# saforem2/l2hmc-qcd

Measured on AMD Instinct MI355X. Metric: chain*leapfrog-steps/sec, 4D SU(3) 8^4 fp64 (+ plaquette/force-kernel HBM GB/s in "rooflines"), higher is better.
Workload: dtype f64; 1 GPU; 4D SU(3) 8x8x8x8, beta=6.0, 256 chains/GPU, complex128/fp64, Dynamics.forward merged L2HMC, nleapfrog=4 (8 LF steps/trajectory), vnet units [256], verbose=False, default Dynamics switches (mc_states.out.v is formed on first access); global_chains=256, parallelism=chains sharded x1

## Files before the change

include/l2q.h:

```cpp
#ifndef L2Q_H_
#define L2Q_H_

#include <stddef.h>
#include <stdint.h>

#ifdef __cplusplus
extern "C" {
#endif

#define L2Q_OK 0
#define L2Q_EINVAL (-1)
#define L2Q_ESHAPE (-2)
#define L2Q_EHIP (-3)

#define L2Q_ACT_NONE 0
#define L2Q_ACT_TANH 1
#define L2Q_ACT_RELU 2
#define L2Q_ACT_LEAKY_RELU 3
#define L2Q_ACT_ELU 4
#define L2Q_ACT_SWISH 5

#define L2Q_HALF_F16 0
#define L2Q_HALF_BF16 1

const char* l2q_last_error(void);
int l2q_version(void);
int l2q_set_tuning(const char* key, int value);
int l2q_kernel_name(const char* entry, int T, int X, int Y, int Z, char* buf, size_t buf_bytes);
int l2q_init(int device);

#define L2Q_COMM_ID_BYTES 128
int l2q_comm_unique_id(void* id_out);
int l2q_comm_init(const void* id, int nranks, int rank, void** comm_out);
int l2q_allreduce_grads(void* comm, void* grad, long n, int elem_bytes, void* stream);
int l2q_comm_destroy(void* comm);
int l2q_comm_abort(void* comm);
int l2q_comm_version(void);

size_t l2q_reduce_ws_bytes(int nb, long n_per_chain);

int l2q_transpose(const void* in, void* out, long batch, int rows, int cols, int elem_bytes,
                  void* stream);
int l2q_su3_pack(const void* x_ref, void* x_nat, int nb, long V, void* stream);
int l2q_su3_unpack(const void* x_nat, void* x_ref, int nb, long V, void* stream);
int l2q_su3_unpack_select(const void* a_nat, const void* b_nat, const float* mask, void* x_ref, int nb,
                          long V, void* stream);

int l2q_su3_plaq_reduce(const void* xn, int nb, int T, int X, int Y, int Z, double* out,
                        void* ws, size_t ws_bytes, void* stream);
int l2q_su3_plaq_planes(const void* xn, int nb, int T, int X, int Y, int Z, double* out, void* ws,
                        size_t ws_bytes, void* stream);
int l2q_su3_wilson_loops(const void* xn, int nb, int T, int X, int Y, int Z, void* out, void* stream);
int l2q_diff_norm2_reduce(const double* a, const double* b, int nb, long n, double* out, void* ws,
                          size_t ws_bytes, void* stream);
int l2q_su3_force(const void* xn, double beta, void* fn, int nb, int T, int X, int Y, int Z,
                  void* stream);
int l2q_su3_force_kick(const void* xn, double beta, double coef, void* vn, int nb, int T,
                       int X, int Y, int Z, void* stream);
int l2q_su3_force_kick_to(const void* xn, double beta, double coef, const void* v_in, void* v_out,
                          int nb, int T, int X, int Y, int Z, void* stream);
int l2q_su3_expm_mul(const void* xn, const void* vn, double eps, const float* mask_n,
                     int complement, void* out, int nb, long V, void* stream);
int l2q_su3_expm_mul2(const void* xn, const void* vn, double eps, const float* mask_n,
                      int complement_first, void* out, int nb, long V, void* stream);
int l2q_su3_expm_mul2_vec8(const void* xn, const void* vn, double eps, const float* mask_n,
                           int complement_first, void* out, double* vec, int nb, long V,
                           void* stream);
int l2q_su3_expm_mul2_digits(const void* xn, const void* vn, double eps, const float* mask_n, int complement_first,
                             void* out, void* image, int a_exp, int nb, long V, void* stream);
int l2q_su3_projsu_digits(const void* in, void* image, int a_exp, long nfields, long V, void* stream);
int l2q_su3_project_su(const void* in, void* out, long nfields, long V, void* stream);
int l2q_su3_projsu_vec8(const void* in, double* vec, long nfields, long V, void* stream);
int l2q_su3_project_u(const void* in, void* out, long nfields, long V, void* stream);
int l2q_su3_mul(const void* a, const void* b, int adjoint_a, int adjoint_b, void* out,
                long nfields, long V, void* stream);
int l2q_su3_project_tah(const void* in, void* out, long nfields, long V, void* stream);
int l2q_su3_kinetic_reduce(const void* vn, int nb, long V, double* out, void* ws,
                           size_t ws_bytes, void* stream);
int l2q_su3_assemble_tah(const double* normals, void* vn, long nfields, long V, void* stream);
int l2q_su3_check_su(const void* xn, int nb, long V, double* out, void* ws, size_t ws_bytes,
                     void* stream);

int l2q_su3_clover_reduce(const void* xn, int nb, int T, int X, int Y, int Z, double* out,
                          void* ws, size_t ws_bytes, void* stream);
int l2q_su3_flow_stage(const void* x_in, const void* p_in, double c, double s, void* p_out, void* x_out,
                       int nb, int T, int X, int Y, int Z, void* stream);
int l2q_su3_flow_step(const void* x_in, void* x_out, void* ws_p, void* ws_x, double eps, int nb, int T, int X,
                      int Y, int Z, void* stream);

int l2q_su3_line_extend(const void* lines_in, const void* xn, int n, void* lines_out, int nb, int T, int X, int Y,
                        int Z, void* stream);
int l2q_su3_loop_reduce(const void* a, int r, const void* b, int t, double* out, int nb, int T, int X, int Y, int Z,
                        void* ws, size_t ws_bytes, void* stream);
int l2q_su3_polyakov(const void* xn, int mu, void* out, int nb, int T, int X, int Y, int Z, void* stream);

int l2q_su3_heatbath(void* xn, double beta, int mu, int parity, const double* u, int ntry, double* fails, int nb,
                     int T, int X, int Y, int Z, void* ws, size_t ws_bytes, void* stream);
int l2q_su3_overrelax(void* xn, int mu, int parity, int nb, int T, int X, int Y, int Z, void* stream);

int l2q_v_update(void* v, const void* force, const void* s, const void* t, const void* q,
                 double eps, int forward, int is_complex, int elem_bytes, int nb, long n,
                 void* logdet, void* ws, size_t ws_bytes, void* stream);
int l2q_v_update_to(const void* v_in, void* v_out, const void* force, const void* s, const void* t,
                    const void* q, double eps, int forward, int is_complex, int elem_bytes, int nb,
                    long n, void* logdet, void* ws, size_t ws_bytes, void* stream);

int l2q_accept(const void* h_init, const void* h_prop, const void* sumlogdet, const void* u,
               void* acc, float* mask, int nb, int elem_bytes, void* stream);
int l2q_select_rows(const void* a, const void* b, const float* mask, void* out, int nb,
                    long row_bytes, void* stream);
int l2q_scale_f64(const double* x, double alpha, double* y, long n, void* stream);

int l2q_gemm_f64(const double* A, const double* W, int M, int N, long K, const double* A2,
                 const double* W2, long K2, const double* bias, const double* bias2,
                 const double* coeff, double scale, int act, double* C, void* ws,
                 size_t ws_bytes, void* stream);
size_t l2q_gemm_ws_bytes(int M, int N, long K, long K2);
size_t l2q_gemm_sliced_bytes(int N, long K);
int l2q_gemm_sliced_build(const double* W, int N, long K, void* image, size_t image_bytes, int* usable,
                          void* stream);
size_t l2q_gemm_sliced_ws_bytes(int M, int N, long K, long K2);
int l2q_gemm_sliced_f64(const double* A, const void* image, long K, int a_exp, const double* A2,
                        const void* image2, long K2, int a2_exp, int M, int N, const double* bias,
                        const double* bias2, const double* coeff, double scale, int act, double* C, void* ws,
                        size_t ws_bytes, void* stream);
size_t l2q_gemm_digits_bytes(long M, long K);
int l2q_gemm_digits_slice(const double* A, long M, long K, int a_exp, void* image, size_t image_bytes, void* stream);
int l2q_gemm_digits_f64(const void* A, const void* image, long K, int a_exp, const void* A2, const void* image2,
                        long K2, int a2_exp, int M, int N, const double* bias, const double* bias2,
                        const double* coeff, double scale, int act, double* C, void* ws, size_t ws_bytes,
                        void* stream);
int l2q_vnet_heads_vupdate_f64(const double* Z, int M, int K, long N, const double* Ws,
                               const double* bs, const double* cs, double scale_s,
                               const double* Wt, const double* bt, double scale_t,
                               const double* Wq, const double* bq, const double* cq,
                               double scale_q, void* v, const void* force, int is_complex,
                               double eps, int forward, double* logdet, void* ws,
                               size_t ws_bytes, void* stream);
int l2q_vnet_heads_vupdate_to_f64(const double* Z, int M, int K, long N, const double* Ws,
                                  const double* bs, const double* cs, double scale_s,
                                  const double* Wt, const double* bt, double scale_t,
                                  const double* Wq, const double* bq, const double* cq,
                                  double scale_q, const void* v_in, void* v_out, const void* force,
                                  int is_complex, double eps, int forward, double* logdet, void* ws,
                                  size_t ws_bytes, void* stream);
int l2q_vnet_heads_vupdate_pair_f64(const double* Z, int M, int K, long N, const double* Ws,
                                    const double* bs, const double* cs, double scale_s,
                                    const double* Wt, const double* bt, double scale_t,
                                    const double* Wq, const double* bq, const double* cq,
                                    double scale_q, void* v, const void* force, int is_complex,
                                    double eps1, int forward1, int flip_between, double eps2,
                                    int forward2, double* logdet, void* ws, size_t ws_bytes,
                                    void* stream);
int l2q_vnet_heads_vupdate_pair_mid_f64(const double* Z, int M, int K, long N, const double* Ws,
                                        const double* bs, const double* cs, double scale_s,
                                        const double* Wt, const double* bt, double scale_t,
                                        const double* Wq, const double* bq, const double* cq,
                                        double scale_q, void* v, const void* force, int is_complex,
                                        double eps1, int forward1, int flip_between, double eps2,
                                        int forward2, double* logdet, double* logdet1,
                                        double* vnorm2_mid, void* ws, size_t ws_bytes, void* stream);
size_t l2q_vnet_heads_ws_bytes(int M, long N);
// ... 221 lines not shown
```

l2hmc-qcd_amd/csrc/heads_common.hpp:

```cpp
#pragma once
#include "l2q_common.hpp"

namespace l2q {

__device__ __forceinline__ double rcp_nr(double d) {
  double r = __builtin_amdgcn_rcp(d);
  r = fma(r, fma(-d, r, 1.0), r);
  r = fma(r, fma(-d, r, 1.0), r);
  return r;
}

__device__ __forceinline__ double fast_tanh(double x) {
  const double c = fmin(fmax(x, -20.0), 20.0);
  const double t = 1.0 - 2.0 * rcp_nr(exp(2.0 * c) + 1.0);
  return (x != x) ? x : t;
}

__device__ __forceinline__ double exp_small(double x) {
  if (fabs(x) < 0.125) {
    double r = 1.0 / 39916800.0;
    r = fma(r, x, 1.0 / 3628800.0);
    r = fma(r, x, 1.0 / 362880.0);
    r = fma(r, x, 1.0 / 40320.0);
    r = fma(r, x, 1.0 / 5040.0);
    r = fma(r, x, 1.0 / 720.0);
    r = fma(r, x, 1.0 / 120.0);
    r = fma(r, x, 1.0 / 24.0);
    r = fma(r, x, 1.0 / 6.0);
    r = fma(r, x, 0.5);
    r = fma(r, x, 1.0);
    return fma(r, x, 1.0);
  }
  return exp(x);
}
__device__ __forceinline__ double exp_bf_core(double xc) {
  const double k = __builtin_rint(xc * 1.4426950408889634);
  double r = fma(-k, 6.93147180369123816490e-01, xc);
  r = fma(-k, 1.90821492927058770002e-10, r);
  double p = 1.0 / 479001600.0;
  p = fma(p, r, 1.0 / 39916800.0);
  p = fma(p, r, 1.0 / 3628800.0);
  p = fma(p, r, 1.0 / 362880.0);
  p = fma(p, r, 1.0 / 40320.0);
  p = fma(p, r, 1.0 / 5040.0);
  p = fma(p, r, 1.0 / 720.0);
  p = fma(p, r, 1.0 / 120.0);
  p = fma(p, r, 1.0 / 24.0);
  p = fma(p, r, 1.0 / 6.0);
  p = fma(p, r, 0.5);
  p = fma(p, r, 1.0);
  p = fma(p, r, 1.0);
  return __builtin_amdgcn_ldexp(p, (int)k);
}
__device__ __forceinline__ double exp_bf(double x) {
  const double y = exp_bf_core(fmin(fmax(x, -708.0), 709.0));
  return (x != x) ? x : y;
}
__device__ __forceinline__ double tanh_bf(double x) {
  const double c = fmin(fmax(x, -20.0), 20.0);
  const double t = 1.0 - 2.0 * rcp_nr(exp_bf_core(2.0 * c) + 1.0);
  return (x != x) ? x : t;
}

struct HeadsArgs {
  const double* Z;
  const double* W[3];
  const double* b[3];
  const double* cs;
  const double* cq;
  double ss, st, sq;
  double eps;
  double eps2;
  int fwd2, flip;
  double* v;
  const double* vin;
  const double* F;
  double* logdet_part;
  double* ld1_part;
  double* ke_part;
  int M, N, K, ncols_part;
  double* tape_s = nullptr;
  double* tape_t = nullptr;
  double* tape_q = nullptr;
};

}
```

l2hmc-qcd_amd/csrc/heads_sliced.hip:

```cpp
#include "heads_common.hpp"
#include <type_traits>
#include <vector>

namespace l2q {

constexpr int OZ_NS = 7;
constexpr int OZ_BITS = 54;
constexpr int OZ_KB = 4;
constexpr int OZ_K = 64 * OZ_KB;
constexpr int OZ_FRAG = 1024;
constexpr int OZ_CHUNK = OZ_NS * OZ_KB * OZ_FRAG;

#ifndef L2Q_SL_PROF
#define L2Q_SL_PROF 0
#endif
#ifndef L2Q_SL_V2
#define L2Q_SL_V2 1
#endif
#ifndef L2Q_SL_SKIP
#define L2Q_SL_SKIP 0
#endif
typedef int v4i32 __attribute__((ext_vector_type(4)));
typedef __attribute__((address_space(3))) void* lds_ptr_t;

// ... 351 lines not shown
    p = fma(p, r, 1.0 / 39916800.0);
    p = fma(p, r, 1.0 / 3628800.0);
    p = fma(p, r, 1.0 / 362880.0);
    p = fma(p, r, 1.0 / 40320.0);
    p = fma(p, r, 1.0 / 5040.0);
    p = fma(p, r, 1.0 / 720.0);
    p = fma(p, r, 1.0 / 120.0);
    p = fma(p, r, 1.0 / 24.0);
    p = fma(p, r, 1.0 / 6.0);
    p = fma(p, r, 0.5);
    p = fma(p, r, 1.0);
    return fma(p, r, 1.0);
  };
#if L2Q_SL_V2
  auto exp_poly7 = [](double r) {
    double p = 1.0 / 5040.0;
    p = fma(p, r, 1.0 / 720.0);
    p = fma(p, r, 1.0 / 120.0);
    p = fma(p, r, 1.0 / 24.0);
    p = fma(p, r, 1.0 / 6.0);
    p = fma(p, r, 0.5);
    p = fma(p, r, 1.0);
    return fma(p, r, 1.0);
  };
#endif
  auto exp4x2 = [&](const double (&xa)[4], const double (&xb)[4], double (&ya)[4], double (&yb)[4]) {
    bool small = true;
#pragma unroll
    for (int r = 0; r < 4; ++r) small = small && fabs(xa[r]) < 0.34 && fabs(xb[r]) < 0.34;
#if L2Q_SL_V2
    bool tiny = true;
#pragma unroll
    for (int r = 0; r < 4; ++r) tiny = tiny && fabs(xa[r]) < 0x1p-6 && fabs(xb[r]) < 0x1p-6;
    if (__all(tiny)) {
#pragma unroll
      for (int r = 0; r < 4; ++r) { ya[r] = exp_poly7(xa[r]); yb[r] = exp_poly7(xb[r]); }
      return;
    }
#endif
    if (__all(small)) {
#pragma unroll
      for (int r = 0; r < 4; ++r) { ya[r] = exp_poly(xa[r]); yb[r] = exp_poly(xb[r]); }
    } else {
#pragma unroll
      for (int r = 0; r < 4; ++r) { ya[r] = exp_bf(xa[r]); yb[r] = exp_bf(xb[r]); }
    }
  };
  auto stage_b = [&] {
    if (L2Q_SL_SKIP & 1) return;
    double xa[4], xb[4];
#pragma unroll
    for (int r = 0; r < 4; ++r) {
      xa[r] = FWD ? heps * s_[r] : -heps * s_[r];
      xb[r] = eps * q_[r];
    }
    exp4x2(xa, xb, es_, eq_);
    if (PAIR && !same2) {
#pragma unroll
      for (int r = 0; r < 4; ++r) {
        xa[r] = a.fwd2 ? h2 * s_[r] : -h2 * s_[r];
        xb[r] = a.eps2 * q_[r];
      }
      exp4x2(xa, xb, es2_, eq2_);
    }
  };
  auto stage_c = [&](long t, const Operands& q, double2 (&outv)[4]) {
    const long n = t * 16 + (lane & 15);
#pragma unroll
    for (int r = 0; r < 4; ++r) {
      const bool ok = n < a.N && (mrow + r) < a.M;
      double vr = q.vv[r].x, vi = q.vv[r].y;
      const double fr0 = q.ff[r].x, fi0 = q.ff[r].y;
      if (L2Q_SL_SKIP & 1) { vr += s_[r] + t_[r] + fr0; vi += q_[r] + fi0; }
      else {
        const double s = s_[r], tt = t_[r];
        const double lj = FWD ? heps * s : -heps * s;
        {
          const double fr = fr0 * eq_[r] + tt, fi = fi0 * eq_[r];
          if (FWD) { vr = es_[r] * vr - heps * fr; vi = es_[r] * vi - heps * fi; }
          else { vr = es_[r] * (vr + heps * fr); vi = es_[r] * (vi + heps * fi); }
        }
        if (!PAIR) {
          if (ok) ld[r] += lj;
        } else {
          if (MID) { if (ok) { ld1[r] += lj; ke[r] += fma(vr, vr, vi * vi); } }
          if (a.flip) { vr = -vr; vi = -vi; }
          const double lj2 = a.fwd2 ? h2 * s : -h2 * s;
          if (ok) ld[r] += lj + lj2;
          const double e2 = same2 ? es_[r] : es2_[r], g2 = same2 ? eq_[r] : eq2_[r];
          const double fr = fr0 * g2 + tt, fi = fi0 * g2;
          if (a.fwd2) { vr = e2 * vr - h2 * fr; vi = e2 * vi - h2 * fi; }
          else { vr = e2 * (vr + h2 * fr); vi = e2 * (vi + h2 * fi); }
        }
      }
      outv[r] = make_double2(vr, vi);
    }
  };
  auto store = [&](long t, const double2 (&outv)[4]) {
    const long n = t * 16 + (lane & 15);
#pragma unroll
    for (int r = 0; r < 4; ++r) {
      if (n < a.N && (mrow + r) < a.M) {
        const long oo = rowoff[r] + n;
        if (CPLX) reinterpret_cast<double2*>(a.v)[oo] = outv[r];
        else a.v[oo] = outv[r].x;
        if (TAPE) { a.tape_s[oo] = s_[r]; a.tape_t[oo] = t_[r]; a.tape_q[oo] = q_[r]; }
      }
    }
  };
  Operands cur, nxt;
  const char* wsrc = o.Wsl + t0 * 3 * (long)OZ_CHUNK + lane * 16;
  auto issue = [&](long qi, int f0) {
    const long qc = qi < nq ? qi : nq - 1;
    const int stage = (int)(qi % 3);
    const char* src = wsrc + qc * (long)OZ_CHUNK;
    __builtin_amdgcn_sched_barrier(0);
#pragma unroll
    for (int f = f0; f < OZ_NS; ++f) {
      const int frag = p + 4 * f;
      __builtin_amdgcn_global_load_lds((const __attribute__((address_space(1))) void*)(src + frag * OZ_FRAG),
                                       (lds_ptr_t)(lds + stage * OZ_CHUNK + frag * OZ_FRAG), 16, 0, 0);
    }
    __builtin_amdgcn_sched_barrier(0);
  };
#if L2Q_SL_PROF
  long long prof_bar = 0, prof_mem = 0, prof_conv = 0;
  const long long prof_t0 = clock64();
#define L2Q_SL_T(acc, ...) do { const long long c0_ = clock64(); __VA_ARGS__; acc += clock64() - c0_; } while (0)
#define L2Q_SL_CBAR(vm) do { const long long c0_ = clock64();                                            \
    asm volatile("s_waitcnt vmcnt(" #vm ") lgkmcnt(0)\n\ts_barrier" ::: "memory"); prof_bar += clock64() - c0_; } while (0)
#else
#define L2Q_SL_T(acc, ...) do { __VA_ARGS__; } while (0)
#define L2Q_SL_CBAR(vm) asm volatile("s_waitcnt vmcnt(" #vm ") lgkmcnt(0)\n\ts_barrier" ::: "memory")
#endif
  double fs[4], ft[4], fq[4], gs[4], gt[4];
  double2 outv[4];
  if (ntl > 0) {
    issue(0, 0);
    issue(1, 0);
    fetch(t0, cur);
    L2Q_SL_CBAR(16);
    issue(2, L2Q_SL_NPD);
    L2Q_SL_CBAR(0);
    issue(3, L2Q_SL_NPD);
    conv(0, fs);
#if L2Q_SL_V2
    tanh_s(cur, fs, sn_);
#endif
    L2Q_SL_CBAR(0);
    issue(4, L2Q_SL_NPD);
    conv(1, ft);
    for (long u = 0; u < ntl; ++u) {
      const long t = t0 + u;
      const bool more = u + 1 < ntl;
      L2Q_SL_CBAR(0);
      L2Q_SL_T(prof_mem, if (u > 0) store(t - 1, outv); issue(3 * u + 5, L2Q_SL_NPD));
      L2Q_SL_T(prof_conv, conv(3 * u + 2, fq));
      L2Q_SL_T(prof_mem, fetch(more ? t + 1 : t, nxt));
      stage_a(cur, fs, ft, fq);
      if (more) {
        L2Q_SL_CBAR(16);
        L2Q_SL_T(prof_mem, issue(3 * u + 6, L2Q_SL_NPD));
        L2Q_SL_T(prof_conv, conv(3 * u + 3, gs));
      }
      stage_b();
      if (more) {
        L2Q_SL_CBAR(0);
        L2Q_SL_T(prof_mem, issue(3 * u + 7, L2Q_SL_NPD));
        L2Q_SL_T(prof_conv, conv(3 * u + 4, gt));
      }
      stage_c(t, cur, outv);
#if L2Q_SL_V2
      if (more) tanh_s(nxt, gs, sn_);
#endif
      if (more) {
        cur = nxt;
#pragma unroll
        for (int r = 0; r < 4; ++r) { fs[r] = gs[r]; ft[r] = gt[r]; }
      }
    }
    store(t1 - 1, outv);
  } else {
    L2Q_SL_CBAR(0);
  }
#undef L2Q_SL_CBAR
#undef L2Q_SL_T
#if L2Q_SL_PROF
  if (o.dbg && lane == 0) {
    long long* d = o.dbg + ((long)blockIdx.x * 8 + wave) * 4;
    d[0] = clock64() - prof_t0; d[1] = prof_bar; d[2] = prof_mem; d[3] = prof_conv;
  }
#endif
  asm volatile("s_waitcnt vmcnt(0)" ::: "memory");
#pragma unroll
  for (int r = 0; r < 4; ++r) {
    double x = ld[r], x1 = ld1[r], xk = ke[r];
#pragma unroll
    for (int off = 8; off > 0; off >>= 1) {
      x += __shfl_xor(x, off, 64);
      if (MID) { x1 += __shfl_xor(x1, off, 64); xk += __shfl_xor(xk, off, 64); }
    }
    const long m = mrow + r;
    if ((lane & 15) == 0 && m < a.M) {
      a.logdet_part[m * a.ncols_part + cw] = x;
      if (MID) {
        a.ld1_part[m * a.ncols_part + cw] = x1;
        a.ke_part[m * a.ncols_part + cw] = xk;
      }
    }
  }
}

static inline long sliced_chunks(long N) { return cdiv(N, 16) * 3; }
static inline size_t sliced_scale_off(long N) { return ((size_t)sliced_chunks(N) * OZ_CHUNK + 255) & ~(size_t)255; }
static inline int sliced_rg(int M) { return (int)cdiv(M, 64); }
static inline int sliced_ncw(int M) {
  const int per_xcd = 32 / sliced_rg(M);
  return 8 * (per_xcd > 0 ? per_xcd : 1);
}

}

using namespace l2q;

static int sliced_launch(const char* who, double* tape_s, double* tape_t, double* tape_q, const double* Z, int M,
                         int K, long N, const void* sliced,
                                      const double* bs, const double* cs, double scale_s, const double* bt,
                                      double scale_t, const double* bq, const double* cq, double scale_q,
                                      const void* v_in, void* v, const void* force, int is_complex, double eps1,
                                      int forward1, int pair, int flip_between, double eps2, int forward2,
                                      double* logdet, double* logdet1, double* vnorm2_mid, void* ws,
                                      size_t ws_bytes, void* stream) {
  L2Q_REQUIRE(Z && sliced && bs && bt && bq && cs && cq && v && force && logdet && ws, L2Q_EINVAL,
              "null pointer (the sliced kernel takes per-entry scales cs / cq)");
  L2Q_REQUIRE(K == OZ_K, L2Q_ESHAPE, "the sliced heads kernel serves K = 256");
  L2Q_REQUIRE(M > 0 && N > 0 && N < 2000000000L, L2Q_EINVAL, "bad size");
  const bool mid = logdet1 != nullptr;
  L2Q_REQUIRE(!mid || (pair && vnorm2_mid), L2Q_EINVAL, "mid-point outputs belong to the pair kernel");
  L2Q_REQUIRE(ws_bytes >= l2q_vnet_heads_sliced_ws_bytes(M, N), L2Q_ESHAPE, "workspace too small");
  auto al = [](const void* p) { return (reinterpret_cast<uintptr_t>(p) & 15) == 0; };
  const void* vin = v_in ? v_in : v;
  L2Q_REQUIRE(al(Z) && al(v) && al(vin) && al(force) && (reinterpret_cast<uintptr_t>(sliced) & 255) == 0 &&
                  (reinterpret_cast<uintptr_t>(ws) & 255) == 0,
              L2Q_ESHAPE, "operands must be 16-byte aligned (slice buffer and workspace 256-byte)");
  hipStream_t st = (hipStream_t)stream;
  const int rg = sliced_rg(M), ncw = sliced_ncw(M);
  const long mpad = (long)rg * 64;
  char* zs = (char*)ws;
  double* zscale = (double*)(zs + (mpad / 16) * OZ_CHUNK);
  double* part = zscale + mpad;
  hipLaunchKernelGGL(oz_split_kernel, dim3((unsigned)cdiv(mpad, 4)), dim3(256), 0, st, Z, (long)M, mpad, 1, 0,
                     zs, zscale, 1, oz_zflag_ptr(), 0x1p-6);
  HeadsArgs a;
  a.tape_s = tape_s; a.tape_t = tape_t; a.tape_q = tape_q;
  a.Z = Z; a.W[0] = a.W[1] = a.W[2] = nullptr;
  a.b[0] = bs; a.b[1] = bt; a.b[2] = bq; a.cs = cs; a.cq = cq;
  a.ss = scale_s; a.st = scale_t; a.sq = scale_q; a.eps = eps1; a.eps2 = eps2; a.fwd2 = forward2;
  a.flip = flip_between;
  a.v = (double*)v; a.vin = (const double*)vin; a.F = (const double*)force;
  a.logdet_part = part; a.ld1_part = part + (size_t)M * ncw; a.ke_part = part + 2 * (size_t)M * ncw;
  a.M = M; a.N = (int)N; a.K = K; a.ncols_part = ncw;
  SlicedArgs o;
  o.Zs = zs; o.zscale = zscale; o.Wsl = (const char*)sliced;
  o.wscale = (const double*)((const char*)sliced + sliced_scale_off(N));
  o.ncw = ncw; o.rg = rg; o.dbg = nullptr;
#if L2Q_SL_PROF
  static long long* dbg = nullptr;
  if (!dbg) (void)hipMalloc(&dbg, 4096 * 8 * 4 * sizeof(long long));
  (void)hipMemsetAsync(dbg, 0, 4096 * 8 * 4 * sizeof(long long), st);
  o.dbg = dbg;
#endif
  o.tiles_per_cw = (int)cdiv(cdiv(N, 16), ncw);
  const dim3 grid((unsigned)(rg * ncw)), block(512);
#define L2Q_SL(C, F, P, MD) hipLaunchKernelGGL((heads_sliced_kernel<C, F, P, MD>), grid, block, 0, st, a, o)
#define L2Q_SL_F(C, P, MD) do { if (forward1) L2Q_SL(C, true, P, MD); else L2Q_SL(C, false, P, MD); } while (0)
#define L2Q_SL_C(P, MD) do { if (is_complex) L2Q_SL_F(true, P, MD); else L2Q_SL_F(false, P, MD); } while (0)
  if (tape_s) {
    if (is_complex) {
      if (forward1) hipLaunchKernelGGL((heads_sliced_kernel<true, true, false, false, true>), grid, block, 0, st, a, o);
      else hipLaunchKernelGGL((heads_sliced_kernel<true, false, false, false, true>), grid, block, 0, st, a, o);
    } else {
      if (forward1) hipLaunchKernelGGL((heads_sliced_kernel<false, true, false, false, true>), grid, block, 0, st, a, o);
      else hipLaunchKernelGGL((heads_sliced_kernel<false, false, false, false, true>), grid, block, 0, st, a, o);
    }
  } else if (mid) L2Q_SL_C(true, true);
  else if (pair) L2Q_SL_C(true, false);
  else L2Q_SL_C(false, false);
#undef L2Q_SL_C
#undef L2Q_SL_F
#undef L2Q_SL
#if L2Q_SL_PROF
  {
    (void)hipStreamSynchronize(st);
    const int nblk = rg * ncw;
    std::vector<long long> h((size_t)nblk * 8 * 4);
    (void)hipMemcpy(h.data(), o.dbg, h.size() * sizeof(long long), hipMemcpyDeviceToHost);
    double tot[2] = {0, 0}, bar[2] = {0, 0}, vm = 0, ldsw = 0, mx[2] = {0, 0}, umem = 0, uconv = 0;
    for (int b = 0; b < nblk; ++b)
      for (int w = 0; w < 8; ++w) {
        const long long* d = &h[((size_t)b * 8 + w) * 4];
        const int c = w >= 4;
        tot[c] += d[0]; bar[c] += d[1]; if (!c) { vm += d[2]; ldsw += d[3]; }
        else { umem += d[2]; uconv += d[3]; }
        if (d[0] > mx[c]) mx[c] = (double)d[0];
      }
    const double n = nblk * 4.0;
    fprintf(stderr, "[sliced prof] matrix waves: total %.0f (max %.0f) barrier %.0f vmcnt %.0f lgkmcnt %.0f | update waves: total %.0f barrier %.0f dma+fetch+store issue %.0f conv %.0f  (clock64 ticks, mean per wave)\n",
            tot[0] / n, mx[0], bar[0] / n, vm / n, ldsw / n, tot[1] / n, bar[1] / n, umem / n, uconv / n);
  }
#endif
  launch_finalize(a.logdet_part, logdet, M, ncw, 1, 1.0, 0.0, st);
  if (mid) {
    launch_finalize(a.ld1_part, logdet1, M, ncw, 1, 1.0, 0.0, st);
    launch_finalize(a.ke_part, vnorm2_mid, M, ncw, 1, 1.0, 0.0, st);
  }
  return check_launch(who);
}

extern "C" {

size_t l2q_heads_sliced_bytes(int K, long N) {
  if (K != OZ_K || N <= 0) return 0;
  return sliced_scale_off(N) + (size_t)3 * N * sizeof(double) + 256;
}

int l2q_heads_sliced_build(const double* Ws, const double* Wt, const double* Wq, int K, long N, void* sliced,
                           size_t sliced_bytes, int* usable, void* stream) {
  L2Q_REQUIRE(Ws && Wt && Wq && sliced && usable, L2Q_EINVAL, "null pointer");
  L2Q_REQUIRE(K == OZ_K, L2Q_ESHAPE, "the sliced heads kernel serves K = 256");
  L2Q_REQUIRE(N > 0 && N < 2000000000L, L2Q_EINVAL, "bad size");
  L2Q_REQUIRE(sliced_bytes >= l2q_heads_sliced_bytes(K, N), L2Q_ESHAPE, "buffer too small");
  auto al = [](const void* p) { return (reinterpret_cast<uintptr_t>(p) & 15) == 0; };
  L2Q_REQUIRE(al(Ws) && al(Wt) && al(Wq) && (reinterpret_cast<uintptr_t>(sliced) & 255) == 0, L2Q_ESHAPE,
              "operands must be 16-byte aligned (the slice buffer 256-byte)");
  hipStream_t st = (hipStream_t)stream;
  char* buf = (char*)sliced;
  double* wscale = (double*)(buf + sliced_scale_off(N));
  int* flag = (int*)(wscale + 3 * N);
  (void)hipMemsetAsync(flag, 0, sizeof(int), st);
  const long Npad = cdiv(N, 16) * 16;
  const double* W[3] = {Ws, Wt, Wq};
  for (int h = 0; h < 3; ++h)
    hipLaunchKernelGGL(oz_split_kernel, dim3((unsigned)cdiv(Npad, 4)), dim3(256), 0, st, W[h], N, Npad, 3, h,
                       buf, wscale + (long)h * N, 0, flag, 0x1p-6);
  int hflag = 0;
  if (hipMemcpyAsync(&hflag, flag, sizeof(int), hipMemcpyDeviceToHost, st) != hipSuccess ||
      hipStreamSynchronize(st) != hipSuccess) {
    set_error("l2q_heads_sliced_build: %s", hipGetErrorString(hipGetLastError()));
    return L2Q_EHIP;
  }
  *usable = hflag ? 0 : 1;
  return check_launch("l2q_heads_sliced_build");
}

int l2q_heads_sliced_zflag(int reset, int* count, void* stream) {
  L2Q_REQUIRE(count, L2Q_EINVAL, "null pointer");
  hipStream_t st = (hipStream_t)stream;
  int* p = oz_zflag_ptr();
  L2Q_REQUIRE(p, L2Q_EHIP, "device symbol not found");
  if (hipMemcpyAsync(count, p, sizeof(int), hipMemcpyDeviceToHost, st) != hipSuccess ||
      (reset && hipMemsetAsync(p, 0, sizeof(int), st) != hipSuccess) ||
      hipStreamSynchronize(st) != hipSuccess) {
    set_error("l2q_heads_sliced_zflag: %s", hipGetErrorString(hipGetLastError()));
    return L2Q_EHIP;
  }
  return L2Q_OK;
}

size_t l2q_vnet_heads_sliced_ws_bytes(int M, long N) {
  if (M <= 0 || N <= 0) return 0;
  const size_t mpad = (size_t)sliced_rg(M) * 64;
  return (mpad / 16) * OZ_CHUNK + mpad * sizeof(double) + (size_t)M * sliced_ncw(M) * 3 * sizeof(double) + 512;
}

int l2q_vnet_heads_vupdate_sliced_f64(const double* Z, int M, int K, long N, const void* sliced,
                                      const double* bs, const double* cs, double scale_s, const double* bt,
                                      double scale_t, const double* bq, const double* cq, double scale_q,
                                      const void* v_in, void* v, const void* force, int is_complex, double eps1,
                                      int forward1, int pair, int flip_between, double eps2, int forward2,
                                      double* logdet, double* logdet1, double* vnorm2_mid, void* ws,
                                      size_t ws_bytes, void* stream) {
  return sliced_launch("l2q_vnet_heads_vupdate_sliced_f64", nullptr, nullptr, nullptr, Z, M, K, N, sliced, bs, cs,
                       scale_s, bt, scale_t, bq, cq, scale_q, v_in, v, force, is_complex, eps1, forward1, pair,
                       flip_between, eps2, forward2, logdet, logdet1, vnorm2_mid, ws, ws_bytes, stream);
}

int l2q_vnet_heads_vupdate_sliced_tape_f64(const double* Z, int M, int K, long N, const void* sliced,
                                           const double* bs, const double* cs, const double* bt, double scale_t,
                                           const double* bq, const double* cq, const void* v_in, void* v,
                                           const void* force, int is_complex, double eps, int forward,
                                           double* s_out, double* t_out, double* q_out, double* logdet, void* ws,
                                           size_t ws_bytes, void* stream) {
  L2Q_REQUIRE(s_out && t_out && q_out, L2Q_EINVAL, "null pointer");
  return sliced_launch("l2q_vnet_heads_vupdate_sliced_tape_f64", s_out, t_out, q_out, Z, M, K, N, sliced, bs, cs, 1.0,
                       bt, scale_t, bq, cq, 1.0, v_in, v, force, is_complex, eps, forward, 0, 0, 0.0, 0, logdet,
                       nullptr, nullptr, ws, ws_bytes, stream);
}

// ... 2 lines not shown
```

l2hmc-qcd_amd/csrc/su3_force_link.hip:

```cpp
#include "su3_force_tile.hpp"
#include "su3_launch.hpp"

namespace l2q {

#ifdef L2Q_LK_NOFENCE
#define L2Q_LK_FENCE() do { } while (0)
#else
#define L2Q_LK_FENCE() do { asm volatile("" ::: "memory"); __builtin_amdgcn_sched_barrier(0); } while (0)
#endif

#ifndef L2Q_LK_EXP
#define L2Q_LK_EXP 0
#endif
#ifndef L2Q_LK_FULL_DIAG
#define L2Q_LK_FULL_DIAG 0
#endif

constexpr int kLkThreads = kRS * 4;
constexpr int kLkOffS0 = 0, kLkOffS1 = 3 * kPlaneB, kLkOffT = 6 * kPlaneB;
constexpr int kLkLds = 7 * kPlaneB;

template <int INM>
__device__ __forceinline__ constexpr bool lk_in(int dir) { return dir == 0 ? true : ((INM >> (dir - 1)) & 1) != 0; }

struct LkCtx {
  __amdgpu_buffer_rsrc_t rs, ro, rv;
  Dims d;
  int V16, Vs16, tile0b, lt, t0, t1;
  int sp, px, py, pz;
  double coef;
  int lo;
};

__host__ __device__ constexpr int lk_other(int mu, int j) { return j + (j >= mu ? 1 : 0); }

template <int MODE, int MU, int INM>
__device__ __forceinline__ void force_link_sweep(const LkCtx& c) {
  constexpr bool IN_MU = lk_in<INM>(MU);
  const Dims& d = c.d;
  const int T = d.T, V16 = c.V16, Vs16 = c.Vs16;
  const __amdgpu_buffer_rsrc_t rs = c.rs, ro = c.ro, rv = c.rv;
  const int q_sp = c.sp * 16;
  int q_pmu = q_sp, mx = c.px, my = c.py, mz = c.pz;
  if (MU != 0) {
    int q = hop(c.sp, c.px, c.py, c.pz, MU, +1, d);
    q_pmu = q * 16;
    mz = q % d.Z; q /= d.Z;
    my = q % d.Y; q /= d.Y;
    mx = q;
  }
  int q_pp[4], q_pm[4], q_pmm[4];
#pragma unroll
  for (int nu = 1; nu < 4; ++nu) {
    q_pp[nu] = hop(c.sp, c.px, c.py, c.pz, nu, +1, d) * 16;
    q_pm[nu] = hop(c.sp, c.px, c.py, c.pz, nu, -1, d) * 16;
    q_pmm[nu] = hop(q_pmu / 16, mx, my, mz, nu, -1, d) * 16;
  }
  const int lb = -c.tile0b;
  const int own = (MU == 0 ? 0 : (MU - 1) * kPlaneB) + c.lt * 16;
  {
    const int ta = (c.t0 - 1 + T) % T;
#pragma unroll
    for (int e = 0; e < 9; ++e) {
      const double2 va = buf_ld(rs, q_sp, (MU * 9 + e) * V16 + ta * Vs16);
      if (MU == 0) {
        *reinterpret_cast<double2*>(fr_lds + kLkOffT + own + e * kEnt) = va;
      } else {
        const double2 vb = buf_ld(rs, q_sp, (MU * 9 + e) * V16 + (c.t0 % T) * Vs16);
        *reinterpret_cast<double2*>(fr_lds + kLkOffS0 + own + e * kEnt) = va;
        *reinterpret_cast<double2*>(fr_lds + kLkOffS1 + own + e * kEnt) = vb;
      }
    }
  }
  __syncthreads();
  int cur = 0;
  M3 carry;
  if (MU != 0) m3_zero(carry);
  const int niter = (c.t1 - c.t0) + 1;
#pragma unroll 1
  for (int it = 0; it < niter; ++it) {
    const int tcur = (c.t0 - 1 + it + T) % T;
    const int tnext = (tcur + 1 == T) ? 0 : tcur + 1;
    const int offSc = cur ? kLkOffS1 : kLkOffS0;
    const int offSn = cur ? kLkOffS0 : kLkOffS1;
    const int gcur = tcur * Vs16, gnxt = tnext * Vs16;
    const bool more = it + 1 < niter;
    auto oc = [&](int rho, int qb) {
      return Opnd<true>{(rho == 0 ? kLkOffT : offSc + (rho - 1) * kPlaneB) + lb + qb, qb, rho * 9 * V16 + gcur};
    };
    auto on = [&](int rho, int qb) {
      return Opnd<true>{offSn + (rho - 1) * kPlaneB + lb + qb, qb, rho * 9 * V16 + gnxt};
    };
#if L2Q_LK_EXP & 1
    auto gco = [&](int rho, int qb) { return oc(rho, q_sp); };
    auto gno = [&](int rho, int qb) { return on(rho == 0 ? 1 : rho, q_sp); };
#else
    auto gco = [&](int rho, int qb) { return Opnd<false>{0, qb, rho * 9 * V16 + gcur}; };
    auto gno = [&](int rho, int qb) { return Opnd<false>{0, qb, rho * 9 * V16 + gnxt}; };
#endif
    double2 pre[9];
    if (more && !(L2Q_LK_EXP & 4)) {
      const int tp = MU == 0 ? tnext : ((tnext + 1 == T) ? 0 : tnext + 1);
#pragma unroll
      for (int e = 0; e < 9; ++e) pre[e] = buf_ld(rs, q_sp, (MU * 9 + e) * V16 + tp * Vs16);
    }
    M3 acc;
    double2 outv[9];
    m3_zero(acc);
    if constexpr (MU == 0) {
      if (it >= c.lo) {
#pragma unroll
        for (int nu_ = 1; nu_ < 4; ++nu_) {
          const int nu = (L2Q_LK_EXP & 64) ? 4 - nu_ : nu_;
          M3 a, t;
          if (it >= c.lo) {
          ld_m(a, on(nu, q_sp), rs, V16);
          if (lk_in<INM>(nu)) mul_xh_stream<false>(t, a, oc(0, q_pp[nu]), rs, V16);
          else mul_xh_stream<false>(t, a, gco(0, q_pp[nu]), rs, V16);
          mac_stream<true>(acc, t, oc(nu, q_sp), rs, V16);
          }
// ... 17 lines not shown
        M3 a, t;
        if (IN_MU) ld_m(a, oc(0, q_pmu), rs, V16);
        else ld_m(a, gco(0, q_pmu), rs, V16);
        if (it >= c.lo) {
          acc = carry;
          mul_xh_stream<false>(t, a, on(MU, q_sp), rs, V16);
          mac_stream<true>(acc, t, oc(0, q_sp), rs, V16);
          L2Q_LK_FENCE();
        }
        if (more) {
          mul_xh_stream<true>(t, a, oc(MU, q_sp), rs, V16);
          m3_zero(carry);
          mac_stream<false>(carry, t, oc(0, q_sp), rs, V16);
          L2Q_LK_FENCE();
        }
      }
      if (it >= c.lo) {
#pragma unroll
        for (int nu_ = 1; nu_ < 4; ++nu_) {
          const int nu = (L2Q_LK_EXP & 64) ? 4 - nu_ : nu_;
          if (nu == MU) continue;
          M3 a, t;
          if (it >= c.lo) {
          if (IN_MU) ld_m(a, oc(nu, q_pmu), rs, V16);
          else ld_m(a, gco(nu, q_pmu), rs, V16);
          if (lk_in<INM>(nu)) mul_xh_stream<false>(t, a, oc(MU, q_pp[nu]), rs, V16);
          else mul_xh_stream<false>(t, a, gco(MU, q_pp[nu]), rs, V16);
          mac_stream<true>(acc, t, oc(nu, q_sp), rs, V16);
          }
          L2Q_LK_FENCE();
          if (it < c.lo) continue;
          if (IN_MU && lk_in<INM>(nu)) ld_m(a, oc(nu, q_pmm[nu]), rs, V16);
          else ld_m(a, gco(nu, q_pmm[nu]), rs, V16);
          if (lk_in<INM>(nu)) {
            mul_xh_stream<true>(t, a, oc(MU, q_pm[nu]), rs, V16);
            mac_stream<false>(acc, t, oc(nu, q_pm[nu]), rs, V16);
            L2Q_LK_FENCE();
          } else {
            mul_xh_stream<true>(t, a, gco(MU, q_pm[nu]), rs, V16);
            mac_stream<false>(acc, t, gco(nu, q_pm[nu]), rs, V16);
            L2Q_LK_FENCE();
          }
        }
      }
    }
    if (MODE == 2 && it >= c.lo) {
      const int so = MU * 9 * V16 + gcur;
      M3 gl, g;
#pragma unroll
      for (int e = 0; e < 9; ++e) {
        const double2 o = buf_ld_nt(rv, q_sp, so + e * V16);
        gl.re[e] = o.x; gl.im[e] = o.y;
      }
      m3_tah(g, gl);
#pragma unroll
      for (int i = 0; i < 3; ++i)
#pragma unroll
        for (int j = 0; j < 3; ++j) {
          double sr = 0.0, si = 0.0;
#pragma unroll
          for (int k = 0; k < 3; ++k) {
            const double ar = acc.re[3 * j + k], ai = -acc.im[3 * j + k];
            sr = fma(g.re[3 * i + k], ar, sr); sr = fma(-g.im[3 * i + k], ai, sr);
            si = fma(g.re[3 * i + k], ai, si); si = fma(g.im[3 * i + k], ar, si);
          }
          const double2 o = buf_ld_nt(ro, q_sp, so + (3 * i + j) * V16);
          outv[3 * i + j] = make_double2(fma(c.coef, sr, o.x), fma(c.coef, si, o.y));
        }
#pragma unroll
      for (int e = 0; e < 9; ++e) buf_st_nt(ro, q_sp, so + e * V16, outv[e]);
    }
    if (MODE != 2 && it >= c.lo) {
      M3 ua;
      const Opnd<true> uo = oc(MU, q_sp);
#pragma unroll
      for (int i = 0; i < 3; ++i) {
        R3 ur;
        ld_row<true>(ur, uo.lds, rs, uo.voff, uo.soff, V16, i);
#pragma unroll
        for (int j = 0; j < 3; ++j) {
          double sr = 0.0, si = 0.0;
#pragma unroll
          for (int k = 0; k < 3; ++k) {
            if (L2Q_LK_FULL_DIAG || i != j) { sr = fma(ur.re[k], acc.re[3 * k + j], sr); sr = fma(-ur.im[k], acc.im[3 * k + j], sr); }
            si = fma(ur.re[k], acc.im[3 * k + j], si); si = fma(ur.im[k], acc.re[3 * k + j], si);
          }
          ua.re[3 * i + j] = sr; ua.im[3 * i + j] = si;
        }
      }
      const int so = MU * 9 * V16 + gcur;
      const double tri = (ua.im[0] + ua.im[4] + ua.im[8]) / 3.0;
#pragma unroll
      for (int i = 0; i < 3; ++i)
#pragma unroll
        for (int j = 0; j < 3; ++j) {
          const int e = 3 * i + j, et = 3 * j + i;
          const double fr = (!L2Q_LK_FULL_DIAG && i == j) ? 0.0 : 0.5 * (ua.re[e] - ua.re[et]);
          double fi = 0.5 * (ua.im[e] + ua.im[et]);
          if (i == j) fi -= tri;
          double2 v2 = make_double2(c.coef * fr, c.coef * fi);
          if (MODE == 1) {
            const double2 o = buf_ld_nt(rv, q_sp, so + e * V16);
            v2.x += o.x; v2.y += o.y;
          }
          outv[e] = v2;
        }
      if (!(L2Q_LK_EXP & 32)) {
#pragma unroll
        for (int e = 0; e < 9; ++e)
          if (!(L2Q_LK_EXP & 2) || outv[e].x == 1.2345e300) {
            if (L2Q_LK_EXP & 16) buf_st(ro, q_sp, so + e * V16, outv[e]);
            else buf_st_nt(ro, q_sp, so + e * V16, outv[e]);
          }
      }
    }
    if (!(L2Q_LK_EXP & 8)) __syncthreads();
    if (more && !(L2Q_LK_EXP & 4)) {
      const int dst = (MU == 0 ? kLkOffT : offSc) + own;
#pragma unroll
      for (int e = 0; e < 9; ++e) *reinterpret_cast<double2*>(fr_lds + dst + e * kEnt) = pre[e];
    }
    if ((L2Q_LK_EXP & 32) && MODE != 2 && it >= c.lo) {
      const int so = MU * 9 * V16 + gcur;
#pragma unroll
      for (int e = 0; e < 9; ++e) {
        if (L2Q_LK_EXP & 16) buf_st(ro, q_sp, so + e * V16, outv[e]);
        else buf_st_nt(ro, q_sp, so + e * V16, outv[e]);
      }
    }
    cur ^= 1;
    if (!(L2Q_LK_EXP & 8)) __syncthreads();
  }
}

#ifndef L2Q_LK_OCC
#define L2Q_LK_OCC 2
#endif
template <int MODE, int INM>
__global__ __launch_bounds__(kLkThreads, L2Q_LK_OCC) void su3_force_link_kernel(
    const double2* __restrict__ xn, Dims d, int nsb, int tsplit, int swz, double coef,
    const double2* vin, double2* out, int lo, int stagger) {
  if (stagger > 0 && blockIdx.x >= 256 && blockIdx.x < 512) {
    for (int i = 0; i < stagger; ++i) __builtin_amdgcn_s_sleep(32);
  }
  const long w = xcd_swizzle(blockIdx.x, gridDim.x, swz);
  const int per_chain = nsb * tsplit;
  const long c = w / per_chain;
  const int rr = (int)(w % per_chain);
  const int tc = rr / nsb, sb = rr % nsb;
  const int V = d.V, T = d.T;
  LkCtx k;
  k.d = d;
  k.V16 = V * 16;
  k.Vs16 = d.X * d.Y * d.Z * 16;
  k.tile0b = sb * kRS * 16;
  k.lt = threadIdx.x & (kRS - 1);
  const int wv = __builtin_amdgcn_readfirstlane(threadIdx.x / kRS);
  const int tlen = (T + tsplit - 1) / tsplit;
  k.t0 = tc * tlen;
  k.t1 = min(T, k.t0 + tlen);
  const int chain_bytes = 36 * k.V16;
  k.rs = __builtin_amdgcn_make_buffer_rsrc((void*)(xn + c * 36L * V), 0, chain_bytes, 0x00020000);
  k.ro = __builtin_amdgcn_make_buffer_rsrc((void*)(out + c * 36L * V), 0, chain_bytes, 0x00020000);
  k.rv = __builtin_amdgcn_make_buffer_rsrc((void*)((MODE != 0 ? vin : out) + c * 36L * V), 0, chain_bytes, 0x00020000);
  k.sp = sb * kRS + k.lt;
  {
    int q = k.sp;
    k.pz = q % d.Z; q /= d.Z;
    k.py = q % d.Y; q /= d.Y;
    k.px = q;
  }
  k.coef = coef;
  k.lo = lo;
  switch (wv) {
    case 0: force_link_sweep<MODE, 0, INM>(k); break;
    case 1: force_link_sweep<MODE, 1, INM>(k); break;
    case 2: force_link_sweep<MODE, 2, INM>(k); break;
    default: force_link_sweep<MODE, 3, INM>(k); break;
  }
}

template <int MODE, int INM>
static void launch_link_variant(const double2* xn, Dims d, int nb, int nsb, int tsplit, double coef,
                                const double2* vin, double2* out, hipStream_t st) {
  static PerDeviceOnce attr_once;
  if (attr_once.first()) {
    (void)hipFuncSetAttribute((const void*)su3_force_link_kernel<MODE, INM>,
                              hipFuncAttributeMaxDynamicSharedMemorySize, kLkLds);
  }
  hipLaunchKernelGGL((su3_force_link_kernel<MODE, INM>), dim3((unsigned)((long)nb * nsb * tsplit)),
                     dim3(kLkThreads), kLkLds, st, xn, d, nsb, tsplit, tuning().xcd_swizzle, coef, vin, out, 1,
                     tuning().force_stagger);
}

int force_link_inmask(const Dims& d) {
  int m = 0;
  if (kRS % d.Z == 0) m |= 4;
  if (kRS % (d.Y * d.Z) == 0) m |= 2;
  if (kRS % (d.X * d.Y * d.Z) == 0) m |= 1;
  return m;
}

bool force_link_applicable(const Dims& d) {
  return (d.X * d.Y * d.Z) % kRS == 0 && 36.0 * d.V * 16.0 < 2.0e9;
}

void launch_force_link_bwd(const double2* xn, Dims d, int nb, double coef, const double2* gf, double2* gx,
                           hipStream_t st) {
  const int Vs = d.X * d.Y * d.Z;
  const int nsb = Vs / kRS;
  const int tsplit = t_chunks((long)nb * nsb, d.T, 1024);
  switch (force_link_inmask(d)) {
    case 7: launch_link_variant<2, 7>(xn, d, nb, nsb, tsplit, coef, gf, gx, st); break;
    case 6: launch_link_variant<2, 6>(xn, d, nb, nsb, tsplit, coef, gf, gx, st); break;
    case 4: launch_link_variant<2, 4>(xn, d, nb, nsb, tsplit, coef, gf, gx, st); break;
    default: launch_link_variant<2, 0>(xn, d, nb, nsb, tsplit, coef, gf, gx, st);
  }
}

void launch_force_link(bool kick, const double2* xn, Dims d, int nb, double coef, double2* out, hipStream_t st,
                       const double2* vin) {
  if (vin == nullptr) vin = out;
  const int Vs = d.X * d.Y * d.Z;
  const int nsb = Vs / kRS;
  const int tsplit = t_chunks((long)nb * nsb, d.T, 1024, tuning().force_tsplit);
#define L2Q_LK_CASE(M)                                                                    \
  case M:                                                                                 \
    if (kick) launch_link_variant<1, M>(xn, d, nb, nsb, tsplit, coef, vin, out, st);           \
    else launch_link_variant<0, M>(xn, d, nb, nsb, tsplit, coef, vin, out, st);                \
    break;
  switch (force_link_inmask(d)) {
    L2Q_LK_CASE(7)
    L2Q_LK_CASE(6)
    L2Q_LK_CASE(4)
    default:
      if (kick) launch_link_variant<1, 0>(xn, d, nb, nsb, tsplit, coef, vin, out, st);
      else launch_link_variant<0, 0>(xn, d, nb, nsb, tsplit, coef, vin, out, st);
  }
#undef L2Q_LK_CASE
}

}
```

l2hmc-qcd_amd/csrc/su3_kernels.hip:

```cpp
#include "su3_launch.hpp"
#include "digits.hpp"
#include "half_common.hpp"

namespace l2q {

template <int OCC>
__global__ __launch_bounds__(kBlock, OCC) void su3_plaq_kernel(const double2* __restrict__ xn,
                                                               Dims d, long nblk, int swz,
                                                               double* __restrict__ partial) {
  __shared__ double lds[8];
  const long total = (long)gridDim.x;
  const long w = xcd_swizzle(blockIdx.x, total, swz);
  const long c = w / nblk, blk = w % nblk;
  const int s = (int)blk * kBlock + threadIdx.x;
  double sr = 0.0, si = 0.0;
  if (s < d.V) {
    const double2* xc = xn + c * 36L * d.V;
    const Site p = site_coords(s, d);
    const int V = d.V;
#pragma unroll 1
    for (int u = 1; u < 4; ++u) {
      const int s_pu = fwd(s, coord_of(p, u), d, u);
#pragma unroll 1
      for (int v = 0; v < u; ++v) {
// ... 610 lines not shown
    }
  }
}
template <bool TWO, bool VEC8>
__global__ __launch_bounds__(kBlock, XU_OCC) void su3_expm_mul_kernel(const double2* xn,
                                                              const double2* __restrict__ vn,
                                                              double eps,
                                                              const float* __restrict__ mask,
                                                              int complement, double2* out,
                                                              double* __restrict__ out_vec,
                                                              int V, long nblk, int lo) {
  const long f = blockIdx.x / nblk, blk = blockIdx.x % nblk;
  const int s = (int)blk * kBlock + threadIdx.x;
  if (s >= V) return;
  su3_expm_mul_body<TWO, VEC8 ? 1 : 0>(xn, vn, eps, mask, complement, out, out_vec, V, f, s, lo, 0.0, 0.0, nullptr);
}
__global__ __launch_bounds__(kBlock, XU_OCC) void su3_expm_mul_digits_kernel(const double2* xn,
                                                                     const double2* __restrict__ vn, double eps,
                                                                     const float* __restrict__ mask, int complement,
                                                                     double2* out, char* __restrict__ image, int V,
                                                                     long nblk, int lo, double dsc, double dlim,
                                                                     int* flag) {
  const long f = blockIdx.x / nblk, blk = blockIdx.x % nblk;
  const int s = (int)blk * kBlock + threadIdx.x;
  if (s >= V) return;
  su3_expm_mul_body<true, 2>(xn, vn, eps, mask, complement, out, image, V, f, s, lo, dsc, dlim, flag);
}

template <int MODE>
__global__ __launch_bounds__(kBlock) void su3_project_kernel(const double2* in,
                                                             double2* out_links,
                                                             double* __restrict__ out_vec, int V,
                                                             long nblk) {
  const long f = blockIdx.x / nblk, blk = blockIdx.x % nblk;
  const int s = (int)blk * kBlock + threadIdx.x;
  if (s >= V) return;
  M3 x, r;
  load_link(x, in + f * 9L * V, V, s);
  if (MODE == 2) {
    m3_tah(r, x);
  } else if (MODE == 3) {
    m3_project_u(r, x);
  } else {
    m3_project_su(r, x);
  }
  if (MODE == 1) {
    double v[8];
    m3_to_vec8(v, r);
#pragma unroll
    for (int a = 0; a < 8; ++a) out_vec[(f * 8 + a) * (long)V + s] = v[a];
  } else {
    store_link(out_links + f * 9L * V, V, s, r);
  }
}
__global__ __launch_bounds__(kBlock) void su3_project_digits_kernel(const double2* in, char* __restrict__ image, int V,
                                                                    long nblk, double dsc, double dlim, int* flag) {
  const long f = blockIdx.x / nblk, blk = blockIdx.x % nblk;
  const int s = (int)blk * kBlock + threadIdx.x;
  if (s >= V) return;
  M3 x, r;
  load_link(x, in + f * 9L * V, V, s);
  m3_project_su(r, x);
  double v[8];
  m3_to_vec8(v, r);
  if (su3_vec8_to_digits(v, image, f, s, V, dsc, dlim)) atomicOr(flag, 1);
}

__global__ __launch_bounds__(kBlock) void su3_mul_kernel(const double2* a, const double2* b,
                                                         int adj_a, int adj_b, double2* out, int V,
                                                         long nblk) {
  const long f = blockIdx.x / nblk, blk = blockIdx.x % nblk;
  const int s = (int)blk * kBlock + threadIdx.x;
  if (s >= V) return;
  M3 x, y, r;
  load_link(x, a + f * 9L * V, V, s);
  load_link(y, b + f * 9L * V, V, s);
  if (adj_a && adj_b) m3_mul_aa(r, x, y);
  else if (adj_a) m3_mul_an(r, x, y);
  else if (adj_b) m3_mul_na(r, x, y);
  else m3_mul_nn(r, x, y);
  store_link(out + f * 9L * V, V, s, r);
}

__global__ __launch_bounds__(kBlock) void su3_assemble_tah_kernel(const double* __restrict__ nrm,
                                                                  double2* __restrict__ vn, long V,
                                                                  long nblk, long nlinks) {
  const long f = blockIdx.x / nblk, blk = blockIdx.x % nblk;
  const long s = blk * kBlock + threadIdx.x;
  if (s >= V) return;
  const long l = f * V + s;
  const double h = 0.70710678118654757;
  const double r3 = h * nrm[0 * nlinks + l];
  const double r8 = h * 0.57735026918962573 * nrm[1 * nlinks + l];
  const double r01 = h * nrm[2 * nlinks + l], r02 = h * nrm[3 * nlinks + l];
  const double r12 = h * nrm[4 * nlinks + l], i01 = h * nrm[5 * nlinks + l];
  const double i02 = h * nrm[6 * nlinks + l], i12 = h * nrm[7 * nlinks + l];
  double2* o = vn + f * 9 * V;
  o[0 * V + s] = make_double2(0.0, r8 + r3);
  o[1 * V + s] = make_double2(r01, i01);
  o[2 * V + s] = make_double2(r02, i02);
  o[3 * V + s] = make_double2(-r01, i01);
  o[4 * V + s] = make_double2(0.0, r8 - r3);
  o[5 * V + s] = make_double2(r12, i12);
  o[6 * V + s] = make_double2(-r02, i02);
  o[7 * V + s] = make_double2(-r12, i12);
  o[8 * V + s] = make_double2(0.0, -2.0 * r8);
}

__global__ __launch_bounds__(kBlock) void su3_norm2_kernel(const double2* __restrict__ vn,
                                                           long n_per_chain, long nblk,
                                                           double* __restrict__ partial) {
  __shared__ double lds[4];
  const long c = blockIdx.x / nblk, blk = blockIdx.x % nblk;
  const double2* v = vn + c * n_per_chain;
  double acc = 0.0;
  const long base = blk * (4L * kBlock);
#pragma unroll
  for (int k = 0; k < 4; ++k) {
    const long j = base + (long)k * kBlock + threadIdx.x;
    if (j < n_per_chain) {
      const double2 d = v[j];
      acc = fma(d.x, d.x, acc);
      acc = fma(d.y, d.y, acc);
    }
  }
  const double r = block_sum(acc, lds);
  if (threadIdx.x == 0) partial[c * nblk + blk] = r;
}

__global__ __launch_bounds__(kBlock) void su3_check_kernel(const double2* __restrict__ xn, long V,
                                                           long nblk, double* __restrict__ psum,
                                                           double* __restrict__ pmax) {
  __shared__ double lds[8];
  const long c = blockIdx.x / nblk, blk = blockIdx.x % nblk;
  const long l = blk * kBlock + threadIdx.x;
  double dv = 0.0;
  const bool on = l < 4 * V;
  if (on) {
    const long mu = l / V, s = l % V;
    M3 x, t;
    load_link(x, xn + (c * 4 + mu) * 9L * V, (int)V, (int)s);
    m3_mul_an(t, x, x);
    t.re[0] -= 1.0; t.re[4] -= 1.0; t.re[8] -= 1.0;
#pragma unroll
    for (int i = 0; i < 9; ++i) dv += t.re[i] * t.re[i] + t.im[i] * t.im[i];
    double dr, di;
    m3_det(dr, di, x);
    dv += (dr - 1.0) * (dr - 1.0) + di * di;
  }
  const double bs = block_sum(dv, lds);
  const double bm = block_max(dv, lds + 4);
  if (threadIdx.x == 0) { psum[c * nblk + blk] = bs; pmax[c * nblk + blk] = bm; }
}

__global__ void check_finalize_kernel(const double* __restrict__ psum,
                                      const double* __restrict__ pmax, long nblk, double nlinks,
                                      double* __restrict__ out) {
  __shared__ double lds[8];
  const long c = blockIdx.x;
  double s = 0.0, m = 0.0;
  for (long b = threadIdx.x; b < nblk; b += blockDim.x) {
    s += psum[c * nblk + b];
    m = fmax(m, pmax[c * nblk + b]);
  }
  const double ts = block_sum(s, lds);
  const double tm = block_max(m, lds + 4);
  if (threadIdx.x == 0) {
    out[c * 2 + 0] = sqrt(ts / nlinks / 20.0);
    out[c * 2 + 1] = sqrt(tm / 20.0);
  }
}

}

using namespace l2q;

template <bool KICK>
struct ForceInst {
  static constexpr int kFS = KICK ? kFSKick : kFSPlain, kVar = KICK ? 2 : 0, kLpt = KICK ? 1 : kLptPlain, kTileOcc = 2;
};

namespace l2q {
ForceKernel pick_force(const Dims& d, bool kick) {
  const int ft = tuning().force_tile;
  if (!kick && ft == 7 && force_plaq_applicable(d)) return ForceKernel::PlaqShare;
  if (ft >= 5 && force_link_applicable(d)) return ForceKernel::Link;
  return (d.X * d.Y * d.Z) % (kick ? kFSKick : kFSPlain) == 0 ? ForceKernel::Slice : ForceKernel::Tile;
}
}

template <bool KICK>
static void launch_force(const double2* xn, Dims d, int nb, double coef, double2* out, hipStream_t st) {
  using I = ForceInst<KICK>;
  switch (pick_force(d, KICK)) {
    case ForceKernel::PlaqShare: launch_force_plaq(xn, d, nb, coef, out, st); return;
    case ForceKernel::Link: launch_force_link(KICK, xn, d, nb, coef, out, st); return;
    case ForceKernel::Slice: {
      const int nsb = d.X * d.Y * d.Z / I::kFS;
      const int tsplit = t_chunks((long)nb * nsb, d.T, 512);
      const size_t lds = 2ul * 4 * 9 * I::kFS * sizeof(double2);
      static PerDeviceOnce attr_once;
      if (attr_once.first()) {
        (void)hipFuncSetAttribute((const void*)su3_force_slice_kernel<KICK, I::kFS, I::kVar, I::kLpt>,
                                  hipFuncAttributeMaxDynamicSharedMemorySize, (int)lds);
      }
      hipLaunchKernelGGL((su3_force_slice_kernel<KICK, I::kFS, I::kVar, I::kLpt>),
                         dim3((unsigned)((long)nb * nsb * tsplit)), dim3(4 * I::kFS / I::kLpt), lds, st, xn, d, nsb,
                         tsplit, tuning().xcd_swizzle, coef, out);
      return;
    }
    case ForceKernel::Tile: {
      const long ntile = cdiv(d.V, 64);
      hipLaunchKernelGGL((su3_force_tile_kernel<KICK, I::kTileOcc>), dim3((unsigned)(nb * ntile)), dim3(kBlock), 0,
                         st, xn, d, ntile, tuning().xcd_swizzle, coef, out);
    }
  }
}

template <bool KICK>
static void force_kernel_name(const Dims& d, char* buf, size_t n) {
  using I = ForceInst<KICK>;
  const char* k = KICK ? "true" : "false";
  switch (pick_force(d, KICK)) {
    case ForceKernel::PlaqShare: snprintf(buf, n, "su3_force_plaq_kernel"); break;
    case ForceKernel::Link: snprintf(buf, n, "su3_force_link_kernel<%d, %d>", KICK, force_link_inmask(d)); break;
    case ForceKernel::Slice:
      snprintf(buf, n, "su3_force_slice_kernel<%s, %d, %d, %d>", k, I::kFS, I::kVar, I::kLpt);
      break;
    case ForceKernel::Tile: snprintf(buf, n, "su3_force_tile_kernel<%s, %d>", k, I::kTileOcc);
  }
}

enum class PlaqKernel { SliceYZ, Slice, Flat };
constexpr int kPlaqOcc = 2;
static PlaqKernel pick_plaq(const Dims& d) {
  if ((d.X * d.Y * d.Z) % kSlice != 0) return PlaqKernel::Flat;
  return kSlice % (d.Y * d.Z) == 0 ? PlaqKernel::SliceYZ : PlaqKernel::Slice;
}

extern "C" {

int l2q_kernel_name(const char* entry, int T, int X, int Y, int Z, char* buf, size_t buf_bytes) {
  L2Q_REQUIRE(entry && buf && buf_bytes > 0, L2Q_EINVAL, "null pointer");
  const Dims dd = strncmp(entry, "l2q_su3_", 8) ? Dims{} : make_dims(T, X, Y, Z);
  buf[0] = 0;
  if (!strcmp(entry, "l2q_su3_plaq_reduce")) {
    const PlaqKernel pk = pick_plaq(dd);
    if (pk == PlaqKernel::Flat) snprintf(buf, buf_bytes, "su3_plaq_kernel<%d>", kPlaqOcc);
    else snprintf(buf, buf_bytes, "su3_plaq_slice_kernel<%s>", pk == PlaqKernel::SliceYZ ? "true" : "false");
  } else if (!strcmp(entry, "l2q_su3_force")) {
    force_kernel_name<false>(dd, buf, buf_bytes);
  } else if (!strcmp(entry, "l2q_su3_force_kick")) {
    force_kernel_name<true>(dd, buf, buf_bytes);
  } else if (!strcmp(entry, "l2q_su3_clover_reduce")) {
    snprintf(buf, buf_bytes, "%s", clover_slice_applicable(dd) ? "su3_clover_slice_kernel" : "su3_clover_kernel");
  } else if (!strcmp(entry, "l2q_su3_flow_stage")) {
    char kick[128];
    force_kernel_name<true>(dd, kick, sizeof(kick));
    snprintf(buf, buf_bytes, "%s + su3_expm_mul_kernel<false, false>", kick);
  } else if (!strcmp(entry, "l2q_vnet_heads_vupdate_sliced_f64")) {
    snprintf(buf, buf_bytes, "heads_sliced_kernel");
  } else if (!strncmp(entry, "l2q_vnet_heads_vupdate", 22)) {
    snprintf(buf, buf_bytes, "%s", heads_f64_kernel_name());
  } else if (!strcmp(entry, "l2q_gemm_h")) {
    snprintf(buf, buf_bytes, "%s", gemm_h_kernel_name(T, X, (long)Y));
  } else if (!strcmp(entry, "l2q_gemm_sliced_f64")) {
    snprintf(buf, buf_bytes, "gemm_sliced_kernel");
  } else if (!strcmp(entry, "l2q_gemm_digits_f64")) {
    snprintf(buf, buf_bytes, "gemm_digits_kernel");
  } else if (!strcmp(entry, "l2q_gemm_digits_slice")) {
    snprintf(buf, buf_bytes, "gd_slice_kernel");
  } else if (!strcmp(entry, "l2q_su3_expm_mul2_digits")) {
    snprintf(buf, buf_bytes, "su3_expm_mul_digits_kernel");
  } else if (!strcmp(entry, "l2q_su3_projsu_digits")) {
    snprintf(buf, buf_bytes, "su3_project_digits_kernel");
  } else if (!strcmp(entry, "l2q_gemm_f64")) {
    snprintf(buf, buf_bytes, "%s", gemm_f64_kernel_name());
  }
  return L2Q_OK;
}

size_t l2q_reduce_ws_bytes(int nb, long n_per_chain) {
  if (nb <= 0 || n_per_chain <= 0) return 0;
  return (size_t)nb * (size_t)cdiv(n_per_chain, kBlock) * 4 * sizeof(double) + 256;
}

int l2q_su3_plaq_reduce(const void* xn, int nb, int T, int X, int Y, int Z, double* out, void* ws,
                        size_t ws_bytes, void* stream) {
  L2Q_REQUIRE(xn && out && ws, L2Q_EINVAL, "null pointer");
  L2Q_REQUIRE(su3_dims_ok(nb, T, X, Y, Z), L2Q_EINVAL, "non-positive size");
  const Dims d = make_dims(T, X, Y, Z);
  hipStream_t st = (hipStream_t)stream;
  double* partial = (double*)ws;
  const int swz = tuning().xcd_swizzle;
  const PlaqKernel pk = pick_plaq(d);
  if (pk != PlaqKernel::Flat) {
    const int nsb = X * Y * Z / kSlice;
    const int tsplit = t_chunks((long)nb * nsb, T, 1024);
    const long per_chain = (long)nsb * tsplit;
    L2Q_REQUIRE(ws_bytes >= (size_t)nb * per_chain * 2 * sizeof(double), L2Q_ESHAPE, "workspace too small");
    if (pk == PlaqKernel::SliceYZ)
      hipLaunchKernelGGL(su3_plaq_slice_kernel<true>, dim3((unsigned)(nb * per_chain)), dim3(kSlice), 0, st,
                         (const double2*)xn, d, nsb, tsplit, swz, partial);
    else hipLaunchKernelGGL(su3_plaq_slice_kernel<false>, dim3((unsigned)(nb * per_chain)), dim3(kSlice), 0, st,
                            (const double2*)xn, d, nsb, tsplit, swz, partial);
    launch_finalize(partial, out, nb, per_chain, 2, 1.0, 0.0, st);
    return check_launch("l2q_su3_plaq_reduce");
  }
  const long nblk = cdiv(d.V, kBlock);
  L2Q_REQUIRE(ws_bytes >= (size_t)nb * nblk * 2 * sizeof(double), L2Q_ESHAPE, "workspace too small");
  hipLaunchKernelGGL(su3_plaq_kernel<kPlaqOcc>, dim3((unsigned)(nb * nblk)), dim3(kBlock), 0, st,
                     (const double2*)xn, d, nblk, swz, partial);
  launch_finalize(partial, out, nb, nblk, 2, 1.0, 0.0, st);
  return check_launch("l2q_su3_plaq_reduce");
}

int l2q_su3_wilson_loops(const void* xn, int nb, int T, int X, int Y, int Z, void* out, void* stream) {
  L2Q_REQUIRE(xn && out, L2Q_EINVAL, "null pointer");
  L2Q_REQUIRE(su3_dims_ok(nb, T, X, Y, Z), L2Q_EINVAL, "non-positive size");
  const Dims d = make_dims(T, X, Y, Z);
  const long nblk = cdiv(d.V, kBlock);
  hipLaunchKernelGGL(su3_wloops_kernel, dim3((unsigned)(nb * nblk)), dim3(kBlock), 0, (hipStream_t)stream,
                     (const double2*)xn, d, nblk, (long)nb, (double2*)out);
  return check_launch("l2q_su3_wilson_loops");
}

int l2q_su3_plaq_planes(const void* xn, int nb, int T, int X, int Y, int Z, double* out, void* ws,
                        size_t ws_bytes, void* stream) {
  L2Q_REQUIRE(xn && out && ws, L2Q_EINVAL, "null pointer");
  L2Q_REQUIRE(su3_dims_ok(nb, T, X, Y, Z), L2Q_EINVAL, "non-positive size");
  const Dims d = make_dims(T, X, Y, Z);
  const long nblk = cdiv(d.V, kBlock);
  L2Q_REQUIRE(ws_bytes >= (size_t)nb * nblk * 12 * sizeof(double), L2Q_ESHAPE, "workspace too small");
  hipStream_t st = (hipStream_t)stream;
  hipLaunchKernelGGL(su3_plaq_planes_kernel, dim3((unsigned)(nb * nblk)), dim3(kBlock), 0, st,
                     (const double2*)xn, d, nblk, (double*)ws);
  launch_finalize((const double*)ws, out, nb, nblk, 12, 1.0, 0.0, st);
  return check_launch("l2q_su3_plaq_planes");
}

int l2q_diff_norm2_reduce(const double* a, const double* b, int nb, long n, double* out, void* ws,
                          size_t ws_bytes, void* stream) {
  L2Q_REQUIRE(a && b && out && ws, L2Q_EINVAL, "null pointer");
  L2Q_REQUIRE(nb > 0 && n > 0, L2Q_EINVAL, "non-positive size");
  const long nblk = cdiv(n, 4L * kBlock);
  L2Q_REQUIRE(ws_bytes >= (size_t)nb * nblk * sizeof(double), L2Q_ESHAPE, "workspace too small");
  hipStream_t st = (hipStream_t)stream;
  hipLaunchKernelGGL(diff_norm2_kernel, dim3((unsigned)(nb * nblk)), dim3(kBlock), 0, st, a, b, n,
                     nblk, (double*)ws);
  launch_finalize((const double*)ws, out, nb, nblk, 1, 1.0, 0.0, st);
  return check_launch("l2q_diff_norm2_reduce");
}

int l2q_su3_force(const void* xn, double beta, void* fn, int nb, int T, int X, int Y, int Z,
                  void* stream) {
  L2Q_REQUIRE(xn && fn, L2Q_EINVAL, "null pointer");
  L2Q_REQUIRE(su3_dims_ok(nb, T, X, Y, Z), L2Q_EINVAL, "non-positive size");
  L2Q_REQUIRE(xn != fn, L2Q_EINVAL, "force output must not alias the gauge field");
  const Dims d = make_dims(T, X, Y, Z);
  launch_force<false>((const double2*)xn, d, nb, beta / 3.0, (double2*)fn, (hipStream_t)stream);
  return check_launch("l2q_su3_force");
}

int l2q_su3_force_kick(const void* xn, double beta, double coef, void* vn, int nb, int T, int X,
                       int Y, int Z, void* stream) {
  L2Q_REQUIRE(xn && vn, L2Q_EINVAL, "null pointer");
  L2Q_REQUIRE(su3_dims_ok(nb, T, X, Y, Z), L2Q_EINVAL, "non-positive size");
  const Dims d = make_dims(T, X, Y, Z);
  launch_force<true>((const double2*)xn, d, nb, coef * beta / 3.0, (double2*)vn, (hipStream_t)stream);
  return check_launch("l2q_su3_force_kick");
}

int l2q_su3_force_kick_to(const void* xn, double beta, double coef, const void* v_in, void* v_out,
                          int nb, int T, int X, int Y, int Z, void* stream) {
  L2Q_REQUIRE(xn && v_in && v_out, L2Q_EINVAL, "null pointer");
  L2Q_REQUIRE(su3_dims_ok(nb, T, X, Y, Z), L2Q_EINVAL, "non-positive size");
  const Dims d = make_dims(T, X, Y, Z);
  hipStream_t st = (hipStream_t)stream;
  if (v_in != v_out && force_link_runs(d)) {
    launch_force_link(true, (const double2*)xn, d, nb, coef * beta / 3.0, (double2*)v_out, st,
                      (const double2*)v_in);
    return check_launch("l2q_su3_force_kick_to");
  }
  if (v_in != v_out)
    (void)hipMemcpyAsync(v_out, v_in, (size_t)nb * 36 * d.V * sizeof(double2), hipMemcpyDeviceToDevice, st);
  return l2q_su3_force_kick(xn, beta, coef, v_out, nb, T, X, Y, Z, stream);
}

int l2q_su3_expm_mul(const void* xn, const void* vn, double eps, const float* mask_n,
                     int complement, void* out, int nb, long V, void* stream) {
  L2Q_REQUIRE(xn && vn && out, L2Q_EINVAL, "null pointer");
  L2Q_REQUIRE(su3_field_ok(nb, V), L2Q_EINVAL, "bad size");
  const long nblk = cdiv(V, kBlock);
  hipLaunchKernelGGL((su3_expm_mul_kernel<false, false>), dim3((unsigned)(nb * 4L * nblk)), dim3(kBlock),
                     0, (hipStream_t)stream, (const double2*)xn, (const double2*)vn, eps, mask_n,
                     complement, (double2*)out, (double*)nullptr, (int)V, nblk, 0);
  return check_launch("l2q_su3_expm_mul");
}

int l2q_su3_expm_mul2(const void* xn, const void* vn, double eps, const float* mask_n,
                      int complement_first, void* out, int nb, long V, void* stream) {
  L2Q_REQUIRE(xn && vn && out && mask_n, L2Q_EINVAL, "null pointer");
  L2Q_REQUIRE(su3_field_ok(nb, V), L2Q_EINVAL, "bad size");
  const long nblk = cdiv(V, kBlock);
  hipLaunchKernelGGL((su3_expm_mul_kernel<true, false>), dim3((unsigned)(nb * 4L * nblk)), dim3(kBlock),
                     0, (hipStream_t)stream, (const double2*)xn, (const double2*)vn, eps, mask_n,
                     complement_first, (double2*)out, (double*)nullptr, (int)V, nblk, 0);
  return check_launch("l2q_su3_expm_mul2");
}

int l2q_su3_expm_mul2_vec8(const void* xn, const void* vn, double eps, const float* mask_n,
                           int complement_first, void* out, double* vec, int nb, long V,
                           void* stream) {
  L2Q_REQUIRE(xn && vn && out && mask_n && vec, L2Q_EINVAL, "null pointer");
  L2Q_REQUIRE(su3_field_ok(nb, V), L2Q_EINVAL, "bad size");
  const long nblk = cdiv(V, kBlock);
  hipLaunchKernelGGL((su3_expm_mul_kernel<true, true>), dim3((unsigned)(nb * 4L * nblk)), dim3(kBlock),
                     0, (hipStream_t)stream, (const double2*)xn, (const double2*)vn, eps, mask_n,
                     complement_first, (double2*)out, vec, (int)V, nblk, 0);
  return check_launch("l2q_su3_expm_mul2_vec8");
}

int l2q_su3_expm_mul2_digits(const void* xn, const void* vn, double eps, const float* mask_n, int complement_first,
                             void* out, void* image, int a_exp, int nb, long V, void* stream) {
  L2Q_REQUIRE(xn && vn && out && mask_n && image, L2Q_EINVAL, "null pointer");
  L2Q_REQUIRE(su3_field_ok(nb, V) && V % 64 == 0, L2Q_EINVAL, "the digit image serves V % 64 == 0");
  L2Q_REQUIRE(a_exp > -900 && a_exp < 900, L2Q_EINVAL, "bad operand exponent");
  L2Q_REQUIRE((reinterpret_cast<uintptr_t>(image) & 15) == 0, L2Q_ESHAPE, "the image must be 16-byte aligned");
  int* flag = gs_flag();
  L2Q_REQUIRE(flag, L2Q_EHIP, "device symbol gs_flag_dev not found");
  const long nblk = cdiv(V, kBlock);
  hipLaunchKernelGGL(su3_expm_mul_digits_kernel, dim3((unsigned)(nb * 4L * nblk)), dim3(kBlock), 0,
                     (hipStream_t)stream, (const double2*)xn, (const double2*)vn, eps, mask_n, complement_first,
                     (double2*)out, (char*)image, (int)V, nblk, 0, ldexp(1.0, GD_BITS - a_exp), ldexp(1.0, a_exp), flag);
  return check_launch("l2q_su3_expm_mul2_digits");
}

int l2q_su3_projsu_digits(const void* in, void* image, int a_exp, long nfields, long V, void* stream) {
  L2Q_REQUIRE(in && image, L2Q_EINVAL, "null pointer");
  L2Q_REQUIRE(su3_field_ok(nfields, V) && V % 64 == 0 && nfields % 4 == 0, L2Q_EINVAL,
              "the digit image serves whole chains (4 fields each) with V % 64 == 0");
  L2Q_REQUIRE(a_exp > -900 && a_exp < 900, L2Q_EINVAL, "bad operand exponent");
  L2Q_REQUIRE((reinterpret_cast<uintptr_t>(image) & 15) == 0, L2Q_ESHAPE, "the image must be 16-byte aligned");
  int* flag = gs_flag();
  L2Q_REQUIRE(flag, L2Q_EHIP, "device symbol gs_flag_dev not found");
  const long nblk = cdiv(V, kBlock);
  hipLaunchKernelGGL(su3_project_digits_kernel, dim3((unsigned)(nfields * nblk)), dim3(kBlock), 0, (hipStream_t)stream,
                     (const double2*)in, (char*)image, (int)V, nblk, ldexp(1.0, GD_BITS - a_exp), ldexp(1.0, a_exp),
                     flag);
  return check_launch("l2q_su3_projsu_digits");
}

int l2q_su3_project_su(const void* in, void* out, long nfields, long V, void* stream) {
  L2Q_REQUIRE(in && out, L2Q_EINVAL, "null pointer");
  L2Q_REQUIRE(su3_field_ok(nfields, V), L2Q_EINVAL, "bad size");
  const long nblk = cdiv(V, kBlock);
  hipLaunchKernelGGL(su3_project_kernel<0>, dim3((unsigned)(nfields * nblk)), dim3(kBlock), 0,
                     (hipStream_t)stream, (const double2*)in, (double2*)out, (double*)nullptr, (int)V,
                     nblk);
  return check_launch("l2q_su3_project_su");
}

int l2q_su3_projsu_vec8(const void* in, double* vec, long nfields, long V, void* stream) {
  L2Q_REQUIRE(in && vec, L2Q_EINVAL, "null pointer");
  L2Q_REQUIRE(su3_field_ok(nfields, V), L2Q_EINVAL, "bad size");
  const long nblk = cdiv(V, kBlock);
  hipLaunchKernelGGL(su3_project_kernel<1>, dim3((unsigned)(nfields * nblk)), dim3(kBlock), 0,
                     (hipStream_t)stream, (const double2*)in, (double2*)nullptr, vec, (int)V, nblk);
  return check_launch("l2q_su3_projsu_vec8");
}

int l2q_su3_project_tah(const void* in, void* out, long nfields, long V, void* stream) {
  L2Q_REQUIRE(in && out, L2Q_EINVAL, "null pointer");
  L2Q_REQUIRE(su3_field_ok(nfields, V), L2Q_EINVAL, "bad size");
  const long nblk = cdiv(V, kBlock);
  hipLaunchKernelGGL(su3_project_kernel<2>, dim3((unsigned)(nfields * nblk)), dim3(kBlock), 0,
                     (hipStream_t)stream, (const double2*)in, (double2*)out, (double*)nullptr, (int)V,
                     nblk);
  return check_launch("l2q_su3_project_tah");
}

int l2q_su3_project_u(const void* in, void* out, long nfields, long V, void* stream) {
  L2Q_REQUIRE(in && out, L2Q_EINVAL, "null pointer");
  L2Q_REQUIRE(su3_field_ok(nfields, V), L2Q_EINVAL, "bad size");
  const long nblk = cdiv(V, kBlock);
  hipLaunchKernelGGL(su3_project_kernel<3>, dim3((unsigned)(nfields * nblk)), dim3(kBlock), 0,
                     (hipStream_t)stream, (const double2*)in, (double2*)out, (double*)nullptr, (int)V,
                     nblk);
  return check_launch("l2q_su3_project_u");
}

int l2q_su3_mul(const void* a, const void* b, int adjoint_a, int adjoint_b, void* out,
                long nfields, long V, void* stream) {
  L2Q_REQUIRE(a && b && out, L2Q_EINVAL, "null pointer");
  L2Q_REQUIRE(su3_field_ok(nfields, V), L2Q_EINVAL, "bad size");
  const long nblk = cdiv(V, kBlock);
  hipLaunchKernelGGL(su3_mul_kernel, dim3((unsigned)(nfields * nblk)), dim3(kBlock), 0,
                     (hipStream_t)stream, (const double2*)a, (const double2*)b, adjoint_a, adjoint_b,
                     (double2*)out, (int)V, nblk);
  return check_launch("l2q_su3_mul");
}

int l2q_su3_kinetic_reduce(const void* vn, int nb, long V, double* out, void* ws, size_t ws_bytes,
                           void* stream) {
  L2Q_REQUIRE(vn && out && ws, L2Q_EINVAL, "null pointer");
  L2Q_REQUIRE(su3_field_ok(nb, V), L2Q_EINVAL, "bad size");
  const long n = 36 * V;
  const long nblk = cdiv(n, 4L * kBlock);
  L2Q_REQUIRE(ws_bytes >= (size_t)nb * nblk * sizeof(double), L2Q_ESHAPE, "workspace too small");
  hipStream_t st = (hipStream_t)stream;
  hipLaunchKernelGGL(su3_norm2_kernel, dim3((unsigned)(nb * nblk)), dim3(kBlock), 0, st,
                     (const double2*)vn, n, nblk, (double*)ws);
  launch_finalize((const double*)ws, out, nb, nblk, 1, 0.5, -0.5 * 8.0 * 4.0 * (double)V, st);
  return check_launch("l2q_su3_kinetic_reduce");
}

int l2q_su3_assemble_tah(const double* normals, void* vn, long nfields, long V, void* stream) {
  L2Q_REQUIRE(normals && vn, L2Q_EINVAL, "null pointer");
  L2Q_REQUIRE(su3_field_ok(nfields, V), L2Q_EINVAL, "bad size");
  const long nblk = cdiv(V, kBlock);
  hipLaunchKernelGGL(su3_assemble_tah_kernel, dim3((unsigned)(nfields * nblk)), dim3(kBlock), 0,
                     (hipStream_t)stream, normals, (double2*)vn, V, nblk, nfields * V);
  return check_launch("l2q_su3_assemble_tah");
}

int l2q_su3_check_su(const void* xn, int nb, long V, double* out, void* ws, size_t ws_bytes,
                     void* stream) {
  L2Q_REQUIRE(xn && out && ws, L2Q_EINVAL, "null pointer");
  L2Q_REQUIRE(su3_field_ok(nb, V), L2Q_EINVAL, "bad size");
  const long nblk = cdiv(4 * V, kBlock);
  L2Q_REQUIRE(ws_bytes >= (size_t)nb * nblk * 2 * sizeof(double), L2Q_ESHAPE, "workspace too small");
  hipStream_t st = (hipStream_t)stream;
  double* psum = (double*)ws;
  double* pmax = psum + (size_t)nb * nblk;
  hipLaunchKernelGGL(su3_check_kernel, dim3((unsigned)(nb * nblk)), dim3(kBlock), 0, st,
                     (const double2*)xn, V, nblk, psum, pmax);
  hipLaunchKernelGGL(check_finalize_kernel, dim3(nb), dim3(kBlock), 0, st, psum, pmax, nblk,
                     4.0 * (double)V, out);
  return check_launch("l2q_su3_check_su");
}

}
```

l2hmc-qcd_amd/csrc/su3_launch.hpp:

```cpp
#pragma once
#include "su3_links.hpp"

namespace l2q {

inline Dims make_dims(int T, int X, int Y, int Z) { return Dims{T, X, Y, Z, T * X * Y * Z}; }

inline bool su3_dims_ok(int nb, int T, int X, int Y, int Z) {
  return nb > 0 && T > 0 && X > 0 && Y > 0 && Z > 0 && (double)T * X * Y * Z * 36.0 < 2.0e9;
}
inline bool su3_field_ok(long n, long V) { return n > 0 && V > 0 && V <= 200000000L; }

inline int t_chunks(long groups, int T, int target, int forced = 0) {
  long tsplit = forced > 0 ? forced : cdiv(target, groups);
  if (tsplit > T) tsplit = T;
  if (tsplit < 1) tsplit = 1;
  return (int)cdiv(T, cdiv(T, tsplit));
}

bool force_link_applicable(const Dims& d);
int force_link_inmask(const Dims& d);
void launch_force_link(bool kick, const double2* xn, Dims d, int nb, double coef, double2* out, hipStream_t st,
                       const double2* vin = nullptr);
void launch_force_link_bwd(const double2* xn, Dims d, int nb, double coef, const double2* gf, double2* gx,
                           hipStream_t st);
bool force_plaq_applicable(const Dims& d);
void launch_force_plaq(const double2* xn, Dims d, int nb, double coef, double2* out, hipStream_t st);
bool clover_slice_applicable(const Dims& d);

enum class ForceKernel { PlaqShare, Link, Slice, Tile };
ForceKernel pick_force(const Dims& d, bool kick);
inline bool force_link_runs(const Dims& d) { return pick_force(d, true) == ForceKernel::Link; }

}
```

l2hmc-qcd_amd/l2hmc/_ops.py:

```python
from __future__ import annotations

import math
from typing import Optional, Sequence

import torch

from . import native as N

C128 = torch.complex128

PARAM_GENERATION = [0]


def _vol(lat: Sequence[int]) -> int:
    v = 1
    for n in lat:
        v *= int(n)
    return v


def _ws(nb: int, n_per_chain: int, device) -> torch.Tensor:
    return N.workspace(N.reduce_ws_bytes(nb, n_per_chain), device)


# ... 11 lines not shown

def su3_pack(x: torch.Tensor) -> torch.Tensor:
    nb = x.shape[0]
    x = x.to(C128).contiguous()
    V = x.numel() // (nb * 36)
    out = torch.empty((nb, 4, 9, V), dtype=C128, device=x.device)
    N.call('l2q_su3_pack', x, out, nb, V)
    return out


def su3_unpack(xn: torch.Tensor, lat: Sequence[int]) -> torch.Tensor:
    nb, _, _, V = xn.shape
    out = torch.empty((nb, 4, *[int(i) for i in lat], 3, 3), dtype=C128, device=xn.device)
    N.call('l2q_su3_unpack', xn.contiguous(), out, nb, V)
    return out


def su3_unpack_select(an: torch.Tensor, bn: torch.Tensor, mask: torch.Tensor,
                      lat: Sequence[int]) -> torch.Tensor:
    nb, _, _, V = an.shape
    out = torch.empty((nb, 4, *[int(i) for i in lat], 3, 3), dtype=C128, device=an.device)
    N.call('l2q_su3_unpack_select', an.contiguous(), bn.contiguous(), mask.to(torch.float32).contiguous(),
           out, nb, V)
    return out


def pack_entries(a: torch.Tensor, V: int, ncomp: int = 9) -> torch.Tensor:
    nb = a.shape[0]
    return transpose(a.reshape(nb * 4, V, ncomp), nb * 4, V, ncomp).reshape(nb, -1)


def unpack_entries(a: torch.Tensor, V: int, ncomp: int = 9) -> torch.Tensor:
    nb = a.shape[0]
    return transpose(a.reshape(nb * 4, ncomp, V), nb * 4, ncomp, V).reshape(nb, -1)


def native_index(V: int, ncomp: int, device) -> torch.Tensor:
    return (torch.arange(4 * V * ncomp, device=device).reshape(4, V, ncomp)
            .permute(0, 2, 1).reshape(-1).contiguous())


def su3_plaq_sums_n(xn: torch.Tensor, lat: Sequence[int]) -> torch.Tensor:
    nb = xn.shape[0]
    T, X, Y, Z = (int(i) for i in lat)
    out = torch.empty((nb, 2), dtype=torch.float64, device=xn.device)
    ws = _ws(nb, T * X * Y * Z * 36, xn.device)
    N.call('l2q_su3_plaq_reduce', xn, nb, T, X, Y, Z, out, ws, ws.numel())
    return out


def su3_plaq_planes_n(xn: torch.Tensor, lat: Sequence[int]) -> torch.Tensor:
    nb = xn.shape[0]
    T, X, Y, Z = (int(i) for i in lat)
    out = torch.empty((nb, 6, 2), dtype=torch.float64, device=xn.device)
    ws = N.workspace(N.reduce_ws_bytes(nb, T * X * Y * Z) * 4, xn.device)
    N.call('l2q_su3_plaq_planes', xn, nb, T, X, Y, Z, out, ws, ws.numel())
    return out


def su3_wilson_loops_n(xn: torch.Tensor, lat: Sequence[int]) -> torch.Tensor:
    nb = xn.shape[0]
    T, X, Y, Z = (int(i) for i in lat)
    out = torch.empty((6, nb, T, X, Y, Z), dtype=C128, device=xn.device)
    N.call('l2q_su3_wilson_loops', xn, nb, T, X, Y, Z, out)
    return out


def diff_norm2(a: torch.Tensor, b: torch.Tensor) -> torch.Tensor:
    nb = a.shape[0]
    a, b = a.contiguous(), b.contiguous()
    n = a.numel() // nb * (2 if a.is_complex() else 1)
    out = torch.empty(nb, dtype=torch.float64, device=a.device)
    ws = _ws(nb, n, a.device)
    N.call('l2q_diff_norm2_reduce', a, b, nb, n, out, ws, ws.numel())
    return out


def su3_force_n(xn: torch.Tensor, beta: float, lat: Sequence[int]) -> torch.Tensor:
    nb = xn.shape[0]
    T, X, Y, Z = (int(i) for i in lat)
    f = torch.empty_like(xn)
    N.call('l2q_su3_force', xn, float(beta), f, nb, T, X, Y, Z)
    return f


def su3_force_kick_n(xn: torch.Tensor, beta: float, coef: float, vn: torch.Tensor,
                     lat: Sequence[int], v_src: Optional[torch.Tensor] = None) -> torch.Tensor:
    T, X, Y, Z = (int(i) for i in lat)
    if v_src is not None:
        assert v_src.shape == vn.shape and v_src.dtype == vn.dtype and v_src.is_contiguous()
        N.call('l2q_su3_force_kick_to', xn, float(beta), float(coef), v_src, vn, xn.shape[0], T, X, Y, Z)
        return vn
    N.call('l2q_su3_force_kick', xn, float(beta), float(coef), vn, xn.shape[0], T, X, Y, Z)
    return vn


def su3_expm_mul_n(xn: torch.Tensor, vn: torch.Tensor, eps: float,
                   mask_n: Optional[torch.Tensor] = None, complement: bool = False,
                   out: Optional[torch.Tensor] = None) -> torch.Tensor:
    nb, _, _, V = xn.shape
    out = torch.empty_like(xn) if out is None else out
    N.call('l2q_su3_expm_mul', xn, vn, float(eps), mask_n, int(complement), out, nb, V)
    return out


def su3_expm_mul2_n(xn: torch.Tensor, vn: torch.Tensor, eps: float, mask_n: torch.Tensor,
                    complement_first: bool, out: Optional[torch.Tensor] = None) -> torch.Tensor:
    nb, _, _, V = xn.shape
    out = torch.empty_like(xn) if out is None else out
    N.call('l2q_su3_expm_mul2', xn, vn, float(eps), mask_n, int(complement_first), out, nb, V)
    return out


def su3_expm_mul2_vec8_n(xn: torch.Tensor, vn: torch.Tensor, eps: float, mask_n: torch.Tensor,
                         complement_first: bool, out: Optional[torch.Tensor] = None):
    nb, _, _, V = xn.shape
    out = torch.empty_like(xn) if out is None else out
    vec = torch.empty((nb, 4, 8, V), dtype=torch.float64, device=xn.device)
    N.call('l2q_su3_expm_mul2_vec8', xn, vn, float(eps), mask_n, int(complement_first), out, vec,
           nb, V)
    return out, vec


def su3_project_su_n(xn: torch.Tensor) -> torch.Tensor:
    out = torch.empty_like(xn)
    nf, V = xn.numel() // (9 * xn.shape[-1]), xn.shape[-1]
    N.call('l2q_su3_project_su', xn, out, nf, V)
    return out


def su3_project_tah_n(xn: torch.Tensor) -> torch.Tensor:
    out = torch.empty_like(xn)
    nf, V = xn.numel() // (9 * xn.shape[-1]), xn.shape[-1]
    N.call('l2q_su3_project_tah', xn, out, nf, V)
    return out


def su3_project_u_n(xn: torch.Tensor) -> torch.Tensor:
    out = torch.empty_like(xn)
    nf, V = xn.numel() // (9 * xn.shape[-1]), xn.shape[-1]
    N.call('l2q_su3_project_u', xn, out, nf, V)
    return out


def su3_mul_n(an: torch.Tensor, bn: torch.Tensor, adjoint_a: bool = False,
              adjoint_b: bool = False) -> torch.Tensor:
    out = torch.empty_like(an)
    nf, V = an.numel() // (9 * an.shape[-1]), an.shape[-1]
    N.call('l2q_su3_mul', an, bn, int(adjoint_a), int(adjoint_b), out, nf, V)
    return out


def su3_projsu_vec8_n(xn: torch.Tensor, out: Optional[torch.Tensor] = None) -> torch.Tensor:
    V = xn.shape[-1]
    nf = xn.numel() // (9 * V)
    shape = (*xn.shape[:-2], 8, V)
    if out is None:
        out = torch.empty(shape, dtype=torch.float64, device=xn.device)
    elif out.numel() != nf * 8 * V or out.dtype != torch.float64 or not out.is_contiguous():
        raise N.L2QError('su3_projsu_vec8_n: bad output buffer')
    N.call('l2q_su3_projsu_vec8', xn, out, nf, V)
    return out.view(shape)


def su3_kinetic_n(vn: torch.Tensor) -> torch.Tensor:
    nb, _, _, V = vn.shape
    out = torch.empty(nb, dtype=torch.float64, device=vn.device)
    ws = _ws(nb, 36 * V, vn.device)
    N.call('l2q_su3_kinetic_reduce', vn, nb, V, out, ws, ws.numel())
    return out


def su3_assemble_tah_n(normals: torch.Tensor) -> torch.Tensor:
    V = normals.shape[-1]
    lead = tuple(normals.shape[1:-1])
    nf = 1
    for i in lead:
        nf *= int(i)
    out = torch.empty((*lead, 9, V), dtype=C128, device=normals.device)
    N.call('l2q_su3_assemble_tah', normals.contiguous(), out, nf, V)
    return out


def su3_check_su_n(xn: torch.Tensor) -> torch.Tensor:
    nb, _, _, V = xn.shape
    out = torch.empty((nb, 2), dtype=torch.float64, device=xn.device)
    ws = _ws(nb, 36 * V, xn.device)
    N.call('l2q_su3_check_su', xn, nb, V, out, ws, ws.numel())
    return out


def su3_clover_sums_n(xn: torch.Tensor, lat: Sequence[int]) -> torch.Tensor:
    nb = xn.shape[0]
    T, X, Y, Z = (int(i) for i in lat)
    out = torch.empty((nb, 3), dtype=torch.float64, device=xn.device)
    ws = _ws(nb, T * X * Y * Z * 36, xn.device)
    N.call('l2q_su3_clover_reduce', xn, nb, T, X, Y, Z, out, ws, ws.numel())
    return out


def su3_flow_stage_n(xn: torch.Tensor, pn: Optional[torch.Tensor], c: float, s: float, lat: Sequence[int],
                     p_out: Optional[torch.Tensor] = None, x_out: Optional[torch.Tensor] = None):
    T, X, Y, Z = (int(i) for i in lat)
    p_out = torch.empty_like(xn) if p_out is None else p_out
    x_out = torch.empty_like(xn) if x_out is None else x_out
    N.call('l2q_su3_flow_stage', xn, pn, float(c), float(s), p_out, x_out, xn.shape[0], T, X, Y, Z)
    return p_out, x_out


def su3_flow_step_n(xn: torch.Tensor, x_out: torch.Tensor, ws_p: torch.Tensor, ws_x: torch.Tensor, eps: float,
                    lat: Sequence[int]) -> torch.Tensor:
    T, X, Y, Z = (int(i) for i in lat)
    N.call('l2q_su3_flow_step', xn, x_out, ws_p, ws_x, float(eps), xn.shape[0], T, X, Y, Z)
    return x_out


def su3_flow_checkpoints_n(xn: torch.Tensor, nsteps: int, eps: float, lat: Sequence[int]):
    cps, cur = [], xn
    if int(nsteps) > 0:
        ws_p, ws_x = torch.empty_like(xn), torch.empty_like(xn)
        for _ in range(int(nsteps)):
            cps.append(cur)
            cur = su3_flow_step_n(cur, torch.empty_like(xn), ws_p, ws_x, eps, lat)
    return cur, cps


def su3_line_extend_n(lines: torch.Tensor, xn: torch.Tensor, n: int, lat: Sequence[int],
                      out: Optional[torch.Tensor] = None) -> torch.Tensor:
    T, X, Y, Z = (int(i) for i in lat)
    out = torch.empty_like(xn) if out is None else out
    N.call('l2q_su3_line_extend', lines, xn, int(n), out, xn.shape[0], T, X, Y, Z)
    return out


def su3_loop_sums_n(a: torch.Tensor, r: int, b: torch.Tensor, t: int, lat: Sequence[int]) -> torch.Tensor:
    nb = a.shape[0]
    T, X, Y, Z = (int(i) for i in lat)
    out = torch.empty((nb, 12, 2), dtype=torch.float64, device=a.device)
    ws = N.workspace(N.reduce_ws_bytes(nb, T * X * Y * Z) * 6, a.device)
    N.call('l2q_su3_loop_reduce', a, int(r), b, int(t), out, nb, T, X, Y, Z, ws, ws.numel())
    return torch.view_as_complex(out)


def su3_polyakov_n(xn: torch.Tensor, mu: int, lat: Sequence[int]) -> torch.Tensor:
    nb = xn.shape[0]
    lat = [int(i) for i in lat]
    mu = int(mu)
    if not 0 <= mu < 4:
        raise ValueError(f'su3_polyakov_n: mu must be 0..3, got {mu}')
    out = torch.empty((nb, *lat[:mu], *lat[mu + 1:]), dtype=C128, device=xn.device)
    N.call('l2q_su3_polyakov', xn, mu, out, nb, *lat)
    return out


def su3_heatbath_(xn: torch.Tensor, beta: float, mu: int, parity: int, u: torch.Tensor, ntry: int,
                  lat: Sequence[int]) -> torch.Tensor:
    nb = xn.shape[0]
    T, X, Y, Z = (int(i) for i in lat)
    ntry = int(ntry)
    vh = T * X * Y * Z // 2
    if u.dtype != torch.float64 or tuple(u.shape) != (nb, 3, 4 * ntry + 2, vh):
        raise ValueError(f'su3_heatbath_: u must be float64 [{nb}, 3, {4 * ntry + 2}, {vh}], got {u.dtype} '
                         f'{list(u.shape)}')
    fails = torch.empty(nb, dtype=torch.float64, device=xn.device)
# ... 337 lines not shown
def mem_gate(what: str, need_bytes: int, fraction: float, device) -> bool:
    pol = MEM_GATE_POLICY[0]
    if pol == 'always':
        ok = True
    elif pol == 'never':
        ok = False
    else:
        key = (what, int(need_bytes))
        if key in _MEM_GATE_AGREED:
            ok = _MEM_GATE_AGREED[key]
        else:
            ok = need_bytes <= fraction * device_headroom(device)
            if _multi_rank():
                ok = _MEM_GATE_AGREED[key] = _ranks_agree(ok, device)
    prev = MEM_GATE_LOG.get(what)
    MEM_GATE_LOG[what] = ok
    if not ok and prev is not False:
        import logging
        logging.getLogger('l2hmc').warning(
            'memory gate: %s not taken (%.2f GiB wanted, policy %s) -- the slower equivalent path runs; '
            'results agree with the faster one to rounding only', what, need_bytes / 2 ** 30, pol)
    return ok


def mem_gate_signature() -> tuple:
    return tuple(sorted(MEM_GATE_LOG.items()))


def heads_sliced_build(heads: dict):
    import ctypes
    ws_, wt, wq = heads['s'][0], heads['t'][0], heads['q'][0]
    n, k = ws_.shape
    if ws_.dtype != torch.float64 or k != SLICED_K or not ws_.is_cuda:
        return None
    nbytes = int(N.load().l2q_heads_sliced_bytes(k, n))
    if not mem_gate('sliced heads image', nbytes, SLICED_IMAGE_MAX_FREE_FRACTION[0], ws_.device):
        return None
    buf = torch.empty(nbytes, dtype=torch.uint8, device=ws_.device)
    usable = ctypes.c_int(0)
    N.call('l2q_heads_sliced_build', ws_, wt, wq, k, n, buf, nbytes, ctypes.byref(usable))
    return buf if usable.value else None


def heads_sliced_build_into(ws_: torch.Tensor, wt: torch.Tensor, wq: torch.Tensor,
                            buf: Optional[torch.Tensor] = None):
    import ctypes
    n, k = ws_.shape
    nbytes = int(N.load().l2q_heads_sliced_bytes(k, n))
    if buf is None or buf.numel() != nbytes or buf.device != ws_.device:
        if not mem_gate('sliced heads image (training tape)', nbytes, SLICED_IMAGE_MAX_FREE_FRACTION[0],
                        ws_.device):
            return None, False
        buf = torch.empty(nbytes, dtype=torch.uint8, device=ws_.device)
    usable = ctypes.c_int(0)
    N.call('l2q_heads_sliced_build', ws_, wt, wq, k, n, buf, nbytes, ctypes.byref(usable))
    return buf, bool(usable.value)


def vnet_heads_vupdate_sliced_tape(z: torch.Tensor, image: torch.Tensor, bs: torch.Tensor, cs: torch.Tensor,
                                   bt: torch.Tensor, scale_t: float, bq: torch.Tensor, cq: torch.Tensor,
                                   v: torch.Tensor, force: torch.Tensor, eps: float, forward: bool):
    m, k = z.shape
    n = bs.numel()
    out = torch.empty_like(v)
    s = torch.empty((m, n), dtype=torch.float64, device=z.device)
    t = torch.empty_like(s)
    q = torch.empty_like(s)
    logdet = torch.empty(m, dtype=torch.float64, device=z.device)
    nbytes = int(N.load().l2q_vnet_heads_sliced_ws_bytes(m, n))
    ws = N.workspace(nbytes, z.device)
    N.call('l2q_vnet_heads_vupdate_sliced_tape_f64', z, m, k, n, image, bs, cs, bt, float(scale_t), bq, cq, v,
           out, force, int(v.is_complex()), float(eps), int(forward), s, t, q, logdet, ws, ws.numel())
    return out, logdet, s, t, q


def heads_sliced_zflag(reset: bool = True) -> int:
    import ctypes
    count = ctypes.c_int(0)
    N.call('l2q_heads_sliced_zflag', int(reset), ctypes.byref(count))
    return int(count.value)


def _sliced_call(z, heads, scales, v, force, eps1, forward1, pair, flip, eps2, forward2, v_src=None,
                 mid=False):
    m, k = z.shape
    _, bs, cs = heads['s']
    _, bt, _ = heads['t']
    wq, bq, cq = heads['q']
    n = wq.shape[0]
    out = torch.empty((3 if mid else 1, m), dtype=torch.float64, device=z.device)
    nbytes = int(N.load().l2q_vnet_heads_sliced_ws_bytes(m, n))
    ws = N.workspace(nbytes, z.device)
    N.call('l2q_vnet_heads_vupdate_sliced_f64', z, m, k, n, heads['sliced'], bs, cs, float(scales[0]), bt,
           float(scales[1]), bq, cq, float(scales[2]), v_src, v, force, int(v.is_complex()), float(eps1),
           int(forward1), int(pair), int(flip), float(eps2), int(forward2), out[0],
           out[1] if mid else None, out[2] if mid else None, ws, ws.numel())
    return out


def _use_sliced(z, heads) -> bool:
    return (USE_SLICED_HEADS[0] and heads.get('use_sliced', True) and heads.get('sliced') is not None
            and z.dtype == torch.float64
            and z.shape[1] == SLICED_K and heads['s'][2] is not None and heads['q'][2] is not None)


def vnet_heads_vupdate_(z: torch.Tensor, heads: dict, scales, v: torch.Tensor,
                        force: torch.Tensor, eps: float, forward: bool,
                        v_src: Optional[torch.Tensor] = None) -> torch.Tensor:
    m, k = z.shape
    ws_, bs, cs = heads['s']
    wt, bt, _ = heads['t']
    wq, bq, cq = heads['q']
    n = ws_.shape[0]
    if _use_sliced(z, heads):
        if v_src is not None:
            assert v_src.shape == v.shape and v_src.dtype == v.dtype and v_src.is_contiguous()
        return _sliced_call(z, heads, scales, v, force, eps, forward, False, False, 0.0, False, v_src)[0]
    logdet = torch.empty(m, dtype=torch.float64, device=z.device)
    nbytes = int(N.load().l2q_vnet_heads_ws_bytes(m, n))
    ws = N.workspace(nbytes, z.device)
    if v_src is not None:
        assert v_src.shape == v.shape and v_src.dtype == v.dtype and v_src.is_contiguous()
        N.call('l2q_vnet_heads_vupdate_to_f64', z, m, k, n, ws_, bs, cs, float(scales[0]), wt, bt,
               float(scales[1]), wq, bq, cq, float(scales[2]), v_src, v, force,
               int(v.is_complex()), float(eps), int(forward), logdet, ws, ws.numel())
        return logdet
    N.call('l2q_vnet_heads_vupdate_f64', z, m, k, n, ws_, bs, cs, float(scales[0]), wt, bt,
           float(scales[1]), wq, bq, cq, float(scales[2]), v, force, int(v.is_complex()),
           float(eps), int(forward), logdet, ws, ws.numel())
    return logdet


def vnet_heads_vupdate_pair_(z: torch.Tensor, heads: dict, scales, v: torch.Tensor,
                             force: torch.Tensor, eps1: float, forward1: bool, flip: bool,
                             eps2: float, forward2: bool) -> torch.Tensor:
    m, k = z.shape
    ws_, bs, cs = heads['s']
    wt, bt, _ = heads['t']
    wq, bq, cq = heads['q']
    n = ws_.shape[0]
    if _use_sliced(z, heads):
        return _sliced_call(z, heads, scales, v, force, eps1, forward1, True, flip, eps2, forward2)[0]
    logdet = torch.empty(m, dtype=torch.float64, device=z.device)
    ws = N.workspace(int(N.load().l2q_vnet_heads_ws_bytes(m, n)), z.device)
    N.call('l2q_vnet_heads_vupdate_pair_f64', z, m, k, n, ws_, bs, cs, float(scales[0]), wt, bt,
           float(scales[1]), wq, bq, cq, float(scales[2]), v, force, int(v.is_complex()),
           float(eps1), int(forward1), int(flip), float(eps2), int(forward2), logdet, ws,
           ws.numel())
    return logdet


def vnet_heads_vupdate_pair_mid_(z: torch.Tensor, heads: dict, scales, v: torch.Tensor,
                                 force: torch.Tensor, eps1: float, forward1: bool, flip: bool,
                                 eps2: float, forward2: bool):
    m, k = z.shape
    ws_, bs, cs = heads['s']
    wt, bt, _ = heads['t']
    wq, bq, cq = heads['q']
    n = ws_.shape[0]
    if _use_sliced(z, heads):
        out = _sliced_call(z, heads, scales, v, force, eps1, forward1, True, flip, eps2, forward2, mid=True)
        return out[0], out[1], out[2]
    out = torch.empty((3, m), dtype=torch.float64, device=z.device)
    ws = N.workspace(int(N.load().l2q_vnet_heads_ws_bytes(m, n)), z.device)
    N.call('l2q_vnet_heads_vupdate_pair_mid_f64', z, m, k, n, ws_, bs, cs, float(scales[0]), wt, bt,
           float(scales[1]), wq, bq, cq, float(scales[2]), v, force, int(v.is_complex()),
           float(eps1), int(forward1), int(flip), float(eps2), int(forward2), out[0], out[1], out[2],
           ws, ws.numel())
    return out[0], out[1], out[2]


def u1_plaq_sums(x: torch.Tensor, lat: Sequence[int]) -> torch.Tensor:
    nb = x.shape[0]
    T, X = (int(i) for i in lat)
    out = torch.empty((nb, 3), dtype=x.dtype, device=x.device)
    N.call('l2q_u1_plaq_reduce', x, nb, T, X, x.element_size(), out)
    return out


def u1_wilson_loops(x: torch.Tensor, lat: Sequence[int]) -> torch.Tensor:
    T, X = (int(i) for i in lat)
    out = torch.empty((x.shape[0], T, X), dtype=x.dtype, device=x.device)
    N.call('l2q_u1_wilson_loops', x, x.shape[0], T, X, x.element_size(), out)
    return out


def u1_wilson_loops_bwd_(dx: torch.Tensor, g: torch.Tensor, lat: Sequence[int]) -> torch.Tensor:
    T, X = (int(i) for i in lat)
    N.call('l2q_u1_wilson_loops_bwd', g.to(dx.dtype).contiguous(), dx.shape[0], T, X, dx.element_size(), dx)
    return dx


def u1_force(x: torch.Tensor, beta: float, lat: Sequence[int]) -> torch.Tensor:
    T, X = (int(i) for i in lat)
    f = torch.empty_like(x)
    N.call('l2q_u1_force', x, float(beta), f, None, 0.0, x.shape[0], T, X, x.element_size())
    return f


def u1_force_kick_(x: torch.Tensor, beta: float, coef: float, v: torch.Tensor,
# ... 601 lines not shown
```

l2hmc-qcd_amd/l2hmc/dynamics/pytorch/dynamics.py:

```python
from __future__ import annotations

import logging
import os
from dataclasses import dataclass
from math import pi as PI
from pathlib import Path
from typing import Callable, Optional, Sequence, Tuple, Union

import numpy as np
import torch
from torch import nn

import l2hmc.configs as cfgs
from l2hmc import DEVICE
from l2hmc import _ops as ops
from l2hmc.dynamics.pytorch.trajectory import SamplerStepper, run_trajectory
from l2hmc.group.su3.pytorch.group import SU3
from l2hmc.group.u1.pytorch.group import U1Phase
from l2hmc.lattice.su3.pytorch.lattice import LatticeSU3
from l2hmc.lattice.u1.pytorch.lattice import LatticeU1
from l2hmc.network.pytorch.network import ConvStack, NetworkFactory, dummy_network

log = logging.getLogger(__name__)

TWO_PI = 2. * PI
Shape = Union[tuple, list]
Tensor = torch.Tensor
Array = np.ndarray

DynamicsInput = Tuple[Tensor, Tensor]
DynamicsOutput = Tuple[Tensor, dict]


class State:

    def __init__(self, x, v, beta, xshape=None):
        self._x, self._v, self.beta = x, v, beta
        if xshape is None:
            xshape = self.x.shape
        self.xshape = xshape
        self.nb = xshape[0]

    @property
    def x(self) -> Tensor:
        if callable(self._x):
            self._x = self._x()
        return self._x

    @x.setter
    def x(self, value) -> None:
        self._x = value

    @property
    def v(self) -> Tensor:
        if callable(self._v):
            self._v = self._v()
        return self._v

    @v.setter
    def v(self, value) -> None:
        self._v = value

    def __iter__(self):
        return iter((self.x, self.v, self.beta))

    def __repr__(self) -> str:
        return f'State(nb={self.nb}, xshape={tuple(self.xshape)}, beta={self.beta})'

    def flatten(self) -> 'State':
        return State(x=self.x.flatten(1), v=self.v.flatten(1), beta=self.beta)

    def to_numpy(self):
        return {'x': self.x.detach().cpu().numpy(), 'v': self.v.detach().cpu().numpy(),
                'beta': torch.as_tensor(self.beta).detach().cpu().numpy()}


@dataclass
class MonteCarloStates:
    init: State
    proposed: State
    out: State


def sigmoid(x: torch.Tensor) -> torch.Tensor:
    return 1. / (1. + torch.exp(-x))

# ... 18 lines not shown

    def combine(self, x: Tensor, y: Tensor) -> Tensor:
        return self.m * x + self.mb * y


def _beta(beta) -> float:
    return float(beta.item()) if isinstance(beta, torch.Tensor) else float(beta)


class Dynamics(nn.Module):
    def __init__(self, potential_fn: Callable, config: cfgs.DynamicsConfig,
                 network_factory: Optional[NetworkFactory] = None):
        super().__init__()
        self.config = config
        self.xdim = self.config.xdim
        self.xshape = self.config.xshape
        self.potential_fn = potential_fn
        self.nlf = self.config.nleapfrog
        self._device = DEVICE
        self.device = DEVICE
        self.group = self.config.group.upper()
        if self.group == 'U1':
            self.g = U1Phase()
            self.lattice = LatticeU1(self.config.nchains, self.config.latvolume)
        else:
            self.g = SU3()
            self.lattice = LatticeSU3(self.config.nchains, self.config.latvolume)
        self.latvolume = tuple(int(i) for i in self.config.latvolume)
        self.volume = int(np.prod(self.latvolume))
        self.network_factory = network_factory
        if network_factory is not None:
            self._networks_built = True
            self.networks = self._build_networks(network_factory)
            self.xnet = self.networks['xnet']
            self.vnet = self.networks['vnet']
            self.register_module('xnet', self.networks['xnet'])
            self.register_module('vnet', self.networks['vnet'])
            if self.group == 'SU3':
                nbytes = sum(p.numel() * p.element_size() for p in self.xnet.parameters())
                dev = DEVICE if isinstance(DEVICE, torch.device) else torch.device(DEVICE)
                if not ops.mem_gate('SU(3) xnet (never called) kept on the device', nbytes, 0.05, dev):
                    self.xnet.to('cpu')
        else:
            self._networks_built = False
            self.xnet = dummy_network
            self.vnet = dummy_network
            self.networks = {'xnet': self.xnet, 'vnet': self.vnet}
        self.masks = self._build_masks()
        self._dtype: torch.dtype = torch.get_default_dtype()
        if self._networks_built:
            self._dtype = self._get_vnet(0).input_layer.xlayer.weight.dtype
        rg = (not self.config.eps_fixed)
        self.xeps = nn.ParameterList([
            nn.parameter.Parameter(torch.tensor(self.config.eps, device=DEVICE),
                                   requires_grad=rg)
            for _ in range(self.config.nleapfrog)])
        self.veps = nn.ParameterList([
            nn.parameter.Parameter(torch.tensor(self.config.eps, device=DEVICE),
                                   requires_grad=rg)
            for _ in range(self.config.nleapfrog)])
        self.rng_device = DEVICE
        self.fuse_heads = True
        self.fuse_x_updates = True
        self.reuse_v_inputs = True
        self.pair_v_updates = True
        self.fuse_x_vec8 = True
        self.fuse_u1_steps = True
        owner = getattr(potential_fn, '__self__', None)
        want = LatticeSU3 if self.group == 'SU3' else LatticeU1
        if not (isinstance(owner, want)
                and getattr(potential_fn, '__name__', '') in ('action', 'potential_energy')):
            raise ValueError(
                'Dynamics(potential_fn=...): expected the bound `action` of a '
                f'{want.__name__} (got {potential_fn!r}); the HIP trajectory computes the Wilson / '
                'improved gauge action itself and cannot call an arbitrary potential')
        if [int(i) for i in owner._lattice_shape] != [int(i) for i in self.config.latvolume]:
            raise ValueError(f'potential_fn belongs to a lattice of shape {owner._lattice_shape}, '
                             f'config.latvolume is {list(self.config.latvolume)}')
        self.potential_c1 = float(getattr(owner, 'c1', 0.0) or 0.0) if self.group == 'SU3' else 0.0
        self.net_precision = None
        self.fuse_half_heads = True
        self.merge_hmc_kicks = True
        self._inject: Optional[dict] = None
        self._eps_cache: dict = {}
        self._masks_native: Optional[list] = None
        self._perm: dict = {}
        self._xcache = None
        self.cache_native_output = False
        self.pair_v_updates_verbose = True
        self.sliced_heads = True
        self.sliced_train_heads = True
        self.sliced_train_input = False
        self.defer_weight_grads = True
        self.fuse_x_halves_train = True
        self.fuse_v_pairs_bwd = True
        self.sliced_input = True
        self.autograd_forward = True
        self.native_training = True
        self.auto_graph = True
        self.auto_graph_su3 = False
        self.auto_graph_after = 3
        self._graphs: dict = {}
        self._graph_seen: dict = {}

    def train(self, mode: bool = True):
        was = self.training
        super().train(mode)
        if was and not mode and self._networks_built:
            from l2hmc.network.pytorch.network import LeapfrogLayer
            for m in self.networks.modules():
                if isinstance(m, LeapfrogLayer):
                    m.native_train_release()
        return self

    def set_net_precision(self, precision) -> None:
        table = {None: None, 'float32': None, 'fp32': None, 'fp16': torch.float16,
                 'bf16': torch.bfloat16, torch.float16: torch.float16,
                 torch.bfloat16: torch.bfloat16, torch.float32: None}
        if precision not in table:
            raise ValueError(f'set_net_precision: {precision!r}')
        half = table[precision]
        if half is not None and self.group != 'U1':
            raise ValueError('half-precision networks: U(1) only (SU(3) is complex128 by '
                             'definition, group/su3/pytorch/group.py:41)')
        from l2hmc.network.pytorch.network import LeapfrogLayer
        for m in self.networks.modules():
            if isinstance(m, LeapfrogLayer):
                m.set_precision(half)
        self.net_precision = half

    def get_models(self) -> dict:
        if self.config.use_separate_networks:
            xnet, vnet = {}, {}
            for lf in range(self.config.nleapfrog):
                vnet[str(lf)] = self._get_vnet(lf)
                if self.config.use_split_xnets:
                    xnet[str(lf)] = {'0': self._get_xnet(lf, first=True),
                                     '1': self._get_xnet(lf, first=False)}
                else:
                    xnet[str(lf)] = self._get_xnet(lf, first=True)
        else:
            vnet = self._get_vnet(0)
            if self.config.use_split_xnets:
                xnet = {'0': self._get_xnet(0, first=True), '1': self._get_xnet(0, first=False)}
            else:
                xnet = self._get_xnet(0, first=True)
        return {'xnet': xnet, 'vnet': vnet}

    def _build_networks(self, network_factory: NetworkFactory) -> nn.ModuleDict:
        split = self.config.use_split_xnets
        n = self.nlf if self.config.use_separate_networks else 1
        return network_factory.build_networks(n, split, group=self.g)

    def _build_masks(self):
        masks = []
        for _ in range(self.config.nleapfrog):
            _idx = np.arange(self.xdim)
            idx = np.random.permutation(_idx)[:self.xdim // 2]
            mask = np.zeros((self.xdim,), dtype=np.float32)
            mask[idx] = 1.
            masks.append(torch.from_numpy(mask[None, :]))
        return masks

    def set_masks(self, masks: Sequence) -> None:
        self.masks = [torch.as_tensor(np.asarray(m), dtype=torch.float32).reshape(1, -1)
                      for m in masks]
# ... 84 lines not shown
                                  float(sigmoid(vals[i].log())), q)
        return self._eps_cache[key][1]

    def _get_vnet(self, step: int):
        if not self._networks_built:
            return self.vnet
        if self.config.use_separate_networks:
            return self.vnet.get_submodule(str(step))
        return self.vnet

    def _get_xnet(self, step: int, first: bool = False):
        if not self._networks_built:
            return self.xnet
        if self.config.use_separate_networks:
            xnet = self.xnet.get_submodule(str(step))
            if self.config.use_split_xnets:
                return xnet.get_submodule('first') if first else xnet.get_submodule('second')
            return xnet
        return self.xnet

    def _get_mask(self, step: int) -> tuple[Tensor, Tensor]:
        m = self.masks[step]
        return m, torch.ones_like(m) - m

    def _native_masks(self) -> list:
        if self._masks_native is None:
            out = []
            for m in self.masks:
                m = m.to(DEVICE).reshape(1, -1).contiguous()
                if self.group == 'SU3':
                    m = ops.pack_entries(m, self.volume)
                out.append(m.reshape(-1).contiguous())
            self._masks_native = out
        return self._masks_native

    def _perms(self):
        if not self._perm:
            self._perm = {'in': ops.native_index(self.volume, 8, DEVICE),
                          'out': ops.native_index(self.volume, 9, DEVICE)}
        return self._perm

    def _pack(self, a: Tensor) -> Tensor:
        a = a.to(DEVICE)
        if self.group == 'SU3':
            return ops.su3_pack(a.reshape(a.shape[0], -1))
        return a.reshape(a.shape[0], 2, *self.latvolume).contiguous().clone()

    def _pack_input(self, x: Tensor) -> Tensor:
        c, self._xcache = self._xcache, None
        if (c is not None and self.group == 'SU3' and x is c[0] and x._version == c[1]
                and self.cache_native_output):
            return c[2]
        return self._pack(x)

    def _unpack(self, an: Tensor) -> Tensor:
        if self.group == 'SU3':
            return ops.su3_unpack(an, self.latvolume)
        return an.reshape(an.shape[0], 2, *self.latvolume)

    def _force_n(self, xn: Tensor, beta) -> Tensor:
        if self.group == 'SU3':
            return ops.su3_force_n(xn, _beta(beta), self.latvolume)
        return ops.u1_force(xn, _beta(beta), self.latvolume)

    def _kick_n(self, xn: Tensor, vn: Tensor, beta, coef: float,
                v_src: Optional[Tensor] = None) -> None:
        if self.group == 'SU3':
            ops.su3_force_kick_n(xn, _beta(beta), coef, vn, self.latvolume, v_src)
        else:
            if v_src is not None:
                vn.copy_(v_src)
            ops.u1_force_kick_(xn, _beta(beta), coef, vn, self.latvolume)

    def _potential_n(self, xn: Tensor, beta) -> Tensor:
        if self.group == 'SU3':
            b, c1 = _beta(beta), self.potential_c1
            pe = (-b * (1.0 - 8.0 * c1) / 3.0) * ops.su3_plaq_sums_n(xn, self.latvolume)[:, 0]
            if c1 != 0.0:
                pe = pe + (-b * c1 / 3.0) * ops.su3_rect_sums_n(xn, self.latvolume)
            return pe
        s = ops.u1_plaq_sums(xn, self.latvolume)
        return _beta(beta) * (self.volume - s[:, 0])

    def _kinetic_n(self, vn: Tensor) -> Tensor:
        return ops.su3_kinetic_n(vn) if self.group == 'SU3' else ops.u1_kinetic(vn)

    def _hamiltonian_n(self, xn: Tensor, vn: Tensor, beta) -> Tensor:
        return self._kinetic_n(vn) + self._potential_n(xn, beta)

    def _momentum_n(self, nb: int) -> Tensor:
        inj = self._inject.get('normals') if self._inject else None
        if self.group == 'SU3':
            shape = (nb, 4, *self.latvolume)
            if inj is not None:
                nrm = torch.as_tensor(inj, dtype=torch.float64).to(DEVICE)
            elif self.rng_device == 'cpu':
                nrm = torch.stack([torch.randn(shape, dtype=torch.float64)
                                   for _ in range(8)]).to(DEVICE)
            else:
                nrm = torch.randn((8, *shape), dtype=torch.float64, device=DEVICE)
            return ops.su3_assemble_tah_n(nrm.reshape(8, nb, 4, self.volume))
        shape = (nb, 2, *self.latvolume)
        if inj is not None:
            v = torch.as_tensor(inj).to(DEVICE)
        else:
            v = torch.randn(shape, device=self.rng_device).to(DEVICE)
        return v.reshape(nb, -1).to(self._real_dtype()).contiguous()

    def _real_dtype(self) -> torch.dtype:
        return torch.float64 if self.group == 'SU3' else self._dtype

    def _uniform(self, acc: Tensor) -> Tensor:
        inj = self._inject.get('u') if self._inject else None
        if inj is not None:
            return torch.as_tensor(inj).to(device=DEVICE, dtype=acc.dtype)
        if self.rng_device == 'cpu':
            return torch.rand(acc.shape, dtype=acc.dtype).to(DEVICE)
        return torch.rand_like(acc)

    def _vnet_n(self, step: int, xn: Tensor, fn: Tensor):
        vnet = self._get_vnet(step)
        nb = xn.shape[0]
        if not self._networks_built:
            z = torch.zeros((nb, self.xdim), dtype=self._real_dtype(), device=DEVICE)
            return z, z, z
        if self.group == 'SU3':
            p = self._perms()
            w = vnet.kernel_weights(p['in'], p['out'])
            xv = ops.su3_projsu_vec8_n(xn).reshape(nb, -1)
            fv = ops.su3_projsu_vec8_n(fn).reshape(nb, -1)
            return vnet.forward_flat(xv, fv, w)
        x = xn
        if isinstance(vnet.input_layer.conv_stack, ConvStack):
            x = vnet.input_layer.conv_stack(xn)
        return vnet.forward_flat(x.reshape(nb, -1), fn.reshape(nb, -1))

    def _xnet_n(self, step: int, first: bool, xn: Tensor, vn: Tensor, mask: Tensor,
                complement: bool):
        xnet = self._get_xnet(step, first)
        nb = xn.shape[0]
        if not self._networks_built:
            z = torch.zeros((nb, self.xdim), dtype=self._real_dtype(), device=DEVICE)
            return z, z, z
        xm = ops.u1_masked_cos_sin(xn, mask, complement, self.latvolume)
        if isinstance(xnet.input_layer.conv_stack, ConvStack):
            xm = xnet.input_layer.conv_stack(xm)
        return xnet.forward_flat(xm.reshape(nb, -1), vn.reshape(nb, -1))

    def _can_fuse_heads(self, vnet) -> bool:
        return (self.fuse_heads and self._networks_built and self.group == 'SU3'
                and vnet.units[-1] % 2 == 0)

    def _digit_inputs(self, vnet, nb: int, V: int) -> bool:
        if (self.training or not self.sliced_input or not ops.USE_SLICED_INPUT[0] or not ops.USE_DIGIT_INPUTS[0]
                or not ops.digits_ok(nb, V) or not self._can_fuse_heads(vnet)):
            return False
        if getattr(vnet, 'half_dtype', None) is not None:
            return False
        p = self._perms()
        w = vnet.kernel_weights(p['in'], p['out'])
        return (w.get('input_img') is not None and w['wx'].dtype == torch.float64
                and ops.gemm_sliced_pays(nb, w['wx'].shape[0], 32 * V, 32 * V))

    def _v_inputs_n(self, vnet, xn: Tensor, beta, ts: Optional[SamplerStepper] = None):
        nb = xn.shape[0]
        reuse = ts is not None and ts.reuse
        if reuse and ts.valid:
            fn = ts.F
        else:
            fn = self._force_n(xn, beta)
            if reuse:
                ts.valid, ts.F = True, fn
                ts.xv = ts.fv = None
                ts.z = {}
        if not self._can_fuse_heads(vnet):
            return fn, None, None
        p = self._perms()
        w = vnet.kernel_weights(p['in'], p['out'])
        hs = w['heads_scaled']
        hs['use_sliced'] = bool(self._sliced_wanted(vnet) and ops.USE_SLICED_HEADS[0])
        if hs['use_sliced'] and 'sliced' not in hs:
            hs['sliced'] = ops.heads_sliced_build(hs)
        if reuse and id(vnet) in ts.z:
            return fn, ts.z[id(vnet)], w
        if reuse and ts.xv is not None:
            xv, fv = ts.xv, ts.fv
            if isinstance(xv, ops.DigitImage) and not self._digit_inputs(vnet, nb, xn.shape[-1]):
                xv = ops.su3_projsu_vec8_n(xn).reshape(nb, -1)
                fv = ops.su3_projsu_vec8_n(fn).reshape(nb, -1)
        else:
            pre = None
            if reuse:
                pre, ts.xv_pre = ts.xv_pre, None
            if self._digit_inputs(vnet, nb, xn.shape[-1]):
                xv = pre if isinstance(pre, ops.DigitImage) else ops.su3_projsu_digits_n(xn)
                fv = ops.su3_projsu_digits_n(fn)
            else:
                if isinstance(pre, ops.DigitImage):
                    pre = None
                xv = pre if pre is not None else ops.su3_projsu_vec8_n(xn).reshape(nb, -1)
                fv = ops.su3_projsu_vec8_n(fn).reshape(nb, -1)
            if reuse:
                ts.xv, ts.fv = xv, fv
        z = vnet.hidden_flat(xv, fv, w, sliced_exp=ops.SLICED_INPUT_EXP if self.sliced_input else None)
        if reuse:
            ts.z[id(vnet)] = z
        return fn, z, w

    def _sliced_wanted(self, vnet) -> bool:
        if self.sliced_heads == 'force':
            return True
        return bool(self.sliced_heads) and getattr(vnet, 'act', None) == 'tanh'

    def _fused_u1(self, net) -> Optional[dict]:
        if not (self.fuse_u1_steps and self.group == 'U1' and self._networks_built
                and self._dtype == torch.float32 and self.xdim <= ops.u1_fused_max_n()
                and getattr(net, 'half_dtype', None) is None):
            return None
        net._check_mode()
        return net.kernel_weights().get('fused_u1')

    def _half_fused(self, net) -> bool:
        return (self.group == 'U1' and self._networks_built and self.fuse_half_heads
                and getattr(net, 'half_dtype', None) is not None)

    def _update_v_n(self, step: int, xn: Tensor, vn: Tensor, beta, forward: bool,
                    ts: Optional[SamplerStepper] = None, acc: Optional[Tensor] = None,
                    v_src: Optional[Tensor] = None) -> Tensor:
        eps = self._eps('v', step)
        nb = xn.shape[0]
        vnet = self._get_vnet(step)
        if v_src is not None and not (self.group == 'SU3' and self._can_fuse_heads(vnet)):
            vn.copy_(v_src)
            v_src = None
        fw = self._fused_u1(vnet)
        if fw is not None:
            return ops.u1_vstep_(xn, vn, _beta(beta), eps, forward, self.latvolume, fw, acc)
        if self._half_fused(vnet):
            fn = self._force_n(xn, beta)
            x = xn
            if isinstance(vnet.input_layer.conv_stack, ConvStack):
                x = vnet.input_layer.conv_stack(xn)
            w = vnet.kernel_weights()
            z = vnet.hidden_flat_h(x.reshape(nb, -1), fn.reshape(nb, -1), w)
            return ops.u1_heads_update_h_(z, w['h']['heads_scaled'], vnet.nw.t, vn.reshape(nb, -1),
                                          fn.reshape(nb, -1), eps, forward)
        fn, z, w = self._v_inputs_n(vnet, xn, beta, ts)
        if z is not None:
            return ops.vnet_heads_vupdate_(z, w['heads_scaled'], (vnet.nw.s, vnet.nw.t, vnet.nw.q),
                                           vn.reshape(nb, -1), fn.reshape(nb, -1), eps, forward,
                                           None if v_src is None else v_src.reshape(nb, -1))
        if v_src is not None:
            vn.copy_(v_src)
        s, t, q = self._vnet_n(step, xn, fn)
        return ops.v_update_(vn.reshape(nb, -1), fn.reshape(nb, -1), s, t, q, eps, forward)

    def _update_v_pair_n(self, step0: int, forward0: bool, flip: bool, step1: int,
                         forward1: bool, xn: Tensor, vn: Tensor, beta,
                         ts: Optional[SamplerStepper] = None) -> Tensor:
        nb = xn.shape[0]
        vnet = self._get_vnet(step1)
        fn, z, w = self._v_inputs_n(vnet, xn, beta, ts)
        args = (z, w['heads_scaled'], (vnet.nw.s, vnet.nw.t, vnet.nw.q), vn.reshape(nb, -1),
                fn.reshape(nb, -1), self._eps('v', step0), forward0, flip, self._eps('v', step1),
                forward1)
        if ts is None or not ts.late:
            return ops.vnet_heads_vupdate_pair_(*args)
        ld, ts.ld1, vn2 = ops.vnet_heads_vupdate_pair_mid_(*args)
        ts.ke = 0.5 * (vn2 - 8.0 * 4.0 * self.volume)
        return ld - ts.ld1

    def _can_pair_mid(self) -> bool:
        if self.group != 'SU3' or not self._networks_built:
            return False
        return all(int(self._get_vnet(st).units[-1]) % 16 == 0
                   for st in range(self.config.nleapfrog))

    def _update_x_n(self, step: int, xn: Tensor, vn: Tensor, mask: Tensor, complement: bool,
                    forward: bool, first: bool, acc: Optional[Tensor] = None) -> Optional[Tensor]:
        eps = self._eps('x', step)
        if self.group == 'SU3':
            ops.su3_expm_mul_n(xn, vn, eps if forward else -eps, mask, complement, out=xn)
            return None
        nb = xn.shape[0]
        fw = self._fused_u1(self._get_xnet(step, first))
        if fw is not None:
            return ops.u1_xstep_(xn.reshape(nb, -1), vn, mask, complement, eps, forward,
                                 self.config.use_ncp, fw, acc)
        xnet = self._get_xnet(step, first)
        if self._half_fused(xnet):
            w = xnet.kernel_weights()
            if isinstance(xnet.input_layer.conv_stack, ConvStack):
                xm = ops.u1_masked_cos_sin(xn, mask, complement, self.latvolume)
                xm = xnet.input_layer.conv_stack(xm)
                z = xnet.hidden_flat_h(xm.reshape(nb, -1), vn.reshape(nb, -1), w)
            else:
                z = xnet.hidden_flat_h_u1x(xn.reshape(nb, -1), mask, complement,
                                           vn.reshape(nb, -1), w)
            return ops.u1_heads_update_h_(z, w['h']['heads_scaled'], xnet.nw.t,
                                          xn.reshape(nb, -1), vn.reshape(nb, -1), eps, forward,
                                          mask=mask, complement=complement,
                                          use_ncp=self.config.use_ncp)
        s, t, q = self._xnet_n(step, first, xn, vn, mask, complement)
        return ops.u1_x_update_(xn.reshape(nb, -1), vn, s, t, q, mask, complement, eps,
                                forward, self.config.use_ncp)

    def _flip_v_n(self, vn: Tensor) -> Tensor:
        if self.group == 'SU3':
            return ops.scale(vn, -1.0, out=vn)
        return vn.neg_()

    def _lf_n(self, step: int, xn: Tensor, vn: Tensor, beta, forward: bool,
              ts: Optional[SamplerStepper] = None) -> Tensor:
        if forward:
            st, order = step, ((False, True), (True, False))
        else:
            st = self.config.nleapfrog - step - 1
            order = ((True, False), (False, True))
        m = self._native_masks()[st]
        if self.group == 'U1' and self.fuse_u1_steps:
            fv = self._fused_u1(self._get_vnet(st))
            fx = {True: self._fused_u1(self._get_xnet(st, True)),
                  False: self._fused_u1(self._get_xnet(st, False))} if fv is not None else None
            if fv is not None and fx[True] is not None and fx[False] is not None:
                nb, b = xn.shape[0], _beta(beta)
                ev, ex = self._eps('v', st), self._eps('x', st)
                ld = ops.u1_vstep_(xn, vn, b, ev, forward, self.latvolume, fv)
                for comp, first in order:
                    ops.u1_xstep_(xn.reshape(nb, -1), vn, m, comp, ex, forward,
                                  self.config.use_ncp, fx[first], ld)
                ops.u1_vstep_(xn, vn, b, ev, forward, self.latvolume, fv, ld)
                return ld
        prev = x_src = v_src = None
        if ts is not None:
            prev, x_src, v_src = ts.pending, ts.x_src, ts.v_src
            ts.pending = ts.x_src = ts.v_src = None
        late = bool(prev is not None and ts.late)
        xr = xn if x_src is None else x_src
        if v_src is not None and prev is not None:
            vn.copy_(v_src)
            v_src = None
        if prev is not None:
            st0, f0, flip = prev
            v0, v1 = self._get_vnet(st0), self._get_vnet(st)
            if v0 is v1 and self._can_fuse_heads(v1):
                ld = self._update_v_pair_n(st0, f0, flip, st, forward, xr, vn, beta, ts)
            else:
                ld = self._update_v_n(st0, xr, vn, beta, f0, ts)
                if late:
                    ts.ld1, ts.ke = ld, self._kinetic_n(vn)
                if flip:
                    self._flip_v_n(vn)
                l1 = self._update_v_n(st, xr, vn, beta, forward, ts)
                ld = l1 if late else ld + l1
        else:
            ld = self._update_v_n(st, xr, vn, beta, forward, ts, v_src=v_src)
        if self.group == 'SU3' and self.fuse_x_updates:
            eps = self._eps('x', st)
            if (ts is not None and ts.reuse and self.fuse_x_vec8
                    and self._can_fuse_heads(self._get_vnet(st))):
                if self._digit_inputs(self._get_vnet(st), xn.shape[0], xn.shape[-1]):
                    _, ts.xv_pre = ops.su3_expm_mul2_digits_n(xr, vn, eps if forward else -eps, m, not forward,
                                                              out=xn)
                else:
                    _, xv = ops.su3_expm_mul2_vec8_n(xr, vn, eps if forward else -eps, m, not forward,
                                                     out=xn)
                    ts.xv_pre = xv.reshape(xn.shape[0], -1)
            else:
                ops.su3_expm_mul2_n(xr, vn, eps if forward else -eps, m, not forward, out=xn)
        else:
            if x_src is not None:
                xn.copy_(x_src)
            for comp, first in order:
                l = self._update_x_n(st, xn, vn, m, comp, forward, first)
                if l is not None:
                    ld = ld + l
        if ts is not None:
            ts.valid = False
            if ts.defer:
                ts.pending = (st, forward, False)
                return ld
        return ld + self._update_v_n(st, xn, vn, beta, forward, ts)

    def _flush_pending_n(self, ts: Optional[SamplerStepper], xn, vn, beta) -> Optional[Tensor]:
        prev = ts.pending if ts is not None else None
        if prev is None:
            return None
        ts.pending = None
        st0, f0, flip = prev
        ld = self._update_v_n(st0, xn, vn, beta, f0, ts)
        if flip:
            self._flip_v_n(vn)
        return ld

    def group_to_vec(self, x: Tensor) -> Tensor:
        return self.g.group_to_vec(self.unflatten(x))

    def vec_to_group(self, x: Tensor) -> Tensor:
        x = self.unflatten(x)
        if self.group == 'SU3':
            return self.g.vec_to_group(x)
        return torch.complex(x[..., 0], x[..., 1])

    def grad_potential(self, x: Tensor, beta: Tensor) -> Tensor:
        return self.lattice.grad_action(x, beta)

    def hamiltonian(self, state: State) -> Tensor:
        return self.kinetic_energy(state.v) + self.potential_energy(state.x, state.beta)

    def kinetic_energy(self, v: Tensor) -> Tensor:
        return self._kinetic_n(self._pack(v) if self.group == 'SU3'
                               else v.to(DEVICE).reshape(v.shape[0], -1).contiguous())

    def potential_energy(self, x: Tensor, beta: Tensor):
        return self.potential_fn(x, beta)

    def _call_vnet(self, step: int, inputs: tuple[Tensor, Tensor]):
        x, force = inputs
        s, t, q = self._vnet_n(step, self._pack(x), self._pack(force))
        return self._heads_to_reference(s, t, q)

    def _call_xnet(self, step: int, inputs: tuple[Tensor, Tensor], first: bool = False):
        x, v = inputs
        if self.group == 'SU3':
            xnet = self._get_xnet(step, first)
            x = torch.stack([x.real, x.imag], 1)
            v = torch.stack([v.real, v.imag], 1)
            return xnet((x, v))
        ones = torch.ones(self.xdim, dtype=torch.float32, device=DEVICE)
        return self._xnet_n(step, first, self._pack(x), v.to(DEVICE).reshape(x.shape[0], -1),
                            ones, False)

    def _heads_to_reference(self, s, t, q):
        if self.group == 'SU3':
            return tuple(ops.unpack_entries(a, self.volume) for a in (s, t, q))
        return s, t, q

    def _update_v(self, step: int, state: State, forward: bool) -> tuple[State, Tensor]:
        xn = self._pack(state.x)
        vn = self._pack(state.v) if self.group == 'SU3' else \
            state.v.to(DEVICE).reshape(state.v.shape[0], -1).contiguous().clone()
        ld = self._update_v_n(step, xn, vn, state.beta, forward)
        v = self._unpack(vn) if self.group == 'SU3' else vn.reshape(state.v.shape)
        return State(state.x, v, state.beta), ld

    def _update_v_fwd(self, step: int, state: State) -> tuple[State, Tensor]:
        return self._update_v(step, state, True)

    def _update_v_bwd(self, step: int, state: State) -> tuple[State, Tensor]:
        return self._update_v(step, state, False)

    def _update_x(self, step: int, state: State, m: Tensor, first: bool, forward: bool):
        xn = self._pack(state.x)
        nb = xn.shape[0]
        m = m.to(DEVICE).reshape(1, -1).float().contiguous()
        if self.group == 'SU3':
            vn = self._pack(state.v)
            mask = ops.pack_entries(m, self.volume).reshape(-1)
        else:
            vn = state.v.to(DEVICE).reshape(nb, -1).contiguous()
            mask = m.reshape(-1)
        ld = self._update_x_n(step, xn, vn, mask, False, forward, first)
        if ld is None:
            ld = torch.zeros(nb, dtype=torch.get_default_dtype(), device=DEVICE)
        return State(x=self._unpack(xn), v=state.v, beta=state.beta), ld

    def _update_x_fwd(self, step: int, state: State, m: Tensor, first: bool):
        return self._update_x(step, state, m, first, True)

    def _update_x_bwd(self, step: int, state: State, m: Tensor, first: bool):
        return self._update_x(step, state, m, first, False)

    def _lf(self, step: int, state: State, forward: bool) -> tuple[State, Tensor]:
# ... 424 lines not shown
        nb, n = x.shape[0], x[0].numel()
        ones = torch.ones(n, dtype=torch.float32, device=DEVICE)
        cs = ops.u1_masked_cos_sin(x.reshape(nb, n), ones, False, (n // 2,)).reshape(nb, 2, n)
        return torch.stack([cs[:, 0].reshape(x.shape), cs[:, 1].reshape(x.shape)], dim=-1)

    @staticmethod
    def complexify(x: Tensor, dim: int = 1) -> Tensor:
        assert len(x.shape) >= 2
        assert x.shape[dim] == 2
        if dim != 1:
            xr, xi = x.transpose(0, dim)
            return torch.complex(xr.transpose(0, dim - 1), xi.transpose(0, dim - 1))
        if len(x.shape) == 2:
            return torch.complex(x[:, 0], x[:, 1])
        return torch.complex(x[:, 0, ...], x[:, 1, ...])

    def generate_proposal_hmc(self, inputs, eps=None, nleapfrog=None) -> dict:
        x, beta = inputs
        xn = self._pack(x)
        vn = self._momentum_n(xn.shape[0])
        x_, v_, hist = self._kernel_hmc_n(xn, vn, beta, eps, nleapfrog)
        return {'init': self._state_from_n(xn, vn, beta),
                'proposed': self._state_from_n(x_, v_, beta), 'metrics': hist}

    def generate_proposal_fb(self, inputs) -> dict:
        x, beta = inputs
        xn = self._pack(x)
        vn = self._momentum_n(xn.shape[0])
        x_, v_, hist = self._kernel_fb_n(xn, vn, beta)
        return {'init': self._state_from_n(xn, vn, beta),
                'proposed': self._state_from_n(x_, v_, beta), 'metrics': hist}

    def generate_proposal(self, inputs, forward: bool) -> dict:
        x, beta = inputs
        xn = self._pack(x)
        vn = self._momentum_n(xn.shape[0])
        x_, v_, hist = self._kernel_n(xn, vn, beta, forward)
        return {'init': self._state_from_n(xn, vn, beta),
                'proposed': self._state_from_n(x_, v_, beta), 'metrics': hist}

    def make_graphed(self, x: Tensor, beta: float, mode: str = 'fb', eps: Optional[float] = None,
                     nleapfrog: Optional[int] = None, warmup: int = 2) -> 'GraphedTransition':
        return GraphedTransition(self, x, float(beta), mode, eps, nleapfrog, warmup)

    def random_state(self, beta: float) -> State:
        x = self.g.random(list(self.xshape)).to(self.device)
        v = self.g.random_momentum(list(self.xshape)).to(x.device)
        return State(x=x, v=v, beta=torch.tensor(beta).to(self.device))

    def test_reversibility(self) -> dict[str, Array]:
        state = self.random_state(beta=1.)
        state_fwd, _ = self.transition_kernel(state, forward=True)
        state_, _ = self.transition_kernel(state_fwd, forward=False)
        dx = torch.abs(state.x - state_.x.reshape(state.x.shape))
        dv = torch.abs(state.v - state_.v.reshape(state.v.shape))
        return {'dx': dx.detach().cpu().numpy(), 'dv': dv.detach().cpu().numpy()}


class GraphedTransition:

    def __init__(self, dyn: Dynamics, x: Tensor, beta: float, mode: str, eps, nleapfrog,
                 warmup: int):
        assert mode in ('fb', 'hmc')
        if not torch.cuda.is_available():
            raise RuntimeError('GraphedTransition needs a GPU')
        self.dyn, self.beta, self.mode = dyn, beta, mode
        self._eps, self._nleapfrog, self._warmup = eps, nleapfrog, max(1, warmup)
        self.static_x = x.to(DEVICE).clone()
        self.captures = 0
        self.replays = 0
        self._capture()

    def _signature(self) -> tuple:
        d = self.dyn
        plist = getattr(self, '_plist', None)
        if plist is None:
            plist = self._plist = list(d.parameters())
        eps_ids = tuple(id(p) for p in d.xeps) + tuple(id(p) for p in d.veps)
        params = (eps_ids, tuple(p._version for p in plist))
        masks = tuple(id(m) for m in d.masks)
        flags = (d.fuse_heads, d.fuse_x_updates, d.reuse_v_inputs, d.pair_v_updates,
                 d.fuse_u1_steps, d.fuse_half_heads, d.merge_hmc_kicks, d.sliced_heads,
                 ops.USE_SLICED_HEADS[0], d.sliced_input, ops.USE_SLICED_INPUT[0], ops.USE_DIGIT_INPUTS[0],
                 d.pair_v_updates_verbose,
                 getattr(d, 'fuse_x_vec8', None), d.net_precision, d.config.verbose, d.training)
        return (ops.PARAM_GENERATION[0], params, masks, flags)

    def _run(self):
        if self.mode == 'fb':
            return self.dyn.apply_transition_fb((self.static_x, self.beta))
        return self.dyn.apply_transition_hmc((self.static_x, self.beta), eps=self._eps,
                                             nleapfrog=self._nleapfrog)

    def _capture(self) -> None:
        from l2hmc import native
        side = torch.cuda.Stream()
        side.wait_stream(torch.cuda.current_stream())
        with torch.cuda.stream(side):
            for _ in range(self._warmup):
                self._run()
        torch.cuda.current_stream().wait_stream(side)
        torch.cuda.synchronize()
        self._pinned = [native.pin_workspace(), list(self.dyn._native_masks())]
        from l2hmc.network.pytorch.network import LeapfrogLayer
        for m in self.dyn.modules():
            if isinstance(m, LeapfrogLayer):
                self._pinned.append(dict(m._head_cache))
        self.graph = torch.cuda.CUDAGraph()
        with torch.cuda.graph(self.graph):
            self.out_x, self.out_metrics = self._run()
        self._plist = None
        self._sig = self._signature()
        self.captures += 1

    def __call__(self, x: Tensor):
        if self._signature() != self._sig:
            self._capture()
        self.static_x.copy_(x.reshape(self.static_x.shape))
        self.graph.replay()
        self.replays += 1
        return self.out_x, self.out_metrics
```

l2hmc-qcd_amd/l2hmc/dynamics/pytorch/trajectory.py:

```python
from __future__ import annotations

import torch

Tensor = torch.Tensor


class SamplerStepper:
    __slots__ = ('dyn', 'beta', 'reuse', 'defer', 'late', 'lazy', 'x_src', 'v_src',
                 'valid', 'F', 'xv_pre', 'xv', 'fv', 'z',
                 'pending', 'ld1', 'ke')

    def __init__(self, dyn, beta, merged: bool):
        verbose = dyn.config.verbose
        su3 = dyn.group == 'SU3' and dyn._networks_built
        self.dyn, self.beta = dyn, beta
        self.reuse = bool(dyn.reuse_v_inputs)
        can_pair = merged and su3 and self.reuse and dyn.pair_v_updates
        self.late = bool(verbose and can_pair and dyn.pair_v_updates_verbose and dyn._can_pair_mid())
        self.defer = bool(can_pair and (not verbose or self.late))
        self.x_src = self.v_src = None
        self.valid = False
        self.F = self.xv_pre = self.xv = self.fv = None
        self.z = {}
        self.pending = self.ld1 = self.ke = None
        self.lazy = bool(merged and su3 and dyn.config.nleapfrog > 0)

    def start(self, xn: Tensor, vn: Tensor):
        if not self.lazy:
            return xn.clone(), vn.clone()
        self.x_src, self.v_src = xn, vn
        return torch.empty_like(xn), torch.empty_like(vn)

    def step(self, step: int, x: Tensor, v: Tensor, forward: bool):
        return x, v, self.dyn._lf_n(step, x, v, self.beta, forward, self)

    def flip(self, v: Tensor) -> Tensor:
        if self.pending is None:
            return self.dyn._flip_v_n(v)
        self.pending = (*self.pending[:2], True)
        return v

    def finish(self, x: Tensor, v: Tensor):
        return self.dyn._flush_pending_n(self, x, v, self.beta)


def run_trajectory(dyn, stepper, xn: Tensor, vn: Tensor, beta, directions: tuple):
    merged = len(directions) == 2
    verbose, nlf = dyn.config.verbose, dyn.config.nleapfrog
    x, v = stepper.start(xn, vn)
    sumlogdet = dyn._zeros_nb(xn.shape[0])
    sldf = sldb = torch.zeros_like(sumlogdet) if merged else None
    history: dict = {}
    h = h_init = dyn._hamiltonian_n(xn, vn, beta)

    def add_sld(forward, logdet):
        nonlocal sldf, sldb
        if forward:
            sldf = sldf + logdet
        else:
            sldb = sldb + logdet

    def record(energy, idx=None, forward=True):
        m = {'energy': energy, 'logprob': energy - sumlogdet, 'logdet': sumlogdet}
        if merged:
            m.update({'sldf': sldf if forward else torch.zeros_like(sldb), 'sldb': sldb,
                      'sld': sumlogdet})
        if idx is not None:
            m.update({'xeps': dyn.xeps[idx], 'veps': dyn.veps[idx]})
        dyn.update_history(m, history)
        return energy

    if verbose:
        record(h_init, 0 if merged else None)
    late_pe = late_idx = late_fwd = None
    for i, forward in enumerate(directions):
        if i > 0:
            v = stepper.flip(v)
        for step in range(nlf):
            x, v, logdet = stepper.step(step, x, v, forward)
            if late_pe is not None:
                sumlogdet = sumlogdet + stepper.ld1
                add_sld(late_fwd, stepper.ld1)
                h = record(stepper.ke + late_pe, late_idx, late_fwd)
            sumlogdet = sumlogdet + logdet
            if not verbose:
                continue
            if merged:
                add_sld(forward, logdet)
            idx = step if (forward or not merged) else nlf - step - 1
            if stepper.late:
                late_pe, late_idx, late_fwd = dyn._potential_n(x, beta), idx, forward
            else:
                h = record(dyn._hamiltonian_n(x, v, beta), idx, forward)
    last = stepper.finish(x, v)
    if last is not None:
        sumlogdet = sumlogdet + last
    if late_pe is not None:
        if last is not None:
            add_sld(late_fwd, last)
        h = record(dyn._kinetic_n(v) + late_pe, late_idx, late_fwd)
    if not verbose or nlf == 0:
        h = dyn._hamiltonian_n(x, v, beta)
    h_pair = (h_init, h) if merged else (h, h_init)
    acc = dyn._accept_prob_n(*h_pair, sumlogdet)
    history.update({'acc': acc, 'sumlogdet': sumlogdet})
    if verbose:
        history = dyn._stack_history(history)
    return x, v, history, h_init, h
```

l2hmc-qcd_amd/l2hmc/native.py:

```python
from __future__ import annotations

import ctypes as C
import os
from typing import Optional

import torch

_HERE = os.path.dirname(os.path.abspath(__file__))
LIB_PATH = os.path.join(_HERE, '_lib', os.environ.get('L2Q_LIB_NAME', 'libl2q.so'))

ACT = {None: 0, 'none': 0, 'tanh': 1, 'relu': 2, 'leaky_relu': 3, 'elu': 4, 'swish': 5}

P, I, L, D, F, Z = C.c_void_p, C.c_int, C.c_long, C.c_double, C.c_float, C.c_size_t

SIGNATURES = {
    'l2q_last_error': (C.c_char_p, []),
    'l2q_version': (I, []),
    'l2q_set_tuning': (I, [C.c_char_p, I]),
    'l2q_kernel_name': (I, [C.c_char_p, I, I, I, I, C.c_char_p, Z]),
    'l2q_init': (I, [I]),
    'l2q_comm_unique_id': (I, [P]),
    'l2q_comm_init': (I, [P, I, I, C.POINTER(P)]),
    'l2q_allreduce_grads': (I, [P, P, L, I, P]),
    'l2q_comm_destroy': (I, [P]),
    'l2q_comm_abort': (I, [P]),
    'l2q_comm_version': (I, []),
    'l2q_reduce_ws_bytes': (Z, [I, L]),
    'l2q_transpose': (I, [P, P, L, I, I, I, P]),
    'l2q_su3_pack': (I, [P, P, I, L, P]),
    'l2q_su3_unpack': (I, [P, P, I, L, P]),
    'l2q_su3_unpack_select': (I, [P, P, P, P, I, L, P]),
    'l2q_su3_plaq_reduce': (I, [P, I, I, I, I, I, P, P, Z, P]),
    'l2q_su3_plaq_planes': (I, [P, I, I, I, I, I, P, P, Z, P]),
    'l2q_su3_wilson_loops': (I, [P, I, I, I, I, I, P, P]),
    'l2q_diff_norm2_reduce': (I, [P, P, I, L, P, P, Z, P]),
    'l2q_su3_force': (I, [P, D, P, I, I, I, I, I, P]),
    'l2q_su3_force_kick': (I, [P, D, D, P, I, I, I, I, I, P]),
    'l2q_su3_force_kick_to': (I, [P, D, D, P, P, I, I, I, I, I, P]),
    'l2q_su3_expm_mul': (I, [P, P, D, P, I, P, I, L, P]),
    'l2q_su3_expm_mul2': (I, [P, P, D, P, I, P, I, L, P]),
    'l2q_su3_expm_mul2_vec8': (I, [P, P, D, P, I, P, P, I, L, P]),
    'l2q_su3_expm_mul2_digits': (I, [P, P, D, P, I, P, P, I, I, L, P]),
    'l2q_su3_projsu_digits': (I, [P, P, I, L, L, P]),
    'l2q_su3_project_su': (I, [P, P, L, L, P]),
    'l2q_su3_projsu_vec8': (I, [P, P, L, L, P]),
    'l2q_su3_project_tah': (I, [P, P, L, L, P]),
    'l2q_su3_project_u': (I, [P, P, L, L, P]),
    'l2q_su3_mul': (I, [P, P, I, I, P, L, L, P]),
    'l2q_su3_kinetic_reduce': (I, [P, I, L, P, P, Z, P]),
    'l2q_su3_assemble_tah': (I, [P, P, L, L, P]),
    'l2q_su3_check_su': (I, [P, I, L, P, P, Z, P]),
    'l2q_su3_clover_reduce': (I, [P, I, I, I, I, I, P, P, Z, P]),
    'l2q_su3_flow_stage': (I, [P, P, D, D, P, P, I, I, I, I, I, P]),
    'l2q_su3_flow_step': (I, [P, P, P, P, D, I, I, I, I, I, P]),
    'l2q_su3_line_extend': (I, [P, P, I, P, I, I, I, I, I, P]),
    'l2q_su3_loop_reduce': (I, [P, I, P, I, P, I, I, I, I, I, P, Z, P]),
    'l2q_su3_polyakov': (I, [P, I, P, I, I, I, I, I, P]),
    'l2q_su3_heatbath': (I, [P, D, I, I, P, I, P, I, I, I, I, I, P, Z, P]),
    'l2q_su3_overrelax': (I, [P, I, I, I, I, I, I, I, P]),
    'l2q_v_update': (I, [P, P, P, P, P, D, I, I, I, I, L, P, P, Z, P]),
    'l2q_v_update_to': (I, [P, P, P, P, P, P, D, I, I, I, I, L, P, P, Z, P]),
    'l2q_accept': (I, [P, P, P, P, P, P, I, I, P]),
    'l2q_select_rows': (I, [P, P, P, P, I, L, P]),
    'l2q_scale_f64': (I, [P, D, P, L, P]),
    'l2q_gemm_f64': (I, [P, P, I, I, L, P, P, L, P, P, P, D, I, P, P, Z, P]),
    'l2q_gemm_ws_bytes': (Z, [I, I, L, L]),
    'l2q_gemm_sliced_bytes': (Z, [I, L]),
    'l2q_gemm_sliced_build': (I, [P, I, L, P, Z, P, P]),
    'l2q_gemm_sliced_ws_bytes': (Z, [I, I, L, L]),
    'l2q_gemm_sliced_f64': (I, [P, P, L, I, P, P, L, I, I, I, P, P, P, D, I, P, P, Z, P]),
    'l2q_gemm_digits_bytes': (Z, [L, L]),
    'l2q_gemm_digits_slice': (I, [P, L, L, I, P, Z, P]),
    'l2q_gemm_digits_f64': (I, [P, P, L, I, P, P, L, I, I, I, P, P, P, D, I, P, P, Z, P]),
    'l2q_vnet_heads_vupdate_f64': (I, [P, I, I, L, P, P, P, D, P, P, D, P, P, P, D, P, P, I, D, I, P, P, Z, P]),
    'l2q_vnet_heads_vupdate_to_f64': (I, [P, I, I, L, P, P, P, D, P, P, D, P, P, P, D, P, P, P, I, D, I, P, P, Z, P]),
    'l2q_vnet_heads_vupdate_pair_f64': (I, [P, I, I, L, P, P, P, D, P, P, D, P, P, P, D, P, P, I, D, I, I, D, I, P, P, Z, P]),
    'l2q_vnet_heads_vupdate_pair_mid_f64': (I, [P, I, I, L, P, P, P, D, P, P, D, P, P, P, D, P, P, I, D, I, I, D, I, P, P, P, P, Z, P]),
    'l2q_vnet_heads_ws_bytes': (Z, [I, L]),
    'l2q_heads_sliced_bytes': (Z, [I, L]),
    'l2q_heads_sliced_build': (I, [P, P, P, I, L, P, Z, P, P]),
    'l2q_heads_sliced_zflag': (I, [I, P, P]),
    'l2q_vnet_heads_sliced_ws_bytes': (Z, [I, L]),
    'l2q_vnet_heads_vupdate_sliced_f64': (I, [P, I, I, L, P, P, P, D, P, D, P, P, D, P, P, P, I, D, I, I, I, D,
                                              I, P, P, P, P, Z, P]),
    'l2q_vnet_heads_vupdate_sliced_tape_f64': (I, [P, I, I, L, P, P, P, P, D, P, P, P, P, P, I, D, I, P, P, P, P,
                                                   P, Z, P]),
    'l2q_gemm_f32': (I, [P, P, I, I, L, P, P, L, P, P, P, F, I, P, P, Z, P]),
    'l2q_gemm_ex': (I, [P, I, P, I, I, I, L, I, I, P, P, Z, P]),
    'l2q_gemm_h': (I, [I, P, I, P, I, I, L, P, P, L, P, P, P, F, I, P, I, P, Z, P]),
    'l2q_gemm_h_ws_bytes': (Z, [I, I, L, L]),
    'l2q_gemm_h_skinny_splits': (I, [I, I, L, L, I]),
    'l2q_gemm_h_u1x': (I, [I, P, P, I, P, I, I, L, P, P, L, P, P, I, P, P, Z, P]),
    'l2q_u1_heads_update_h': (I, [I, P, I, I, L, P, P, P, P, P, F, P, P, P, I, P, P, P, I, F, I, I, P,
                                  I, P, Z, P]),
    'l2q_u1_heads_update_h_ws_bytes': (Z, [I, L]),
    'l2q_conv_gemm_periodic_h': (I, [I, P, I, L, L, L, L, I, I, I, I, I, P, I, P, I, I, P, P]),
    'l2q_conv_pool_gemm_periodic_h': (I, [I, P, I, L, L, L, L, I, I, I, I, I, P, I, P, I, I, P, P]),
    'l2q_maxpool_act_nhwc_h': (I, [I, P, I, I, I, I, I, I, P, P]),
    'l2q_nchw_to_nhwc_pad_h': (I, [I, P, I, I, I, I, I, P, P]),
    'l2q_u1_plaq_reduce': (I, [P, I, I, I, I, P, P]),
    'l2q_u1_wilson_loops': (I, [P, I, I, I, I, P, P]),
    'l2q_u1_wilson_loops_bwd': (I, [P, I, I, I, I, P, P]),
    'l2q_u1_force': (I, [P, D, P, P, D, I, I, I, I, P]),
    'l2q_u1_x_update': (I, [P, P, P, P, P, P, I, D, I, I, I, I, L, P, P]),
    'l2q_u1_wrap': (I, [P, P, L, I, P]),
    'l2q_u1_kinetic_reduce': (I, [P, I, L, I, P, P]),
    'l2q_axpy': (I, [P, D, P, L, I, P]),
    'l2q_u1_masked_cos_sin': (I, [P, P, I, P, I, L, I, P]),
    'l2q_conv2d_periodic_f32': (I, [P, P, P, P, I, I, I, I, I, I, I, I, P]),
    'l2q_im2col_periodic_f32': (I, [P, L, L, L, L, I, I, I, I, I, I, P, P]),
    'l2q_maxpool_act_nhwc_f32': (I, [P, I, I, I, I, I, I, P, P]),
    'l2q_conv_gemm_periodic_f32': (I, [P, L, L, L, L, I, I, I, I, I, P, I, P, I, I, P, P]),
    'l2q_nchw_to_nhwc_pad_f32': (I, [P, I, I, I, I, I, P, P]),
    'l2q_im2col_periodic_f64': (I, [P, L, L, L, L, I, I, I, I, I, I, P, P]),
    'l2q_maxpool_act_nhwc_f64': (I, [P, I, I, I, I, I, I, P, P]),
    'l2q_conv_gemm_periodic_f64': (I, [P, L, L, L, L, I, I, I, I, I, P, I, P, I, I, P, P]),
    'l2q_nchw_to_nhwc_pad_f64': (I, [P, I, I, I, I, I, P, P]),
    'l2q_u1_fused_max_n': (I, []),
    'l2q_u1_vstep_f32': (I, [P, P, D, D, I, I, I, I, P, P, P, P, P, I, P, P, P, P, P, D, P, P, P, I, I, P, P]),
    'l2q_u1_xstep_f32': (I, [P, P, P, I, D, I, I, I, I, P, P, P, P, P, I, P, P, P, P, P, D, P, P, P, I, I, P, P]),
    'l2q_act_fwd': (I, [P, I, L, I, P, P]),
    'l2q_act_bwd': (I, [P, P, I, L, I, P, P]),
    'l2q_act_bwd_sums': (I, [P, P, I, L, I, I, P, P, P, Z, P]),
    'l2q_act_fwd_r16': (I, [I, P, I, L, P, P]),
    'l2q_mul': (I, [P, P, D, L, I, P, P]),
    'l2q_axpy_rows': (I, [P, P, I, L, I, P, P]),
    'l2q_colsum': (I, [P, P, L, I, D, I, I, P, P, Z, P]),
    'l2q_colsum_ws_bytes': (Z, [L, I]),
    'l2q_scaled_tanh_bwd': (I, [P, P, P, D, I, I, I, P, P]),
    'l2q_scaled_tanh_bwd_sums': (I, [P, P, P, D, I, I, I, P, P, P, P, Z, P]),
    'l2q_bn_train_fwd': (I, [P, P, P, D, D, P, P, I, I, I, P, P, P, P]),
    'l2q_bn_bwd': (I, [P, P, P, P, P, I, I, I, P, P, P, P]),
    'l2q_col2im_periodic_f32': (I, [P, L, L, L, L, I, I, I, I, I, I, P, P]),
# ... 129 lines not shown
```

Baseline: 96210 chain*leapfrog-steps/s.

## Fuse plaquette action into force kernel and kinetic norms into momentum/heads kernels

Adds a force+action kernel that accumulates the plaquette real trace during the link-force sweep, so the potential energy for the Hamiltonian comes from the force pass instead of a separate plaquette reduction over the gauge field. Also fuses the momentum norm into the TAH momentum assembly and into the non-paired v-update heads kernel, so the separate kinetic-energy reductions are skipped. The trajectory code threads these cached energies through a sentinel and new stepper fields, which adds bookkeeping complexity and an extra finalize launch.

```diff
diff --git a/include/l2q.h b/include/l2q.h
--- a/include/l2q.h
+++ b/include/l2q.h
@@ -55,6 +55,9 @@
                           size_t ws_bytes, void* stream);
 int l2q_su3_force(const void* xn, double beta, void* fn, int nb, int T, int X, int Y, int Z,
                   void* stream);
+size_t l2q_su3_force_action_ws_bytes(int nb, int T, int X, int Y, int Z);
+int l2q_su3_force_action(const void* xn, double beta, void* fn, double* plaq, int nb, int T, int X, int Y, int Z,
+                         void* ws, size_t ws_bytes, void* stream);
 int l2q_su3_force_kick(const void* xn, double beta, double coef, void* vn, int nb, int T,
                        int X, int Y, int Z, void* stream);
 int l2q_su3_force_kick_to(const void* xn, double beta, double coef, const void* v_in, void* v_out,
@@ -78,6 +81,8 @@
 int l2q_su3_kinetic_reduce(const void* vn, int nb, long V, double* out, void* ws,
                            size_t ws_bytes, void* stream);
 int l2q_su3_assemble_tah(const double* normals, void* vn, long nfields, long V, void* stream);
+int l2q_su3_assemble_tah_norm2(const double* normals, void* vn, int nb, long V, double* norm2, void* ws,
+                               size_t ws_bytes, void* stream);
 int l2q_su3_check_su(const void* xn, int nb, long V, double* out, void* ws, size_t ws_bytes,
                      void* stream);
 
diff --git a/l2hmc-qcd_amd/csrc/heads_common.hpp b/l2hmc-qcd_amd/csrc/heads_common.hpp
--- a/l2hmc-qcd_amd/csrc/heads_common.hpp
+++ b/l2hmc-qcd_amd/csrc/heads_common.hpp
@@ -82,6 +82,7 @@
   double* tape_s = nullptr;
   double* tape_t = nullptr;
   double* tape_q = nullptr;
+  int want_ke = 0;
 };
 
 }
diff --git a/l2hmc-qcd_amd/csrc/heads_sliced.hip b/l2hmc-qcd_amd/csrc/heads_sliced.hip
--- a/l2hmc-qcd_amd/csrc/heads_sliced.hip
+++ b/l2hmc-qcd_amd/csrc/heads_sliced.hip
@@ -457,6 +457,7 @@
         }
         if (!PAIR) {
           if (ok) ld[r] += lj;
+          if (!TAPE && ok && a.want_ke) ke[r] += fma(vr, vr, vi * vi);
         } else {
           if (MID) { if (ok) { ld1[r] += lj; ke[r] += fma(vr, vr, vi * vi); } }
           if (a.flip) { vr = -vr; vi = -vi; }
@@ -570,18 +571,18 @@
 #pragma unroll
   for (int r = 0; r < 4; ++r) {
     double x = ld[r], x1 = ld1[r], xk = ke[r];
+    const bool vn2 = !PAIR && !TAPE && a.want_ke;
 #pragma unroll
     for (int off = 8; off > 0; off >>= 1) {
       x += __shfl_xor(x, off, 64);
-      if (MID) { x1 += __shfl_xor(x1, off, 64); xk += __shfl_xor(xk, off, 64); }
+      if (MID) x1 += __shfl_xor(x1, off, 64);
+      if (MID || vn2) xk += __shfl_xor(xk, off, 64);
     }
     const long m = mrow + r;
     if ((lane & 15) == 0 && m < a.M) {
       a.logdet_part[m * a.ncols_part + cw] = x;
-      if (MID) {
-        a.ld1_part[m * a.ncols_part + cw] = x1;
-        a.ke_part[m * a.ncols_part + cw] = xk;
-      }
+      if (MID) a.ld1_part[m * a.ncols_part + cw] = x1;
+      if (MID || vn2) a.ke_part[m * a.ncols_part + cw] = xk;
     }
   }
 }
@@ -635,6 +636,8 @@
   a.v = (double*)v; a.vin = (const double*)vin; a.F = (const double*)force;
   a.logdet_part = part; a.ld1_part = part + (size_t)M * ncw; a.ke_part = part + 2 * (size_t)M * ncw;
   a.M = M; a.N = (int)N; a.K = K; a.ncols_part = ncw;
+  const bool vn2 = !pair && !mid && !tape_s && vnorm2_mid != nullptr;
+  a.want_ke = vn2 ? 1 : 0;
   SlicedArgs o;
   o.Zs = zs; o.zscale = zscale; o.Wsl = (const char*)sliced;
   o.wscale = (const double*)((const char*)sliced + sliced_scale_off(N));
@@ -689,6 +692,7 @@
     launch_finalize(a.ld1_part, logdet1, M, ncw, 1, 1.0, 0.0, st);
     launch_finalize(a.ke_part, vnorm2_mid, M, ncw, 1, 1.0, 0.0, st);
   }
+  if (vn2) launch_finalize(a.ke_part, vnorm2_mid, M, ncw, 1, 1.0, 0.0, st);
   return check_launch(who);
 }
 
diff --git a/l2hmc-qcd_amd/csrc/su3_force_link.hip b/l2hmc-qcd_amd/csrc/su3_force_link.hip
--- a/l2hmc-qcd_amd/csrc/su3_force_link.hip
+++ b/l2hmc-qcd_amd/csrc/su3_force_link.hip
@@ -35,7 +35,9 @@
 __host__ __device__ constexpr int lk_other(int mu, int j) { return j + (j >= mu ? 1 : 0); }
 
 template <int MODE, int MU, int INM>
-__device__ __forceinline__ void force_link_sweep(const LkCtx& c) {
+__device__ __forceinline__ double force_link_sweep(const LkCtx& c) {
+  constexpr bool ACTION = MODE == 3;
+  double esum = 0.0;
   constexpr bool IN_MU = lk_in<INM>(MU);
   const Dims& d = c.d;
   const int T = d.T, V16 = c.V16, Vs16 = c.Vs16;
@@ -219,13 +221,14 @@
           double sr = 0.0, si = 0.0;
 #pragma unroll
           for (int k = 0; k < 3; ++k) {
-            if (L2Q_LK_FULL_DIAG || i != j) { sr = fma(ur.re[k], acc.re[3 * k + j], sr); sr = fma(-ur.im[k], acc.im[3 * k + j], sr); }
+            if (L2Q_LK_FULL_DIAG || ACTION || i != j) { sr = fma(ur.re[k], acc.re[3 * k + j], sr); sr = fma(-ur.im[k], acc.im[3 * k + j], sr); }
             si = fma(ur.re[k], acc.im[3 * k + j], si); si = fma(ur.im[k], acc.re[3 * k + j], si);
           }
           ua.re[3 * i + j] = sr; ua.im[3 * i + j] = si;
         }
       }
       const int so = MU * 9 * V16 + gcur;
+      if (ACTION) esum += (ua.re[0] + ua.re[4]) + ua.re[8];
       const double tri = (ua.im[0] + ua.im[4] + ua.im[8]) / 3.0;
 #pragma unroll
       for (int i = 0; i < 3; ++i)
@@ -268,19 +271,20 @@
     cur ^= 1;
     if (!(L2Q_LK_EXP & 8)) __syncthreads();
   }
+  return esum;
 }
 
 #ifndef L2Q_LK_OCC
 #define L2Q_LK_OCC 2
 #endif
 template <int MODE, int INM>
-__global__ __launch_bounds__(kLkThreads, L2Q_LK_OCC) void su3_force_link_kernel(
-    const double2* __restrict__ xn, Dims d, int nsb, int tsplit, int swz, double coef,
-    const double2* vin, double2* out, int lo, int stagger) {
+__device__ __forceinline__ double force_link_block(const double2* __restrict__ xn, const Dims& d, int nsb, int tsplit,
+                                                   int swz, double coef, const double2* vin, double2* out, int lo,
+                                                   int stagger, long& w) {
   if (stagger > 0 && blockIdx.x >= 256 && blockIdx.x < 512) {
     for (int i = 0; i < stagger; ++i) __builtin_amdgcn_s_sleep(32);
   }
-  const long w = xcd_swizzle(blockIdx.x, gridDim.x, swz);
+  w = xcd_swizzle(blockIdx.x, gridDim.x, swz);
   const int per_chain = nsb * tsplit;
   const long c = w / per_chain;
   const int rr = (int)(w % per_chain);
@@ -299,7 +303,7 @@
   const int chain_bytes = 36 * k.V16;
   k.rs = __builtin_amdgcn_make_buffer_rsrc((void*)(xn + c * 36L * V), 0, chain_bytes, 0x00020000);
   k.ro = __builtin_amdgcn_make_buffer_rsrc((void*)(out + c * 36L * V), 0, chain_bytes, 0x00020000);
-  k.rv = __builtin_amdgcn_make_buffer_rsrc((void*)((MODE != 0 ? vin : out) + c * 36L * V), 0, chain_bytes, 0x00020000);
+  k.rv = __builtin_amdgcn_make_buffer_rsrc((void*)((MODE == 1 || MODE == 2 ? vin : out) + c * 36L * V), 0, chain_bytes, 0x00020000);
   k.sp = sb * kRS + k.lt;
   {
     int q = k.sp;
@@ -310,11 +314,29 @@
   k.coef = coef;
   k.lo = lo;
   switch (wv) {
-    case 0: force_link_sweep<MODE, 0, INM>(k); break;
-    case 1: force_link_sweep<MODE, 1, INM>(k); break;
-    case 2: force_link_sweep<MODE, 2, INM>(k); break;
-    default: force_link_sweep<MODE, 3, INM>(k); break;
-  }
+    case 0: return force_link_sweep<MODE, 0, INM>(k);
+    case 1: return force_link_sweep<MODE, 1, INM>(k);
+    case 2: return force_link_sweep<MODE, 2, INM>(k);
+    default: return force_link_sweep<MODE, 3, INM>(k);
+  }
+}
+
+template <int MODE, int INM>
+__global__ __launch_bounds__(kLkThreads, L2Q_LK_OCC) void su3_force_link_kernel(
+    const double2* __restrict__ xn, Dims d, int nsb, int tsplit, int swz, double coef,
+    const double2* vin, double2* out, int lo, int stagger) {
+  long w;
+  (void)force_link_block<MODE, INM>(xn, d, nsb, tsplit, swz, coef, vin, out, lo, stagger, w);
+}
+
+template <int INM>
+__global__ __launch_bounds__(kLkThreads, L2Q_LK_OCC) void su3_force_link_action_kernel(
+    const double2* __restrict__ xn, Dims d, int nsb, int tsplit, int swz, double coef, double2* out, int lo,
+    int stagger, double* __restrict__ part) {
+  long w;
+  const double e = force_link_block<3, INM>(xn, d, nsb, tsplit, swz, coef, out, out, lo, stagger, w);
+  const double r = block_sum(e, reinterpret_cast<double*>(fr_lds));
+  if (threadIdx.x == 0) part[w] = r;
 }
 
 template <int MODE, int INM>
@@ -355,12 +377,43 @@
   }
 }
 
+static int force_link_tsplit(const Dims& d, int nb) {
+  return t_chunks((long)nb * (d.X * d.Y * d.Z / kRS), d.T, 1024, tuning().force_tsplit);
+}
+
+long force_link_action_parts(const Dims& d, int nb) { return (long)(d.X * d.Y * d.Z / kRS) * force_link_tsplit(d, nb); }
+
+template <int INM>
+static void launch_link_action(const double2* xn, Dims d, int nb, int nsb, int tsplit, double coef, double2* out,
+                               double* part, hipStream_t st) {
+  static PerDeviceOnce attr_once;
+  if (attr_once.first()) {
+    (void)hipFuncSetAttribute((const void*)su3_force_link_action_kernel<INM>,
+                              hipFuncAttributeMaxDynamicSharedMemorySize, kLkLds);
+  }
+  hipLaunchKernelGGL((su3_force_link_action_kernel<INM>), dim3((unsigned)((long)nb * nsb * tsplit)),
+                     dim3(kLkThreads), kLkLds, st, xn, d, nsb, tsplit, tuning().xcd_swizzle, coef, out, 1,
+                     tuning().force_stagger, part);
+}
+
+void launch_force_link_action(const double2* xn, Dims d, int nb, double coef, double2* out, double* part,
+                              hipStream_t st) {
+  const int nsb = d.X * d.Y * d.Z / kRS;
+  const int tsplit = force_link_tsplit(d, nb);
+  switch (force_link_inmask(d)) {
+    case 7: launch_link_action<7>(xn, d, nb, nsb, tsplit, coef, out, part, st); break;
+    case 6: launch_link_action<6>(xn, d, nb, nsb, tsplit, coef, out, part, st); break;
+    case 4: launch_link_action<4>(xn, d, nb, nsb, tsplit, coef, out, part, st); break;
+    default: launch_link_action<0>(xn, d, nb, nsb, tsplit, coef, out, part, st);
+  }
+}
+
 void launch_force_link(bool kick, const double2* xn, Dims d, int nb, double coef, double2* out, hipStream_t st,
                        const double2* vin) {
   if (vin == nullptr) vin = out;
   const int Vs = d.X * d.Y * d.Z;
   const int nsb = Vs / kRS;
-  const int tsplit = t_chunks((long)nb * nsb, d.T, 1024, tuning().force_tsplit);
+  const int tsplit = force_link_tsplit(d, nb);
 #define L2Q_LK_CASE(M)                                                                    \
   case M:                                                                                 \
     if (kick) launch_link_variant<1, M>(xn, d, nb, nsb, tsplit, coef, vin, out, st);           \
diff --git a/l2hmc-qcd_amd/csrc/su3_kernels.hip b/l2hmc-qcd_amd/csrc/su3_kernels.hip
--- a/l2hmc-qcd_amd/csrc/su3_kernels.hip
+++ b/l2hmc-qcd_amd/csrc/su3_kernels.hip
@@ -716,12 +716,8 @@
   store_link(out + f * 9L * V, V, s, r);
 }
 
-__global__ __launch_bounds__(kBlock) void su3_assemble_tah_kernel(const double* __restrict__ nrm,
-                                                                  double2* __restrict__ vn, long V,
-                                                                  long nblk, long nlinks) {
-  const long f = blockIdx.x / nblk, blk = blockIdx.x % nblk;
-  const long s = blk * kBlock + threadIdx.x;
-  if (s >= V) return;
+__device__ __forceinline__ double assemble_tah_link(const double* __restrict__ nrm, double2* __restrict__ vn,
+                                                    long V, long nlinks, long f, long s) {
   const long l = f * V + s;
   const double h = 0.70710678118654757;
   const double r3 = h * nrm[0 * nlinks + l];
@@ -730,15 +726,43 @@
   const double r12 = h * nrm[4 * nlinks + l], i01 = h * nrm[5 * nlinks + l];
   const double i02 = h * nrm[6 * nlinks + l], i12 = h * nrm[7 * nlinks + l];
   double2* o = vn + f * 9 * V;
-  o[0 * V + s] = make_double2(0.0, r8 + r3);
-  o[1 * V + s] = make_double2(r01, i01);
-  o[2 * V + s] = make_double2(r02, i02);
-  o[3 * V + s] = make_double2(-r01, i01);
-  o[4 * V + s] = make_double2(0.0, r8 - r3);
-  o[5 * V + s] = make_double2(r12, i12);
-  o[6 * V + s] = make_double2(-r02, i02);
-  o[7 * V + s] = make_double2(-r12, i12);
-  o[8 * V + s] = make_double2(0.0, -2.0 * r8);
+  const double2 m[9] = {make_double2(0.0, r8 + r3), make_double2(r01, i01),      make_double2(r02, i02),
+                        make_double2(-r01, i01),    make_double2(0.0, r8 - r3),  make_double2(r12, i12),
+                        make_double2(-r02, i02),    make_double2(-r12, i12),     make_double2(0.0, -2.0 * r8)};
+  double acc = 0.0;
+#pragma unroll
+  for (int e = 0; e < 9; ++e) {
+    o[e * V + s] = m[e];
+    acc = fma(m[e].x, m[e].x, acc);
+    acc = fma(m[e].y, m[e].y, acc);
+  }
+  return acc;
+}
+
+__global__ __launch_bounds__(kBlock) void su3_assemble_tah_kernel(const double* __restrict__ nrm,
+                                                                  double2* __restrict__ vn, long V,
+                                                                  long nblk, long nlinks) {
+  const long f = blockIdx.x / nblk, blk = blockIdx.x % nblk;
+  const long s = blk * kBlock + threadIdx.x;
+  if (s >= V) return;
+  (void)assemble_tah_link(nrm, vn, V, nlinks, f, s);
+}
+
+__global__ __launch_bounds__(kBlock) void su3_assemble_tah_norm2_kernel(const double* __restrict__ nrm,
+                                                                        double2* __restrict__ vn, long V,
+                                                                        long nblk, long nlinks,
+                                                                        double* __restrict__ partial) {
+  __shared__ double lds[4];
+  const long f = blockIdx.x / nblk, blk = blockIdx.x % nblk;
+  const long s = blk * kBlock + threadIdx.x;
+  const double acc = s < V ? assemble_tah_link(nrm, vn, V, nlinks, f, s) : 0.0;
+  const double r = block_sum(acc, lds);
+  if (threadIdx.x == 0) partial[blockIdx.x] = r;
+}
+
+__global__ void su3_plaq_re_kernel(const double* __restrict__ sums, double* __restrict__ out, int nb) {
+  const int c = blockIdx.x * blockDim.x + threadIdx.x;
+  if (c < nb) out[c] = sums[2 * c];
 }
 
 __global__ __launch_bounds__(kBlock) void su3_norm2_kernel(const double2* __restrict__ vn,
@@ -886,6 +910,15 @@
     force_kernel_name<false>(dd, buf, buf_bytes);
   } else if (!strcmp(entry, "l2q_su3_force_kick")) {
     force_kernel_name<true>(dd, buf, buf_bytes);
+  } else if (!strcmp(entry, "l2q_su3_force_action")) {
+    if (pick_force(dd, false) == ForceKernel::Link) {
+      snprintf(buf, buf_bytes, "su3_force_link_action_kernel<%d>", force_link_inmask(dd));
+    } else {
+      char force[128], plaq[128];
+      force_kernel_name<false>(dd, force, sizeof(force));
+      (void)l2q_kernel_name("l2q_su3_plaq_reduce", T, X, Y, Z, plaq, sizeof(plaq));
+      snprintf(buf, buf_bytes, "%s + %s", force, plaq);
+    }
   } else if (!strcmp(entry, "l2q_su3_clover_reduce")) {
     snprintf(buf, buf_bytes, "%s", clover_slice_applicable(dd) ? "su3_clover_slice_kernel" : "su3_clover_kernel");
   } else if (!strcmp(entry, "l2q_su3_flow_stage")) {
@@ -996,6 +1029,34 @@
   return check_launch("l2q_su3_force");
 }
 
+size_t l2q_su3_force_action_ws_bytes(int nb, int T, int X, int Y, int Z) {
+  if (!su3_dims_ok(nb, T, X, Y, Z)) return 0;
+  return (((size_t)nb * 2 * sizeof(double) + 255) & ~(size_t)255) + l2q_reduce_ws_bytes(nb, 36L * T * X * Y * Z);
+}
+
+int l2q_su3_force_action(const void* xn, double beta, void* fn, double* plaq, int nb, int T, int X, int Y, int Z,
+                         void* ws, size_t ws_bytes, void* stream) {
+  L2Q_REQUIRE(xn && fn && plaq && ws, L2Q_EINVAL, "null pointer");
+  L2Q_REQUIRE(su3_dims_ok(nb, T, X, Y, Z), L2Q_EINVAL, "non-positive size");
+  L2Q_REQUIRE(xn != fn, L2Q_EINVAL, "force output must not alias the gauge field");
+  L2Q_REQUIRE(ws_bytes >= l2q_su3_force_action_ws_bytes(nb, T, X, Y, Z), L2Q_ESHAPE, "workspace too small");
+  const Dims d = make_dims(T, X, Y, Z);
+  hipStream_t st = (hipStream_t)stream;
+  if (pick_force(d, false) == ForceKernel::Link) {
+    const long parts = force_link_action_parts(d, nb);
+    launch_force_link_action((const double2*)xn, d, nb, beta / 3.0, (double2*)fn, (double*)ws, st);
+    launch_finalize((const double*)ws, plaq, nb, parts, 1, 0.25, 0.0, st);
+    return check_launch("l2q_su3_force_action");
+  }
+  launch_force<false>((const double2*)xn, d, nb, beta / 3.0, (double2*)fn, st);
+  const size_t head = ((size_t)nb * 2 * sizeof(double) + 255) & ~(size_t)255;
+  const int rc = l2q_su3_plaq_reduce(xn, nb, T, X, Y, Z, (double*)ws, (char*)ws + head, ws_bytes - head, stream);
+  if (rc != L2Q_OK) return rc;
+  hipLaunchKernelGGL(su3_plaq_re_kernel, dim3((unsigned)cdiv(nb, kBlock)), dim3(kBlock), 0, st, (const double*)ws,
+                     plaq, nb);
+  return check_launch("l2q_su3_force_action");
+}
+
 int l2q_su3_force_kick(const void* xn, double beta, double coef, void* vn, int nb, int T, int X,
                        int Y, int Z, void* stream) {
   L2Q_REQUIRE(xn && vn, L2Q_EINVAL, "null pointer");
@@ -1156,6 +1217,19 @@
   hipLaunchKernelGGL(su3_assemble_tah_kernel, dim3((unsigned)(nfields * nblk)), dim3(kBlock), 0,
                      (hipStream_t)stream, normals, (double2*)vn, V, nblk, nfields * V);
   return check_launch("l2q_su3_assemble_tah");
+}
+
+int l2q_su3_assemble_tah_norm2(const double* normals, void* vn, int nb, long V, double* norm2, void* ws,
+                               size_t ws_bytes, void* stream) {
+  L2Q_REQUIRE(normals && vn && norm2 && ws, L2Q_EINVAL, "null pointer");
+  L2Q_REQUIRE(su3_field_ok(nb, V), L2Q_EINVAL, "bad size");
+  const long nblk = cdiv(V, kBlock);
+  L2Q_REQUIRE(ws_bytes >= (size_t)nb * 4 * nblk * sizeof(double), L2Q_ESHAPE, "workspace too small");
+  hipStream_t st = (hipStream_t)stream;
+  hipLaunchKernelGGL(su3_assemble_tah_norm2_kernel, dim3((unsigned)(nb * 4L * nblk)), dim3(kBlock), 0, st, normals,
+                     (double2*)vn, V, nblk, nb * 4L * V, (double*)ws);
+  launch_finalize((const double*)ws, norm2, nb, 4 * nblk, 1, 1.0, 0.0, st);
+  return check_launch("l2q_su3_assemble_tah_norm2");
 }
 
 int l2q_su3_check_su(const void* xn, int nb, long V, double* out, void* ws, size_t ws_bytes,
diff --git a/l2hmc-qcd_amd/csrc/su3_launch.hpp b/l2hmc-qcd_amd/csrc/su3_launch.hpp
--- a/l2hmc-qcd_amd/csrc/su3_launch.hpp
+++ b/l2hmc-qcd_amd/csrc/su3_launch.hpp
@@ -23,6 +23,9 @@
                        const double2* vin = nullptr);
 void launch_force_link_bwd(const double2* xn, Dims d, int nb, double coef, const double2* gf, double2* gx,
                            hipStream_t st);
+long force_link_action_parts(const Dims& d, int nb);
+void launch_force_link_action(const double2* xn, Dims d, int nb, double coef, double2* out, double* part,
+                              hipStream_t st);
 bool force_plaq_applicable(const Dims& d);
 void launch_force_plaq(const double2* xn, Dims d, int nb, double coef, double2* out, hipStream_t st);
 bool clover_slice_applicable(const Dims& d);
diff --git a/l2hmc-qcd_amd/l2hmc/_ops.py b/l2hmc-qcd_amd/l2hmc/_ops.py
--- a/l2hmc-qcd_amd/l2hmc/_ops.py
+++ b/l2hmc-qcd_amd/l2hmc/_ops.py
@@ -117,6 +117,19 @@
     f = torch.empty_like(xn)
     N.call('l2q_su3_force', xn, float(beta), f, nb, T, X, Y, Z)
     return f
+
+
+USE_KERNEL_ENERGIES = [True]
+
+
+def su3_force_action_n(xn: torch.Tensor, beta: float, lat: Sequence[int]):
+    nb = xn.shape[0]
+    T, X, Y, Z = (int(i) for i in lat)
+    f = torch.empty_like(xn)
+    plaq = torch.empty(nb, dtype=torch.float64, device=xn.device)
+    ws = N.workspace(int(N.load().l2q_su3_force_action_ws_bytes(nb, T, X, Y, Z)), xn.device)
+    N.call('l2q_su3_force_action', xn, float(beta), f, plaq, nb, T, X, Y, Z, ws, ws.numel())
+    return f, plaq
 
 
 def su3_force_kick_n(xn: torch.Tensor, beta: float, coef: float, vn: torch.Tensor,
@@ -215,6 +228,16 @@
     out = torch.empty((*lead, 9, V), dtype=C128, device=normals.device)
     N.call('l2q_su3_assemble_tah', normals.contiguous(), out, nf, V)
     return out
+
+
+def su3_assemble_tah_norm2_n(normals: torch.Tensor):
+    _, nb, four, V = normals.shape
+    assert four == 4
+    out = torch.empty((nb, 4, 9, V), dtype=C128, device=normals.device)
+    n2 = torch.empty(nb, dtype=torch.float64, device=normals.device)
+    ws = _ws(nb, 4 * V, normals.device)
+    N.call('l2q_su3_assemble_tah_norm2', normals.contiguous(), out, nb, V, n2, ws, ws.numel())
+    return out, n2
 
 
 def su3_check_su_n(xn: torch.Tensor) -> torch.Tensor:
@@ -718,19 +741,20 @@
 
 
 def _sliced_call(z, heads, scales, v, force, eps1, forward1, pair, flip, eps2, forward2, v_src=None,
-                 mid=False):
+                 mid=False, norm2=False):
     m, k = z.shape
     _, bs, cs = heads['s']
     _, bt, _ = heads['t']
     wq, bq, cq = heads['q']
     n = wq.shape[0]
-    out = torch.empty((3 if mid else 1, m), dtype=torch.float64, device=z.device)
+    assert not (norm2 and (pair or mid))
+    out = torch.empty((3 if mid or norm2 else 1, m), dtype=torch.float64, device=z.device)
     nbytes = int(N.load().l2q_vnet_heads_sliced_ws_bytes(m, n))
     ws = N.workspace(nbytes, z.device)
     N.call('l2q_vnet_heads_vupdate_sliced_f64', z, m, k, n, heads['sliced'], bs, cs, float(scales[0]), bt,
            float(scales[1]), bq, cq, float(scales[2]), v_src, v, force, int(v.is_complex()), float(eps1),
            int(forward1), int(pair), int(flip), float(eps2), int(forward2), out[0],
-           out[1] if mid else None, out[2] if mid else None, ws, ws.numel())
+           out[1] if mid else None, out[2] if mid or norm2 else None, ws, ws.numel())
     return out
 
 
@@ -742,7 +766,7 @@
 
 def vnet_heads_vupdate_(z: torch.Tensor, heads: dict, scales, v: torch.Tensor,
                         force: torch.Tensor, eps: float, forward: bool,
-                        v_src: Optional[torch.Tensor] = None) -> torch.Tensor:
+                        v_src: Optional[torch.Tensor] = None, norm2: Optional[list] = None) -> torch.Tensor:
     m, k = z.shape
     ws_, bs, cs = heads['s']
     wt, bt, _ = heads['t']
@@ -751,7 +775,11 @@
     if _use_sliced(z, heads):
         if v_src is not None:
             assert v_src.shape == v.shape and v_src.dtype == v.dtype and v_src.is_contiguous()
-        return _sliced_call(z, heads, scales, v, force, eps, forward, False, False, 0.0, False, v_src)[0]
+        out = _sliced_call(z, heads, scales, v, force, eps, forward, False, False, 0.0, False, v_src,
+                           norm2=norm2 is not None)
+        if norm2 is not None:
+            norm2.append(out[2])
+        return out[0]
     logdet = torch.empty(m, dtype=torch.float64, device=z.device)
     nbytes = int(N.load().l2q_vnet_heads_ws_bytes(m, n))
     ws = N.workspace(nbytes, z.device)
diff --git a/l2hmc-qcd_amd/l2hmc/dynamics/pytorch/dynamics.py b/l2hmc-qcd_amd/l2hmc/dynamics/pytorch/dynamics.py
--- a/l2hmc-qcd_amd/l2hmc/dynamics/pytorch/dynamics.py
+++ b/l2hmc-qcd_amd/l2hmc/dynamics/pytorch/dynamics.py
@@ -2,6 +2,7 @@
 
 import logging
 import os
+import weakref
 from dataclasses import dataclass
 from math import pi as PI
 from pathlib import Path
@@ -186,6 +187,7 @@
         self.fuse_half_heads = True
         self.merge_hmc_kicks = True
         self._inject: Optional[dict] = None
+        self._mom_norm2 = None
         self._eps_cache: dict = {}
         self._masks_native: Optional[list] = None
         self._perm: dict = {}
@@ -436,8 +438,21 @@
         s = ops.u1_plaq_sums(xn, self.latvolume)
         return _beta(beta) * (self.volume - s[:, 0])
 
+    def _potential_from_plaq(self, plaq: Tensor, beta) -> Tensor:
+        return (-_beta(beta) / 3.0) * plaq
+
+    def _kinetic_from_norm2(self, n2: Tensor) -> Tensor:
+        return 0.5 * (n2 - 8.0 * 4.0 * self.volume)
+
     def _kinetic_n(self, vn: Tensor) -> Tensor:
+        kept, self._mom_norm2 = self._mom_norm2, None
+        if kept is not None and kept[0]() is vn:
+            return self._kinetic_from_norm2(kept[1])
         return ops.su3_kinetic_n(vn) if self.group == 'SU3' else ops.u1_kinetic(vn)
+
+    def _kernel_energies(self, xn: Tensor) -> bool:
+        return bool(ops.USE_KERNEL_ENERGIES[0] and self.group == 'SU3' and xn.is_cuda
+                    and self.potential_c1 == 0.0 and not self.training)
 
     def _hamiltonian_n(self, xn: Tensor, vn: Tensor, beta) -> Tensor:
         return self._kinetic_n(vn) + self._potential_n(xn, beta)
@@ -453,7 +468,12 @@
                                    for _ in range(8)]).to(DEVICE)
             else:
                 nrm = torch.randn((8, *shape), dtype=torch.float64, device=DEVICE)
-            return ops.su3_assemble_tah_n(nrm.reshape(8, nb, 4, self.volume))
+            nrm = nrm.reshape(8, nb, 4, self.volume)
+            if ops.USE_KERNEL_ENERGIES[0] and inj is None and not self.training and nrm.is_cuda:
+                vn, n2 = ops.su3_assemble_tah_norm2_n(nrm)
+                self._mom_norm2 = (weakref.ref(vn), n2)
+                return vn
+            return ops.su3_assemble_tah_n(nrm)
         shape = (nb, 2, *self.latvolume)
         if inj is not None:
             v = torch.as_tensor(inj).to(DEVICE)
@@ -522,7 +542,12 @@
         if reuse and ts.valid:
             fn = ts.F
         else:
-            fn = self._force_n(xn, beta)
+            if reuse and ts.want_pe:
+                fn, ts.plaq = ops.su3_force_action_n(xn, _beta(beta), self.latvolume)
+            else:
+                fn = self._force_n(xn, beta)
+                if reuse:
+                    ts.plaq = None
             if reuse:
                 ts.valid, ts.F = True, fn
                 ts.xv = ts.fv = None
@@ -580,7 +605,7 @@
 
     def _update_v_n(self, step: int, xn: Tensor, vn: Tensor, beta, forward: bool,
                     ts: Optional[SamplerStepper] = None, acc: Optional[Tensor] = None,
-                    v_src: Optional[Tensor] = None) -> Tensor:
+                    v_src: Optional[Tensor] = None, norm2: Optional[list] = None) -> Tensor:
         eps = self._eps('v', step)
         nb = xn.shape[0]
         vnet = self._get_vnet(step)
@@ -603,7 +628,7 @@
         if z is not None:
             return ops.vnet_heads_vupdate_(z, w['heads_scaled'], (vnet.nw.s, vnet.nw.t, vnet.nw.q),
                                            vn.reshape(nb, -1), fn.reshape(nb, -1), eps, forward,
-                                           None if v_src is None else v_src.reshape(nb, -1))
+                                           None if v_src is None else v_src.reshape(nb, -1), norm2=norm2)
         if v_src is not None:
             vn.copy_(v_src)
         s, t, q = self._vnet_n(step, xn, fn)
@@ -621,7 +646,7 @@
         if ts is None or not ts.late:
             return ops.vnet_heads_vupdate_pair_(*args)
         ld, ts.ld1, vn2 = ops.vnet_heads_vupdate_pair_mid_(*args)
-        ts.ke = 0.5 * (vn2 - 8.0 * 4.0 * self.volume)
+        ts.ke = self._kinetic_from_norm2(vn2)
         return ld - ts.ld1
 
     def _can_pair_mid(self) -> bool:
@@ -689,6 +714,7 @@
         if ts is not None:
             prev, x_src, v_src = ts.pending, ts.x_src, ts.v_src
             ts.pending = ts.x_src = ts.v_src = None
+            ts.want_pe = bool(ts.energies and ts.late and prev is not None)
         late = bool(prev is not None and ts.late)
         xr = xn if x_src is None else x_src
         if v_src is not None and prev is not None:
@@ -742,7 +768,11 @@
             return None
         ts.pending = None
         st0, f0, flip = prev
-        ld = self._update_v_n(st0, xn, vn, beta, f0, ts)
+        n2 = [] if ts.energies else None
+        ts.want_pe = ts.energies
+        ld = self._update_v_n(st0, xn, vn, beta, f0, ts, norm2=n2)
+        ts.want_pe = False
+        ts.ke_out = self._kinetic_from_norm2(n2[0]) if n2 else None
         if flip:
             self._flip_v_n(vn)
         return ld
@@ -1333,7 +1363,7 @@
         flags = (d.fuse_heads, d.fuse_x_updates, d.reuse_v_inputs, d.pair_v_updates,
                  d.fuse_u1_steps, d.fuse_half_heads, d.merge_hmc_kicks, d.sliced_heads,
                  ops.USE_SLICED_HEADS[0], d.sliced_input, ops.USE_SLICED_INPUT[0], ops.USE_DIGIT_INPUTS[0],
-                 d.pair_v_updates_verbose,
+                 ops.USE_KERNEL_ENERGIES[0], d.pair_v_updates_verbose,
                  getattr(d, 'fuse_x_vec8', None), d.net_precision, d.config.verbose, d.training)
         return (ops.PARAM_GENERATION[0], params, masks, flags)
 
diff --git a/l2hmc-qcd_amd/l2hmc/dynamics/pytorch/trajectory.py b/l2hmc-qcd_amd/l2hmc/dynamics/pytorch/trajectory.py
--- a/l2hmc-qcd_amd/l2hmc/dynamics/pytorch/trajectory.py
+++ b/l2hmc-qcd_amd/l2hmc/dynamics/pytorch/trajectory.py
@@ -4,11 +4,13 @@
 
 Tensor = torch.Tensor
 
+_WITH_FORCE = object()
+
 
 class SamplerStepper:
     __slots__ = ('dyn', 'beta', 'reuse', 'defer', 'late', 'lazy', 'x_src', 'v_src',
                  'valid', 'F', 'xv_pre', 'xv', 'fv', 'z',
-                 'pending', 'ld1', 'ke')
+                 'pending', 'ld1', 'ke', 'energies', 'want_pe', 'plaq', 'ke_out')
 
     def __init__(self, dyn, beta, merged: bool):
         verbose = dyn.config.verbose
@@ -24,8 +26,11 @@
         self.z = {}
         self.pending = self.ld1 = self.ke = None
         self.lazy = bool(merged and su3 and dyn.config.nleapfrog > 0)
+        self.energies = self.want_pe = False
+        self.plaq = self.ke_out = None
 
     def start(self, xn: Tensor, vn: Tensor):
+        self.energies = bool(self.defer and self.lazy and self.dyn._kernel_energies(xn))
         if not self.lazy:
             return xn.clone(), vn.clone()
         self.x_src, self.v_src = xn, vn
@@ -43,11 +48,20 @@
     def finish(self, x: Tensor, v: Tensor):
         return self.dyn._flush_pending_n(self, x, v, self.beta)
 
+    def potential(self, x: Tensor) -> Tensor:
+        if self.plaq is None:
+            return self.dyn._potential_n(x, self.beta)
+        return self.dyn._potential_from_plaq(self.plaq, self.beta)
+
+    def kinetic_out(self, v: Tensor) -> Tensor:
+        return self.dyn._kinetic_n(v) if self.ke_out is None else self.ke_out
+
 
 def run_trajectory(dyn, stepper, xn: Tensor, vn: Tensor, beta, directions: tuple):
     merged = len(directions) == 2
     verbose, nlf = dyn.config.verbose, dyn.config.nleapfrog
     x, v = stepper.start(xn, vn)
+    energies = getattr(stepper, 'energies', False)
     sumlogdet = dyn._zeros_nb(xn.shape[0])
     sldf = sldb = torch.zeros_like(sumlogdet) if merged else None
     history: dict = {}
@@ -81,6 +95,8 @@
             if late_pe is not None:
                 sumlogdet = sumlogdet + stepper.ld1
                 add_sld(late_fwd, stepper.ld1)
+                if late_pe is _WITH_FORCE:
+                    late_pe = dyn._potential_from_plaq(stepper.plaq, beta)
                 h = record(stepper.ke + late_pe, late_idx, late_fwd)
             sumlogdet = sumlogdet + logdet
             if not verbose:
@@ -89,7 +105,8 @@
                 add_sld(forward, logdet)
             idx = step if (forward or not merged) else nlf - step - 1
             if stepper.late:
-                late_pe, late_idx, late_fwd = dyn._potential_n(x, beta), idx, forward
+                late_pe = _WITH_FORCE if energies else dyn._potential_n(x, beta)
+                late_idx, late_fwd = idx, forward
             else:
                 h = record(dyn._hamiltonian_n(x, v, beta), idx, forward)
     last = stepper.finish(x, v)
@@ -98,9 +115,12 @@
     if late_pe is not None:
         if last is not None:
             add_sld(late_fwd, last)
-        h = record(dyn._kinetic_n(v) + late_pe, late_idx, late_fwd)
+        if late_pe is _WITH_FORCE:
+            h = record(stepper.kinetic_out(v) + stepper.potential(x), late_idx, late_fwd)
+        else:
+            h = record(dyn._kinetic_n(v) + late_pe, late_idx, late_fwd)
     if not verbose or nlf == 0:
-        h = dyn._hamiltonian_n(x, v, beta)
+        h = stepper.kinetic_out(v) + stepper.potential(x) if energies else dyn._hamiltonian_n(x, v, beta)
     h_pair = (h_init, h) if merged else (h, h_init)
     acc = dyn._accept_prob_n(*h_pair, sumlogdet)
     history.update({'acc': acc, 'sumlogdet': sumlogdet})
diff --git a/l2hmc-qcd_amd/l2hmc/native.py b/l2hmc-qcd_amd/l2hmc/native.py
--- a/l2hmc-qcd_amd/l2hmc/native.py
+++ b/l2hmc-qcd_amd/l2hmc/native.py
@@ -36,6 +36,8 @@
     'l2q_diff_norm2_reduce': (I, [P, P, I, L, P, P, Z, P]),
     'l2q_su3_force': (I, [P, D, P, I, I, I, I, I, P]),
     'l2q_su3_force_kick': (I, [P, D, D, P, I, I, I, I, I, P]),
+    'l2q_su3_force_action_ws_bytes': (Z, [I, I, I, I, I]),
+    'l2q_su3_force_action': (I, [P, D, P, P, I, I, I, I, I, P, Z, P]),
     'l2q_su3_force_kick_to': (I, [P, D, D, P, P, I, I, I, I, I, P]),
     'l2q_su3_expm_mul': (I, [P, P, D, P, I, P, I, L, P]),
     'l2q_su3_expm_mul2': (I, [P, P, D, P, I, P, I, L, P]),
@@ -49,6 +51,7 @@
     'l2q_su3_mul': (I, [P, P, I, I, P, L, L, P]),
     'l2q_su3_kinetic_reduce': (I, [P, I, L, P, P, Z, P]),
     'l2q_su3_assemble_tah': (I, [P, P, L, L, P]),
+    'l2q_su3_assemble_tah_norm2': (I, [P, P, I, L, P, P, Z, P]),
     'l2q_su3_check_su': (I, [P, I, L, P, P, Z, P]),
     'l2q_su3_clover_reduce': (I, [P, I, I, I, I, I, P, P, Z, P]),
     'l2q_su3_flow_stage': (I, [P, P, D, D, P, P, I, I, I, I, I, P]),
```

After: 98050 chain*leapfrog-steps/s, median of 6. 1.02x the previous value.
